# ika-rwth-aachen/PCLSegmentation

Measured on NVIDIA B200. Metric: range-image frames/sec (SqueezeSegV2, 64x2048), higher is better.
Workload: dtype f16 storage / f32 accumulate

## Files before the change

pclsegmentation_b200/csrc/conv_tc.cu:

```cuda
#include "tc_ptx.cuh"

#include <cstring>

namespace pcls {

constexpr int TC_MAX_TAPS = 9;
#ifndef PCLS_TC_VSTREAM
#define PCLS_TC_VSTREAM 0
#endif
#ifndef PCLS_TC_NG_NORES
#define PCLS_TC_NG_NORES 2
#endif
constexpr int tc_ng(bool res) { return res ? 2 : PCLS_TC_NG_NORES; }
constexpr int tc_threads(bool res) { return 64 + 128 * tc_ng(res); }

struct TcParams {
  int pdl_early;
  int BW, BH, bw_shift;
  int n_wt, n_ht, n_nt, n_phase, num_tiles;
  int Hgrid, Wgrid;
  int out_wmul;
  int Wout;
  int n_groups, sub;
  int kchunks;
  int ksteps;
  int KC, BN;
  int grp_dh[2][TC_MAX_TAPS], grp_dw[2][TC_MAX_TAPS], grp_par[2][TC_MAX_TAPS];
  int grp_w[2][TC_MAX_TAPS][3];
  int sub_row[3];
  int a_is_5d;
  int a_rows;
  int b_resident;
  int ntaps_total;
  int use_base_offset;
  int stages, a_bytes, b_tile_bytes, bres_bytes;
  uint32_t idesc, desc_hi;
  uint32_t tmem_cols;
  int n_acc;
  int tma_store, cbw, c_is_5d, c_stage_bytes;
  int G, cout_blk, cout_blk_shift;
  int res_smem;
  int res_tma;
  int n_cbuf;
  int n1, b_small_bytes, bres_tx;
  uint32_t idesc_small, idesc_lo;
  int nsplit, perm, cblk_off[8];
  int vstream, R, n_hseg;
  uint32_t desc_hi_b, idesc_blk;
  int cout, out_channels, out_coff, act, out_f32, is_bf16;
  void* out;
  const void* res0;
  const void* res1;
  int res0_channels, res1_channels;
  const float* bias;
  int skip;
  const void* skip_w;
  int head, none_index;
  const uint8_t* mask;
  float* probs;
  int32_t* preds;
  float* logits;
  unsigned long long* dbg;
};

template <typename T> __device__ __forceinline__ uint32_t pack2_relu(float lo, float hi);
template <> __device__ __forceinline__ uint32_t pack2_relu<__half>(float lo, float hi) {
  uint32_t d;
  asm("cvt.rn.relu.f16x2.f32 %0, %1, %2;" : "=r"(d) : "f"(hi), "f"(lo));
  return d;
}
template <> __device__ __forceinline__ uint32_t pack2_relu<__nv_bfloat16>(float lo, float hi) {
  uint32_t d;
  asm("cvt.rn.relu.bf16x2.f32 %0, %1, %2;" : "=r"(d) : "f"(hi), "f"(lo));
  return d;
}

template <typename T> __device__ __forceinline__ uint32_t add2_16(uint32_t a, uint32_t b);
template <> __device__ __forceinline__ uint32_t add2_16<__half>(uint32_t a, uint32_t b) {
  uint32_t d;
  asm("add.rn.f16x2 %0, %1, %2;" : "=r"(d) : "r"(a), "r"(b));
  return d;
}
template <> __device__ __forceinline__ uint32_t add2_16<__nv_bfloat16>(uint32_t a, uint32_t b) {
  uint32_t d;
  asm("add.rn.bf16x2 %0, %1, %2;" : "=r"(d) : "r"(a), "r"(b));
  return d;
}

#ifndef PCLS_TC_PACKED_SKIP
#define PCLS_TC_PACKED_SKIP 1
#endif

template <typename T> __device__ __forceinline__ uint32_t pack2_rn(float lo, float hi);
template <> __device__ __forceinline__ uint32_t pack2_rn<__half>(float lo, float hi) {
  uint32_t d;
  asm("cvt.rn.f16x2.f32 %0, %1, %2;" : "=r"(d) : "f"(hi), "f"(lo));
  return d;
}
template <> __device__ __forceinline__ uint32_t pack2_rn<__nv_bfloat16>(float lo, float hi) {
  uint32_t d;
  asm("cvt.rn.bf16x2.f32 %0, %1, %2;" : "=r"(d) : "f"(hi), "f"(lo));
  return d;
}
template <typename T> __device__ __forceinline__ void mma_16x8x8(float (&d)[4], uint32_t a0, uint32_t a1, uint32_t b);
template <> __device__ __forceinline__ void mma_16x8x8<__half>(float (&d)[4], uint32_t a0, uint32_t a1, uint32_t b) {
  asm volatile("mma.sync.aligned.m16n8k8.row.col.f32.f16.f16.f32 {%0, %1, %2, %3}, {%4, %5}, {%6}, {%7, %7, %7, %7};"
               : "=f"(d[0]), "=f"(d[1]), "=f"(d[2]), "=f"(d[3]) : "r"(a0), "r"(a1), "r"(b), "f"(0.0f));
}
template <> __device__ __forceinline__ void mma_16x8x8<__nv_bfloat16>(float (&d)[4], uint32_t a0, uint32_t a1, uint32_t b) {
  asm volatile("mma.sync.aligned.m16n8k8.row.col.f32.bf16.bf16.f32 {%0, %1, %2, %3}, {%4, %5}, {%6}, {%7, %7, %7, %7};"
               : "=f"(d[0]), "=f"(d[1]), "=f"(d[2]), "=f"(d[3]) : "r"(a0), "r"(a1), "r"(b), "f"(0.0f));
}
__device__ __forceinline__ void ldmatrix_x4(uint32_t addr, uint32_t (&r)[4]) {
  asm volatile("ldmatrix.sync.aligned.m8n8.x4.shared.b16 {%0, %1, %2, %3}, [%4];"
               : "=r"(r[0]), "=r"(r[1]), "=r"(r[2]), "=r"(r[3]) : "r"(addr) : "memory");
}
__device__ __forceinline__ void stmatrix_x4(uint32_t addr, uint32_t r0, uint32_t r1, uint32_t r2, uint32_t r3) {
  asm volatile("stmatrix.sync.aligned.m8n8.x4.shared.b16 [%0], {%1, %2, %3, %4};" ::"r"(addr), "r"(r0), "r"(r1), "r"(r2), "r"(r3)
               : "memory");
}

template <typename T, bool LEAKY, bool BIAS>
__device__ __forceinline__ int4 epilogue_vec8(const uint32_t* acc, const float* bias8, float lo, bool has_r0, const int4& r0,
                                              bool has_r1, const int4& r1) {
  if constexpr (!BIAS && !LEAKY) {
    if (!has_r0 && !has_r1) {
      int4 o;
      if (lo == 0.0f) {
        o.x = (int)pack2_relu<T>(__uint_as_float(acc[0]), __uint_as_float(acc[1]));
        o.y = (int)pack2_relu<T>(__uint_as_float(acc[2]), __uint_as_float(acc[3]));
        o.z = (int)pack2_relu<T>(__uint_as_float(acc[4]), __uint_as_float(acc[5]));
        o.w = (int)pack2_relu<T>(__uint_as_float(acc[6]), __uint_as_float(acc[7]));
      } else {
        const float f[8] = {__uint_as_float(acc[0]), __uint_as_float(acc[1]), __uint_as_float(acc[2]), __uint_as_float(acc[3]),
                            __uint_as_float(acc[4]), __uint_as_float(acc[5]), __uint_as_float(acc[6]), __uint_as_float(acc[7])};
        o = pack8<T>(f);
      }
      return o;
    }
  }
  if constexpr (PCLS_TC_PACKED_SKIP && !LEAKY) {
    if (has_r0 && !has_r1 && lo == 0.0f) {
      float v[8];
      if constexpr (BIAS) {
        const float4 b0 = *reinterpret_cast<const float4*>(bias8);
        const float4 b1 = *reinterpret_cast<const float4*>(bias8 + 4);
        v[0] = __uint_as_float(acc[0]) + b0.x; v[1] = __uint_as_float(acc[1]) + b0.y; v[2] = __uint_as_float(acc[2]) + b0.z;
        v[3] = __uint_as_float(acc[3]) + b0.w; v[4] = __uint_as_float(acc[4]) + b1.x; v[5] = __uint_as_float(acc[5]) + b1.y;
        v[6] = __uint_as_float(acc[6]) + b1.z; v[7] = __uint_as_float(acc[7]) + b1.w;
      } else {
#pragma unroll
        for (int j = 0; j < 8; ++j) v[j] = __uint_as_float(acc[j]);
      }
      int4 o;
      o.x = (int)add2_16<T>(pack2_relu<T>(v[0], v[1]), (uint32_t)r0.x);
      o.y = (int)add2_16<T>(pack2_relu<T>(v[2], v[3]), (uint32_t)r0.y);
      o.z = (int)add2_16<T>(pack2_relu<T>(v[4], v[5]), (uint32_t)r0.z);
      o.w = (int)add2_16<T>(pack2_relu<T>(v[6], v[7]), (uint32_t)r0.w);
      return o;
    }
  }
  float v[8];
  if constexpr (BIAS) {
    const float4 b0 = *reinterpret_cast<const float4*>(bias8);
    const float4 b1 = *reinterpret_cast<const float4*>(bias8 + 4);
    v[0] = __uint_as_float(acc[0]) + b0.x; v[1] = __uint_as_float(acc[1]) + b0.y; v[2] = __uint_as_float(acc[2]) + b0.z;
    v[3] = __uint_as_float(acc[3]) + b0.w; v[4] = __uint_as_float(acc[4]) + b1.x; v[5] = __uint_as_float(acc[5]) + b1.y;
    v[6] = __uint_as_float(acc[6]) + b1.z; v[7] = __uint_as_float(acc[7]) + b1.w;
  } else {
#pragma unroll
    for (int j = 0; j < 8; ++j) v[j] = __uint_as_float(acc[j]);
  }
#pragma unroll
  for (int j = 0; j < 8; ++j) v[j] = LEAKY ? fmaxf(v[j], v[j] * 0.1f) : fmaxf(v[j], lo);
  if (has_r0) {
    float f[8];
    unpack8<T>(r0, f);
#pragma unroll
    for (int j = 0; j < 8; ++j) v[j] += f[j];
  }
  if (has_r1) {
    float f[8];
    unpack8<T>(r1, f);
#pragma unroll
    for (int j = 0; j < 8; ++j) v[j] += f[j];
  }
  return pack8<T>(v);
}

template <typename T, int KC, int SUB, int G, bool RES, bool LEAKY, int KS = KC / 16, int RM = 0>
__global__ void __launch_bounds__(tc_threads(RES), 1)
conv_tc_kernel(const __grid_constant__ CUtensorMap map_a, const __grid_constant__ CUtensorMap map_b,
               const __grid_constant__ CUtensorMap map_c, const __grid_constant__ CUtensorMap map_r,
               const __grid_constant__ CUtensorMap map_b2, const __grid_constant__ CUtensorMap map_c2,
               const __grid_constant__ TcParams p, const int num_tiles) {
  constexpr bool PRELOAD = !RES;
  constexpr int TC_NG = tc_ng(RES);
  constexpr bool RTMA = RES && RM == 1;
  constexpr bool PTMA = !RES && RM == 2;
  constexpr bool SKIP = RES && RM == 3;
  static_assert(!SKIP || (G == 4 && !LEAKY), "the computed skip exists for the pixel-group view G = 4 with ReLU");
  constexpr bool FIXED = RTMA || SKIP;
  extern __shared__ uint8_t smem_raw[];
  const uint32_t smem_base = (smem_u32(smem_raw) + 1023u) & ~1023u;
  const int S = p.stages;
  const uint32_t a_bytes = (uint32_t)p.a_bytes, b_tile_bytes = (uint32_t)p.b_tile_bytes;
  const bool b_resident = p.b_resident != 0;
  const uint32_t b_stage_bytes = b_resident ? 0u : (uint32_t)SUB * b_tile_bytes;
  const uint32_t stage_bytes = a_bytes + b_stage_bytes;
  const uint32_t bres_base = smem_base + (uint32_t)S * stage_bytes;
  const uint32_t cstage_base = bres_base + (uint32_t)p.bres_bytes;
  const uint32_t rstage_base = cstage_base + (p.tma_store ? (uint32_t)(p.n_cbuf * TC_NG) * (uint32_t)p.c_stage_bytes : 0u);
  const uint32_t bar_base = rstage_base + ((RES && (SKIP || p.res_smem)) ? (uint32_t)TC_NG * 16384u : 0u);
#define FULL_BAR(s) (bar_base + 8u * (uint32_t)(s))
#define EMPTY_BAR(s) (bar_base + 8u * (uint32_t)(S + (s)))
#define TFULL_BAR(a) (bar_base + 8u * (uint32_t)(2 * S + (a)))
#define TEMPTY_BAR(a) (bar_base + 8u * (uint32_t)(2 * S + 8 + (a)))
#define BRES_BAR (bar_base + 8u * (uint32_t)(2 * S + 16))
#define RFULL_BAR(i) (bar_base + 8u * (uint32_t)(2 * S + 17 + (i)))
  const uint32_t tmem_slot = bar_base + 8u * (uint32_t)(2 * S + 17 + 3 * TC_NG);
  volatile uint32_t* tmem_slot_ptr =
      reinterpret_cast<volatile uint32_t*>(smem_raw + (tmem_slot - smem_u32(smem_raw)));
  float* bias_s = reinterpret_cast<float*>(smem_raw + (((tmem_slot + 16u + 15u) & ~15u) - smem_u32(smem_raw)));
  for (int i = threadIdx.x; i < p.n_nt * p.BN; i += blockDim.x) bias_s[i] = p.bias[G > 1 ? i % p.cout_blk : i];
  float* head_s = bias_s + ((p.n_nt * p.BN + 3) & ~3);

  const int warp = threadIdx.x >> 5, lane = threadIdx.x & 31;
  unsigned long long* const dbg = PCLS_TC_DEBUG ? p.dbg : nullptr;
  unsigned long long dbg_acc[8] = {0, 0, 0, 0, 0, 0, 0, 0};
  const unsigned long long dbg_start = dbg ? clk() : 0ull;

  if (warp == 0 && lane == 0) {
    asm volatile("prefetch.tensormap [%0];" ::"l"(&map_a) : "memory");
    asm volatile("prefetch.tensormap [%0];" ::"l"(&map_b) : "memory");
    if (p.n1 > 0) asm volatile("prefetch.tensormap [%0];" ::"l"(&map_b2) : "memory");
    if (p.tma_store) asm volatile("prefetch.tensormap [%0];" ::"l"(&map_c) : "memory");
    if (RES && (SKIP || p.res_tma)) asm volatile("prefetch.tensormap [%0];" ::"l"(&map_r) : "memory");
    for (int i = 0; i < 3 * TC_NG; ++i) mbar_init(RFULL_BAR(i), 1);
    for (int s = 0; s < S; ++s) { mbar_init(FULL_BAR(s), 1); mbar_init(EMPTY_BAR(s), 1); }
    for (int a = 0; a < 8; ++a) { mbar_init(TFULL_BAR(a), 1); mbar_init(TEMPTY_BAR(a), 4); }
    mbar_init(BRES_BAR, 1);
    asm volatile("fence.mbarrier_init.release.cluster;" ::: "memory");
    asm volatile("fence.proxy.async.shared::cta;" ::: "memory");
  }
  if (warp == 1) {
    asm volatile("tcgen05.alloc.cta_group::1.sync.aligned.shared::cta.b32 [%0], %1;" ::"r"(tmem_slot), "r"(p.tmem_cols)
                 : "memory");
    asm volatile("tcgen05.relinquish_alloc_permit.cta_group::1.sync.aligned;" ::: "memory");
  }
  tc_fence_before();
  __syncthreads();
  tc_fence_after();
  const uint32_t tmem_base = *tmem_slot_ptr;
  pdl_trigger(p.pdl_early);
  if (warp != 0) pdl_wait();

  const int n_groups = p.n_groups, kchunks = p.kchunks, n_nt = p.n_nt, n_phase = p.n_phase, n_wt = p.n_wt, n_ht = p.n_ht;
  const int BN = p.BN;

  if (warp == 0) {
    {
      if (b_resident) {
        mbar_arrive_expect_tx_elect(BRES_BAR, (uint32_t)p.bres_tx);
        uint32_t dst = bres_base;
        const int n0r = p.nsplit ? (int)(blockIdx.x % (unsigned)n_nt) * BN : 0;
        for (int ph = 0; ph < n_phase; ++ph)
          for (int g = 0; g < n_groups; ++g)
            for (int kc = 0; kc < kchunks; ++kc)
#pragma unroll
              for (int u = 0; u < SUB; ++u) {
                const int tap = p.grp_w[ph][g][u];
                if (p.n1 > 0 && tap != 4) {
                  tma_load_3d_elect(dst, &map_b2, BRES_BAR, kc * KC, n0r + p.n1, tap);
                  dst += (uint32_t)p.b_small_bytes;
                } else {
                  tma_load_3d_elect(dst, &map_b, BRES_BAR, kc * KC, n0r, tap);
                  dst += b_tile_bytes;
                }
              }
      }
      pdl_wait();
      const uint32_t a_tx_bytes = (uint32_t)(p.a_rows * KC * 2);
      const int BW = p.BW, BH = p.BH;
      const bool is5d = p.a_is_5d != 0;
      int stage = 0;
      uint32_t phase = 0;
      if (PCLS_TC_VSTREAM && p.vstream) {
        const int R = p.R, n_hseg = p.n_hseg, num_units = num_tiles / R;
        for (int unit = blockIdx.x; unit < num_units; unit += gridDim.x) {
          const int wt = unit % n_wt, hseg = (unit / n_wt) % n_hseg, b = unit / (n_wt * n_hseg);
          const int ww = wt * BW - 1;
          for (int hh = hseg * R - 1; hh <= hseg * R + R; ++hh)
            for (int kc = 0; kc < kchunks; ++kc) {
              { DBG_T0; mbar_wait(EMPTY_BAR(stage), phase ^ 1u); DBG_ADD(0); }
              const uint32_t fb = FULL_BAR(stage);
              mbar_arrive_expect_tx_elect(fb, a_tx_bytes);
              tma_load_4d_elect(smem_base + (uint32_t)stage * stage_bytes, &map_a, fb, kc * KC, ww, hh, b);
              if (++stage == S) { stage = 0; phase ^= 1u; }
            }
        }
      } else
      for (int tile = blockIdx.x; tile < num_tiles; tile += gridDim.x) {
        int r = tile;
        const int nt = r % n_nt; r /= n_nt;
        const int ph = r % n_phase; r /= n_phase;
        const int wt = r % n_wt; r /= n_wt;
        const int ht = r % n_ht;
        const int b = r / n_ht;
        const int w0 = wt * BW, h0 = ht * BH, n0 = nt * BN;
        for (int g = 0; g < n_groups; ++g) {
          const int hh = h0 + p.grp_dh[ph][g], ww = w0 + p.grp_dw[ph][g], par = p.grp_par[ph][g];
          int wtap[SUB];
#pragma unroll
          for (int u = 0; u < SUB; ++u) wtap[u] = p.grp_w[ph][g][u];
          for (int kc = 0; kc < kchunks; ++kc) {
            { DBG_T0; mbar_wait(EMPTY_BAR(stage), phase ^ 1u); DBG_ADD(0); }
            const uint32_t a_dst = smem_base + (uint32_t)stage * stage_bytes;
            const uint32_t fb = FULL_BAR(stage);
            uint32_t tx_bytes = a_tx_bytes;
            if (!b_resident) {
#pragma unroll
              for (int u = 0; u < SUB; ++u) tx_bytes += (p.n1 > 0 && wtap[u] != 4) ? (uint32_t)p.b_small_bytes : b_tile_bytes;
            }
            mbar_arrive_expect_tx_elect(fb, tx_bytes);
            if (is5d) tma_load_5d_elect(a_dst, &map_a, fb, kc * KC, par, ww, hh, b);
            else tma_load_4d_elect(a_dst, &map_a, fb, kc * KC, ww, hh, b);
            if (!b_resident) {
#pragma unroll
              for (int u = 0; u < SUB; ++u) {
                if (p.n1 > 0 && wtap[u] != 4)
                  tma_load_3d_elect(a_dst + a_bytes + (uint32_t)u * b_tile_bytes, &map_b2, fb, kc * KC, p.n1, wtap[u]);
                else
                  tma_load_3d_elect(a_dst + a_bytes + (uint32_t)u * b_tile_bytes, &map_b, fb, kc * KC, n0, wtap[u]);
              }
            }
            if (++stage == S) { stage = 0; phase ^= 1u; }
          }
        }
      }
    }
  } else if (warp == 1) {
    {
      const uint32_t desc_hi = p.desc_hi, idesc = p.idesc;
      const uint32_t n_acc = (uint32_t)p.n_acc;
      uint32_t sub_off[SUB];
#pragma unroll
      for (int u = 0; u < SUB; ++u) sub_off[u] = (uint32_t)(p.sub_row[u] * KC * 2);
      const int k_iters = n_groups * kchunks;
      const uint32_t bres_phase_bytes = (uint32_t)(k_iters * SUB) * b_tile_bytes;
      int stage = 0;
      uint32_t phase = 0, acc = 0, acc_phase = 0;
      if (b_resident) mbar_wait(BRES_BAR, 0u);
      const bool vs = PCLS_TC_VSTREAM && p.vstream != 0;
      const int vs_R = vs ? p.R : 1;
      const int my_tiles = vs ? ((num_tiles / vs_R - (int)blockIdx.x + (int)gridDim.x - 1) / (int)gridDim.x) * vs_R
                              : (num_tiles - (int)blockIdx.x + (int)gridDim.x - 1) / (int)gridDim.x;
      uint32_t vs_slot = 0, vs_phase = 0, vs_idx = 0, vs_waited = 0;
      int vs_row = 0;
      auto vs_release = [&](int n) {
        for (int i = 0; i < n; ++i) {
          umma_commit_elect(EMPTY_BAR(vs_slot));
          if (++vs_slot == (uint32_t)S) { vs_slot = 0; vs_phase ^= 1u; }
        }
        vs_idx += (uint32_t)n;
      };
      for (int seq = 0; seq < my_tiles; ++seq) {
        const int tile = blockIdx.x + seq * gridDim.x;
        { DBG_T0; mbar_wait(TEMPTY_BAR(acc), PRELOAD ? acc_phase : (acc_phase ^ 1u)); DBG_ADD(1); }
        tc_fence_after();
        const uint32_t d_tmem = tmem_base + acc * (uint32_t)BN;
        uint32_t b_res = bres_base + (n_phase > 1 ? (uint32_t)((tile / n_nt) % n_phase) * bres_phase_bytes : 0u);
        uint32_t accumulate = PRELOAD ? 1u : 0u, acc_lo = accumulate;
        int kc_i = 0, g_i = 0;
        for (int k = 0; k < k_iters; ++k) {
          uint32_t a_addr;
          if (vs) {
            uint32_t sl = vs_slot + (uint32_t)k, par = vs_phase;
            if (sl >= (uint32_t)S) { sl -= (uint32_t)S; par ^= 1u; }
            if (vs_idx + (uint32_t)k >= vs_waited) {
              { DBG_T0; mbar_wait(FULL_BAR(sl), par); DBG_ADD(2); }
              vs_waited = vs_idx + (uint32_t)k + 1u;
            }
            a_addr = smem_base + sl * stage_bytes;
          } else {
            { DBG_T0; mbar_wait(FULL_BAR(stage), phase); DBG_ADD(2); }
            a_addr = smem_base + (uint32_t)stage * stage_bytes;
          }
          tc_fence_after();
          if constexpr (G == 1) {
            uint32_t b_addr = b_resident ? b_res : a_addr + a_bytes;
            const uint32_t n1 = (uint32_t)p.n1;
#pragma unroll
            for (int u = 0; u < SUB; ++u) {
              const uint64_t a_desc = ((uint64_t)desc_hi << 32) | (uint64_t)((((a_addr + sub_off[u]) >> 4) & 0x3FFFu) | 0x10000u);
              const uint64_t b_desc = ((uint64_t)desc_hi << 32) | (uint64_t)(((b_addr >> 4) & 0x3FFFu) | 0x10000u);
              if (n1 == 0u) {
#pragma unroll
                for (int j = 0; j < KS; ++j) {
                  umma_f16_elect(d_tmem, a_desc + (uint64_t)(2 * j), b_desc + (uint64_t)(2 * j), idesc, accumulate);
                  accumulate = 1u;
                }
                b_addr += b_tile_bytes;
              } else if (p.grp_w[0][g_i][u] != 4) {
#pragma unroll
                for (int j = 0; j < KC / 16; ++j) {
                  umma_f16_elect(d_tmem + n1, a_desc + (uint64_t)(2 * j), b_desc + (uint64_t)(2 * j), p.idesc_small, accumulate);
                  accumulate = 1u;
                }
                b_addr += b_resident ? (uint32_t)p.b_small_bytes : b_tile_bytes;
              } else {
                const uint32_t b_hi = b_addr + n1 * (uint32_t)(KC * 2);
                const uint64_t b_desc_hi = ((uint64_t)desc_hi << 32) | (uint64_t)(((b_hi >> 4) & 0x3FFFu) | 0x10000u);
#pragma unroll
                for (int j = 0; j < KC / 16; ++j) {
                  umma_f16_elect(d_tmem, a_desc + (uint64_t)(2 * j), b_desc + (uint64_t)(2 * j), p.idesc_lo, acc_lo);
                  umma_f16_elect(d_tmem + n1, a_desc + (uint64_t)(2 * j), b_desc_hi + (uint64_t)(2 * j), p.idesc_small, accumulate);
                  acc_lo = 1u; accumulate = 1u;
                }
                b_addr += b_tile_bytes;
              }
            }
            if (b_resident) b_res = b_addr;
          } else {
            constexpr int CIN = KC / G;
            const uint32_t desc_hi_b = p.desc_hi_b, idesc_blk = p.idesc_blk, cout_blk = (uint32_t)p.cout_blk;
#pragma unroll
            for (int u = 0; u < SUB; ++u) {
              const uint32_t b_addr = b_res + (uint32_t)u * b_tile_bytes;
              const uint64_t b_desc = ((uint64_t)desc_hi_b << 32) | (uint64_t)(((b_addr >> 4) & 0x3FFFu) | 0x10000u);
#pragma unroll
              for (int pp = 0; pp < G; ++pp) {
                constexpr int dummy = 0; (void)dummy;
                const int t = pp + (SUB == 3 ? u - 1 : 0);
                const int dq = t < 0 ? -1 : (t >= G ? 1 : 0);
                const int par = t - dq * G;
                const uint32_t a_start = a_addr + (uint32_t)((SUB == 3 ? dq + 1 : 0) * KC * 2 + par * CIN * 2);
                const uint64_t a_desc = ((uint64_t)desc_hi << 32) | (uint64_t)(((a_start >> 4) & 0x3FFFu) | 0x10000u);
#pragma unroll
                for (int j = 0; j < CIN / 16; ++j)
                  umma_f16_elect(d_tmem + (uint32_t)pp * cout_blk, a_desc + (uint64_t)(2 * j), b_desc + (uint64_t)(2 * j),
                           idesc_blk, (PRELOAD || (k | u | j) != 0) ? 1u : 0u);
              }
            }
          }
          if constexpr (G > 1) b_res += (uint32_t)SUB * b_tile_bytes;
          if (++kc_i == kchunks) { kc_i = 0; ++g_i; }
          if (!vs) {
            umma_commit_elect(EMPTY_BAR(stage));
            if (++stage == S) { stage = 0; phase ^= 1u; }
          }
        }
        if (vs) {
          if (++vs_row == vs_R) { vs_row = 0; vs_release(3 * kchunks); }
          else vs_release(kchunks);
        }
        umma_commit_elect(TFULL_BAR(acc));
        if (++acc == n_acc) { acc = 0; acc_phase ^= 1u; }
      }
    }
  } else {
    const int grp = (warp - 2) >> 2;
    const int q = warp & 3;
    const int m = q * 32 + lane;
    const int ml_h = m >> p.bw_shift, ml_w = m & (p.BW - 1);
    const uint32_t n_acc = (uint32_t)p.n_acc;
    const int BW = p.BW, BH = p.BH, Hgrid = p.Hgrid, Wgrid = p.Wgrid, Wout = p.Wout, out_wmul = p.out_wmul;
    const int cout = p.cout, out_channels = p.out_channels, out_coff = p.out_coff;
    const int blk_shift = p.cout_blk_shift;
    const int blk_mask = G > 1 ? (1 << blk_shift) - 1 : -1;
    const float slope = p.act == PCLS_ACT_RELU ? 0.0f : (p.act == PCLS_ACT_LEAKY ? 0.1f : 1.0f);
    const float act_lo = (FIXED || p.act == PCLS_ACT_RELU) ? 0.0f : -INFINITY;
    const uint16_t* res0 = reinterpret_cast<const uint16_t*>(p.res0);
    const uint16_t* res1 = reinterpret_cast<const uint16_t*>(p.res1);
    const int res0_channels = p.res0_channels, res1_channels = p.res1_channels;
    const bool has_r0 = FIXED || res0 != nullptr, has_r1 = !FIXED && res1 != nullptr;
    const bool tma_store = FIXED || PTMA || p.tma_store != 0, out_f32 = !FIXED && !PTMA && p.out_f32 != 0, c_is_5d = p.c_is_5d != 0;
    const uint32_t c_stage_bytes = (uint32_t)p.c_stage_bytes;
    T* const outp = reinterpret_cast<T*>(p.out);
    const bool issuer = (q == 2) && lane == 0;
    const int bar_id = 1 + grp;
    const uint32_t ng = n_acc < (uint32_t)TC_NG ? n_acc : (uint32_t)TC_NG;
    uint32_t tl = 0, blk = 0;
    const uint32_t nrb = (uint32_t)p.n_cbuf;
    auto issue_res = [&](int rtile, int rcb, uint32_t bi) {
      int r2 = rtile;
      const int nt2 = r2 % n_nt; r2 /= n_nt;
      const int ph2 = r2 % n_phase; r2 /= n_phase;
      const int wt2 = r2 % n_wt; r2 /= n_wt;
      const int ht2 = r2 % n_ht;
      const int b2 = r2 / n_ht;
      const uint32_t dst = cstage_base + (uint32_t)(grp * p.n_cbuf + (int)bi) * c_stage_bytes;
      const uint32_t bar = RFULL_BAR(grp * 3 + (int)bi);
      const int pp2 = G > 1 ? (nt2 * BN + rcb) >> blk_shift : 0;
      const int c02 = out_coff + (p.perm ? p.cblk_off[(nt2 * BN + rcb) >> 6] : ((nt2 * BN + rcb) & blk_mask));
      mbar_arrive_expect_tx(bar, 128u * 64u * 2u);
      if (c_is_5d) tma_load_5d(dst, &map_r, bar, c02, G > 1 ? pp2 : ph2, wt2 * BW, ht2 * BH, b2);
      else tma_load_4d(dst, &map_r, bar, c02, wt2 * BW, ht2 * BH, b2);
    };
    const bool vs = PCLS_TC_VSTREAM && p.vstream != 0;
    const int vs_R = vs ? p.R : 1, vs_hseg = p.n_hseg;
    auto tile_at = [&](uint32_t seq) -> int {
      if (!vs) {
        const long long t = (long long)blockIdx.x + (long long)seq * gridDim.x;
        return t < num_tiles ? (int)t : -1;
      }
      const int unit = (int)blockIdx.x + (int)(seq / (uint32_t)vs_R) * (int)gridDim.x;
      if (unit >= num_tiles / vs_R) return -1;
      const int i = (int)(seq % (uint32_t)vs_R);
      const int uwt = unit % n_wt, hseg = (unit / n_wt) % vs_hseg, ub = unit / (n_wt * vs_hseg);
      return (ub * n_ht + hseg * vs_R + i) * n_wt + uwt;
    };
    if (RES && !SKIP && p.res_tma != 0 && has_r0 && issuer && (uint32_t)grp < ng && tile_at((uint32_t)grp) >= 0)
      issue_res(tile_at((uint32_t)grp), 0, 0u);
    uint32_t skw[8] = {0, 0, 0, 0, 0, 0, 0, 0};
    const uint32_t in_base = rstage_base + (uint32_t)grp * 16384u;
    const bool ones_lane = (lane & 3) == 3;
    const uint32_t one2 = std::is_same<T, __half>::value ? 0x3C003C00u : 0x3F803F80u;
    if constexpr (SKIP) {
      const uint32_t* w32 = reinterpret_cast<const uint32_t*>(p.skip_w);
#pragma unroll
      for (int j = 0; j < 8; ++j) skw[j] = __ldg(w32 + (8 * j + (lane >> 2)) * 4 + (lane & 3));
    }
    auto issue_in = [&](int rtile, uint32_t bi) {
      const int wt2 = (rtile / n_nt / n_phase) % n_wt;
      const int ht2 = (rtile / n_nt / n_phase / n_wt) % n_ht;
      const int b2 = rtile / n_nt / n_phase / n_wt / n_ht;
      const uint32_t bar = RFULL_BAR(grp * 3 + (int)bi);
      mbar_arrive_expect_tx(bar, 8192u);
      tma_load_4d(in_base + bi * 8192u, &map_r, bar, 0, wt2 * BW, ht2 * BH, b2);
    };
    auto compute_skip = [&](uint32_t buf, int pp, uint32_t in_buf) {
      uint32_t a[4];
      ldmatrix_x4(in_buf + (uint32_t)(m * 64) + (uint32_t)((pp ^ ((m >> 1) & 3)) << 4), a);
#pragma unroll
      for (int k = 0; k < 4; ++k) a[k] = ones_lane ? one2 : a[k];
      const int sr = (q * 32 + ((lane >> 3) & 1) * 8 + (lane & 7));
#pragma unroll
      for (int i = 0; i < 2; ++i)
#pragma unroll
        for (int jp = 0; jp < 4; ++jp) {
          float d0[4], d1[4];
          mma_16x8x8<T>(d0, a[2 * i], a[2 * i + 1], skw[2 * jp]);
          mma_16x8x8<T>(d1, a[2 * i], a[2 * i + 1], skw[2 * jp + 1]);
          const uint32_t chunk = (uint32_t)((2 * jp + (lane >> 4)) ^ (lane & 7));
          stmatrix_x4(buf + (uint32_t)((sr + 16 * i) * 128) + (chunk << 4), pack2_rn<T>(d0[0], d0[1]), pack2_rn<T>(d0[2], d0[3]),
                      pack2_rn<T>(d1[0], d1[1]), pack2_rn<T>(d1[2], d1[3]));
        }
      __syncwarp();
    };
    if (SKIP && issuer && (uint32_t)grp < ng && tile_at((uint32_t)grp) >= 0) issue_in(tile_at((uint32_t)grp), 0u);
    auto preload_bias = [&](uint32_t a, int tile_next) {
      if (tile_next >= 0) {
        const float* bsrc = bias_s + (tile_next % n_nt) * BN;
        const uint32_t t_dst = tmem_base + ((uint32_t)(q * 32) << 16) + a * (uint32_t)BN;
#pragma unroll 1
        for (int c = 0; c + 32 <= BN; c += 32) {
          uint32_t bv[32];
#pragma unroll
          for (int j = 0; j < 32; j += 4) {
            const float4 t4 = *reinterpret_cast<const float4*>(bsrc + c + j);
            bv[j] = __float_as_uint(t4.x); bv[j + 1] = __float_as_uint(t4.y); bv[j + 2] = __float_as_uint(t4.z); bv[j + 3] = __float_as_uint(t4.w);
          }
          tmem_st32(t_dst + (uint32_t)c, bv);
        }
        if (BN & 16) {
          uint32_t bv[16];
#pragma unroll
          for (int j = 0; j < 16; j += 4) {
            const float4 t4 = *reinterpret_cast<const float4*>(bsrc + (BN & ~31) + j);
            bv[j] = __float_as_uint(t4.x); bv[j + 1] = __float_as_uint(t4.y); bv[j + 2] = __float_as_uint(t4.z); bv[j + 3] = __float_as_uint(t4.w);
          }
          tmem_st16(t_dst + (uint32_t)(BN & ~31), bv);
        }
        tmem_st_wait();
      }
      tc_fence_before();
      __syncwarp();
      if (lane == 0) mbar_arrive(TEMPTY_BAR(a));
    };
    if (PRELOAD && (uint32_t)grp < ng)
      for (uint32_t a = (uint32_t)grp; a < n_acc; a += ng) preload_bias(a, tile_at(a));
    for (; (uint32_t)grp < ng; ++tl) {
      const int tile = tile_at(tl);
      if (tile < 0) break;
      if ((int)(tl % ng) != grp) continue;
      int r = tile;
      const int nt = r % n_nt; r /= n_nt;
      const int ph = r % n_phase; r /= n_phase;
      const int wt = r % n_wt; r /= n_wt;
      const int ht = r % n_ht;
      const int b = r / n_ht;
      const int h = ht * BH + ml_h, w = wt * BW + ml_w;
      const bool valid = h < Hgrid && w < Wgrid;
      const int64_t pix = ((int64_t)b * Hgrid + h) * Wout + (int64_t)w * out_wmul + ph;
      const uint32_t acc = tl & (n_acc - 1u), acc_parity = (tl / n_acc) & 1u;
      const int n0 = nt * BN;
      const uint32_t t_row = tmem_base + ((uint32_t)(q * 32) << 16) + acc * (uint32_t)BN;
      auto elem_off = [&](int n, int channels) -> int64_t {
        const int pp = G > 1 ? n >> blk_shift : 0;
        const int co = n & blk_mask;
        return (valid && co + 8 <= cout) ? (pix + pp) * channels + out_coff + co : (int64_t)-1;
      };
      const uint32_t rslot = rstage_base + (uint32_t)grp * 16384u + (uint32_t)(m & 127) * 16u;
      int4 r0[4], r1[4];
      const bool res_smem = !FIXED && RES && p.res_smem != 0 && has_r0;
      const bool res_tma = RTMA || (RES && !SKIP && p.res_tma != 0 && has_r0);
      const bool res_stage = res_tma || SKIP;
      uint32_t res_row = 0;
      auto prefetch_r0 = [&](int cs) {
        if constexpr (RES) {
          if (res_smem) {
#pragma unroll 4
            for (int i = 0; i < 8; ++i) {
              const int64_t o = (cs + i * 8 < BN) ? elem_off(n0 + cs + i * 8, res0_channels) : (int64_t)-1;
              cp_async16(rslot + (uint32_t)i * 2048u, res0 + (o >= 0 ? o : 0), o >= 0);
            }
            cp_async_commit();
          }
        }
      };
      auto load_r1 = [&](int c) {
        if constexpr (RES) {
#pragma unroll
          for (int g = 0; g < 4; ++g) {
            const int64_t o = has_r1 ? elem_off(n0 + c + g * 8, res1_channels) : (int64_t)-1;
            r1[g] = o >= 0 ? __ldg(reinterpret_cast<const int4*>(res1 + o)) : make_int4(0, 0, 0, 0);
            if (has_r0 && !res_smem && !res_stage) {
              const int64_t o0 = elem_off(n0 + c + g * 8, res0_channels);
              r0[g] = o0 >= 0 ? __ldg(reinterpret_cast<const int4*>(res0 + o0)) : make_int4(0, 0, 0, 0);
            }
          }
        }
      };
      const bool reg_res = RES && (has_r1 || (has_r0 && !res_smem && !res_stage));
      prefetch_r0(0);
      if (reg_res) load_r1(0);
      uint8_t head_mask = 1;
      if (out_f32 && p.head && valid) head_mask = p.mask[pix];
      { DBG_T0; mbar_wait(TFULL_BAR(acc), acc_parity); DBG_ADD(3); }
      const unsigned long long _te = dbg ? clk() : 0ull;
      tc_fence_after();
      if (res_smem) cp_async_wait_all();
      auto process = [&](const uint32_t* v, int cc, auto&& sink) {
        if constexpr (RES) {
          if (res_smem && cc > 0 && (cc & 63) == 0) { prefetch_r0(cc); cp_async_wait_all(); }
        }
#pragma unroll
        for (int g = 0; g < 4; ++g) {
          int4 r0v = make_int4(0, 0, 0, 0);
          if constexpr (RES) {
            r0v = res_stage ? ld_shared_v4(res_row + (uint32_t)(((((cc & 63) >> 3) + g) ^ (m & 7)) << 4))
                : res_smem ? ld_shared_v4(rslot + (uint32_t)(((cc & 63) >> 3) + g) * 2048u) : r0[g];
          }
          sink(g, epilogue_vec8<T, LEAKY, !PRELOAD>(v + g * 8, bias_s + n0 + cc + g * 8, act_lo, RES && has_r0, r0v, RES && has_r1, r1[g]));
        }
        if (reg_res && cc + 32 < BN) load_r1(cc + 32);
      };
      auto chunk = [&](int cc, auto&& sink) {
        uint32_t v[32];
        if (cc + 32 <= BN) {
          tmem_ld32(t_row + (uint32_t)cc, v);
        } else {
          uint32_t v16[16];
          tmem_ld16(t_row + (uint32_t)cc, v16);
#pragma unroll
          for (int j = 0; j < 16; ++j) { v[j] = v16[j]; v[16 + j] = 0u; }
        }
        tmem_ld_wait();
        process(v, cc, sink);
      };
      bool released = false;
      auto release_acc = [&]() {
        released = true;
        if constexpr (PRELOAD) {
          preload_bias(acc, tile_at(tl + n_acc));
        } else {
          tc_fence_before();
          __syncwarp();
          if (lane == 0) mbar_arrive(TEMPTY_BAR(acc));
        }
      };
      if (out_f32) {
        float lg[32];
        {
          uint32_t v[32];
          if (BN >= 32) {
            tmem_ld32(t_row, v);
          } else {
            uint32_t v16[16];
            tmem_ld16(t_row, v16);
#pragma unroll
            for (int j = 0; j < 16; ++j) { v[j] = v16[j]; v[16 + j] = 0u; }
          }
          tmem_ld_wait();
#pragma unroll
          for (int c4 = 0; c4 < 32; c4 += 4) {
            if (c4 < cout) {
#pragma unroll
              for (int j = c4; j < c4 + 4; ++j) {
                const float x = __uint_as_float(v[j]) + (PRELOAD ? 0.0f : bias_s[n0 + j]);
                lg[j] = (j < cout) ? fmaxf(x, x * slope) : -INFINITY;
              }
            }
          }
        }
        float* stg = head_s + (warp - 2) * (32 * 33);
        const int64_t pix0 = __shfl_sync(0xffffffffu, pix, 0);
        const int n_valid = __popc(__ballot_sync(0xffffffffu, valid));
        auto write_rows = [&](float* dst) {
          if ((cout & 3) == 0) {
            if (lane == 0) bulk_wait_read0();
            __syncwarp();
#pragma unroll
            for (int c4 = 0; c4 < 32; c4 += 4)
              if (c4 < cout) *reinterpret_cast<float4*>(stg + lane * cout + c4) = make_float4(lg[c4], lg[c4 + 1], lg[c4 + 2], lg[c4 + 3]);
            asm volatile("fence.proxy.async.shared::cta;" ::: "memory");
            __syncwarp();
            if (lane == 0 && n_valid > 0) {
              bulk_store_1d(dst + pix0 * cout, smem_u32(stg), (uint32_t)(n_valid * cout * 4));
              bulk_commit();
            }
            return;
          }
          __syncwarp();
#pragma unroll
          for (int c = 0; c < 32; ++c) if (c < cout) stg[lane * 33 + c] = lg[c];
          __syncwarp();
          const int n_el = n_valid * cout;
          int px = lane / cout, cc = lane - px * cout;
          const int dpx = 32 / cout, dcc = 32 - dpx * cout;
          for (int e = lane; e < n_el; e += 32) {
            dst[pix0 * cout + e] = stg[px * 33 + cc];
            px += dpx; cc += dcc;
            if (cc >= cout) { cc -= cout; ++px; }
          }
        };
        if (!p.head) {
          if (valid) {
            float* o = reinterpret_cast<float*>(p.out) + pix * out_channels + out_coff;
#pragma unroll
            for (int c = 0; c < 32; ++c) if (c < cout) o[c] = lg[c];
          }
        } else {
          if (p.logits) write_rows(p.logits);
          float mx = lg[0];
#pragma unroll
          for (int c4 = 0; c4 < 32; c4 += 4)
            if (c4 < cout) mx = fmaxf(fmaxf(mx, fmaxf(lg[c4], lg[c4 + 1])), fmaxf(lg[c4 + 2], lg[c4 + 3]));
          float sum = 0.0f;
#pragma unroll
          for (int c4 = 0; c4 < 32; c4 += 4)
            if (c4 < cout) {
#pragma unroll
              for (int j = c4; j < c4 + 4; ++j) { lg[j] = ex2_ftz((lg[j] - mx) * 1.4426950408889634f); sum += lg[j]; }
            }
          const float inv = __fdividef(1.0f, sum);
          int best = 0;
          float bp = -1.0f;
#pragma unroll
          for (int c4 = 0; c4 < 32; c4 += 4)
            if (c4 < cout) {
#pragma unroll
              for (int j = c4; j < c4 + 4; ++j) { lg[j] *= inv; if (lg[j] > bp) { bp = lg[j]; best = j; } }
            }
          if (valid) {
            if (head_mask == 0) best = p.none_index;
            p.preds[pix] = best;
          }
          if (p.probs) write_rows(p.probs);
        }
      } else if (tma_store) {
        constexpr bool DBUF = !(RES && G == 1);
        uint32_t va[32], vb[DBUF ? 32 : 1];
        if constexpr (DBUF) tmem_ld32(t_row, va);
        for (int cb = 0; cb < BN; cb += 64, ++blk) {
          uint32_t buf;
          if (res_tma) {
            if (issuer) {
              int ntile = tile, ncb = cb + 64;
              if (ncb >= BN) { ncb = 0; ntile = tile_at(tl + ng); }
              if (ntile >= 0) {
                if (nrb == 3u) bulk_wait_read1(); else bulk_wait_read0();
                issue_res(ntile, ncb, (blk + 1u) % nrb);
              }
            }
            buf = cstage_base + (uint32_t)(grp * (int)nrb + (int)(blk % nrb)) * c_stage_bytes;
            { DBG_T0; mbar_wait(RFULL_BAR(grp * 3 + (int)(blk % nrb)), (blk / nrb) & 1u); DBG_ADD(4); }
          } else {
            buf = cstage_base + (uint32_t)(grp * 2 + (int)(blk & 1u)) * c_stage_bytes;
            if constexpr (SKIP) {
              const uint32_t tg = tl / ng;
              if (cb == 0) {
                if (issuer && tile_at(tl + ng) >= 0) issue_in(tile_at(tl + ng), (tg + 1u) & 1u);
                DBG_T0; mbar_wait(RFULL_BAR(grp * 3 + (int)(tg & 1u)), (tg >> 1) & 1u); DBG_ADD(4);
              }
              compute_skip(buf, cb >> 6, in_base + (tg & 1u) * 8192u);
            }
          }
          const bool narrow = !RES && BN - cb < 64;
          const uint32_t row_addr = buf + (uint32_t)(m * (narrow ? 64 : 128));
          res_row = row_addr;
          if constexpr (!DBUF) {
#pragma unroll 1
            for (int ci = 0; ci < 2; ++ci)
              chunk(cb + ci * 32, [&](int g, const int4& o) {
                st_shared_v4(row_addr + (uint32_t)(((ci * 4 + g) ^ (m & 7)) << 4), o); });
          } else if (narrow) {
            tmem_ld_wait();
            release_acc();
            process(va, cb, [&](int g, const int4& o) { st_shared_v4(row_addr + (uint32_t)((g ^ ((m >> 1) & 3)) << 4), o); });
          } else {
            tmem_ld_wait();
            tmem_ld32(t_row + (uint32_t)(cb + 32), vb);
            process(va, cb, [&](int g, const int4& o) { st_shared_v4(row_addr + (uint32_t)((g ^ (m & 7)) << 4), o); });
            tmem_ld_wait();
            if (cb + 64 < BN) tmem_ld32(t_row + (uint32_t)(cb + 64), va);
            else release_acc();
            process(vb, cb + 32, [&](int g, const int4& o) { st_shared_v4(row_addr + (uint32_t)(((4 + g) ^ (m & 7)) << 4), o); });
          }
          asm volatile("fence.proxy.async.shared::cta;" ::: "memory");
          if (!res_tma) { DBG_T0; if (issuer) bulk_wait_read0(); DBG_ADD(4); }
          { DBG_T0; group_barrier(bar_id); DBG_ADD(5); }
          if (issuer) {
            const int pp = G > 1 ? (n0 + cb) >> blk_shift : 0;
            const int c0 = out_coff + (p.perm ? p.cblk_off[(n0 + cb) >> 6] : ((n0 + cb) & blk_mask));
            if (c_is_5d) tma_store_5d(&map_c, buf, c0, G > 1 ? pp : ph, wt * BW, ht * BH, b);
            else tma_store_4d(narrow ? &map_c2 : &map_c, buf, c0, wt * BW, ht * BH, b);
            bulk_commit();
          }
        }
      } else {
#pragma unroll 1
        for (int c = 0; c < BN; c += 32)
          chunk(c, [&](int g, const int4& o) {
            const int64_t off = (c + g * 8 < BN) ? elem_off(n0 + c + g * 8, out_channels) : (int64_t)-1;
            if (off >= 0) *reinterpret_cast<int4*>(outp + off) = o;
          });
      }
      if (!released) release_acc();
      if (dbg) { dbg_acc[6] += clk() - _te; dbg_acc[7] += 1; }
    }
    if (p.tma_store && q == 2 && lane == 0) bulk_wait_all();
    if (out_f32 && lane == 0) bulk_wait_all();
  }

  if (dbg && lane == 0 && (warp == 0 || warp == 1 || warp == 2 || warp == 6)) {
    unsigned long long* o = dbg + (size_t)blockIdx.x * 24;
    if (warp == 0) { o[0] = dbg_acc[0]; o[8] = clk() - dbg_start; }
    if (warp == 1) { o[1] = dbg_acc[1]; o[2] = dbg_acc[2]; o[9] = clk() - dbg_start; }
    if (warp == 2) { for (int i = 3; i < 8; ++i) o[i] = dbg_acc[i]; o[10] = clk() - dbg_start; }
    if (warp == 6) { for (int i = 3; i < 8; ++i) o[8 + i] = dbg_acc[i]; }
  }
  __syncwarp();
  tc_fence_before();
  __syncthreads();
  if (warp == 1) {
    tc_fence_after();
    asm volatile("tcgen05.dealloc.cta_group::1.sync.aligned.b32 %0, %1;" ::"r"(tmem_base), "r"(p.tmem_cols) : "memory");
  }
#undef FULL_BAR
#undef EMPTY_BAR
#undef TFULL_BAR
#undef TEMPTY_BAR
#undef BRES_BAR
#undef RFULL_BAR
}

typedef void (*TcKernelFn)(const CUtensorMap, const CUtensorMap, const CUtensorMap, const CUtensorMap, const CUtensorMap, const CUtensorMap, const TcParams, const int);

#ifndef PCLS_TC_PART
#define PCLS_TC_PART -1
#endif
template <typename T, bool RES, bool LEAKY>
TcKernelFn tc_kernel_for_t(int KC, int SUB, int G) {
  if (G == 4) return SUB == 3 ? conv_tc_kernel<T, 64, 3, 4, RES, LEAKY> : conv_tc_kernel<T, 64, 1, 4, RES, LEAKY>;
  if (G == 2) {
    if (KC == 64) return SUB == 3 ? conv_tc_kernel<T, 64, 3, 2, RES, LEAKY> : conv_tc_kernel<T, 64, 1, 2, RES, LEAKY>;
    return SUB == 3 ? conv_tc_kernel<T, 32, 3, 2, RES, LEAKY> : conv_tc_kernel<T, 32, 1, 2, RES, LEAKY>;
  }
  if (SUB == 3) return KC == 64 ? conv_tc_kernel<T, 64, 3, 1, RES, LEAKY> : KC == 32 ? conv_tc_kernel<T, 32, 3, 1, RES, LEAKY> : conv_tc_kernel<T, 16, 3, 1, RES, LEAKY>;
  return KC == 64 ? conv_tc_kernel<T, 64, 1, 1, RES, LEAKY> : KC == 32 ? conv_tc_kernel<T, 32, 1, 1, RES, LEAKY> : conv_tc_kernel<T, 16, 1, 1, RES, LEAKY>;
}
template <typename T, bool LEAKY>
TcKernelFn tc_ptma_kernel_for(int KC, int SUB, int G, int ks) {
  if constexpr (!LEAKY) {
    if (ks == 3 && KC == 64 && SUB == 3 && G == 1) return conv_tc_kernel<T, 64, 3, 1, false, false, 3, 2>;
  }
  if (G == 4) return SUB == 3 ? conv_tc_kernel<T, 64, 3, 4, false, LEAKY, 4, 2> : conv_tc_kernel<T, 64, 1, 4, false, LEAKY, 4, 2>;
  if (G == 2) {
    if (KC == 64) return SUB == 3 ? conv_tc_kernel<T, 64, 3, 2, false, LEAKY, 4, 2> : conv_tc_kernel<T, 64, 1, 2, false, LEAKY, 4, 2>;
    return SUB == 3 ? conv_tc_kernel<T, 32, 3, 2, false, LEAKY, 2, 2> : conv_tc_kernel<T, 32, 1, 2, false, LEAKY, 2, 2>;
  }
  if (SUB == 3) return KC == 64 ? conv_tc_kernel<T, 64, 3, 1, false, LEAKY, 4, 2> : KC == 32 ? conv_tc_kernel<T, 32, 3, 1, false, LEAKY, 2, 2> : conv_tc_kernel<T, 16, 3, 1, false, LEAKY, 1, 2>;
  return KC == 64 ? conv_tc_kernel<T, 64, 1, 1, false, LEAKY, 4, 2> : KC == 32 ? conv_tc_kernel<T, 32, 1, 1, false, LEAKY, 2, 2> : conv_tc_kernel<T, 16, 1, 1, false, LEAKY, 1, 2>;
}
#if PCLS_TC_PART >= 0
#if PCLS_TC_PART == 1
template TcKernelFn tc_kernel_for_t<__half, false, false>(int, int, int);
#else
extern template TcKernelFn tc_kernel_for_t<__half, false, false>(int, int, int);
#endif
#if PCLS_TC_PART == 2
template TcKernelFn tc_kernel_for_t<__half, false, true>(int, int, int);
#else
extern template TcKernelFn tc_kernel_for_t<__half, false, true>(int, int, int);
#endif
#if PCLS_TC_PART == 3
template TcKernelFn tc_kernel_for_t<__half, true, false>(int, int, int);
#else
extern template TcKernelFn tc_kernel_for_t<__half, true, false>(int, int, int);
#endif
#if PCLS_TC_PART == 4
template TcKernelFn tc_kernel_for_t<__half, true, true>(int, int, int);
#else
extern template TcKernelFn tc_kernel_for_t<__half, true, true>(int, int, int);
#endif
#if PCLS_TC_PART == 5
template TcKernelFn tc_kernel_for_t<__nv_bfloat16, false, false>(int, int, int);
#else
extern template TcKernelFn tc_kernel_for_t<__nv_bfloat16, false, false>(int, int, int);
#endif
#if PCLS_TC_PART == 6
template TcKernelFn tc_kernel_for_t<__nv_bfloat16, false, true>(int, int, int);
#else
extern template TcKernelFn tc_kernel_for_t<__nv_bfloat16, false, true>(int, int, int);
#endif
#if PCLS_TC_PART == 7
template TcKernelFn tc_kernel_for_t<__nv_bfloat16, true, false>(int, int, int);
#else
extern template TcKernelFn tc_kernel_for_t<__nv_bfloat16, true, false>(int, int, int);
#endif
#if PCLS_TC_PART == 8
template TcKernelFn tc_kernel_for_t<__nv_bfloat16, true, true>(int, int, int);
#else
extern template TcKernelFn tc_kernel_for_t<__nv_bfloat16, true, true>(int, int, int);
#endif
#if PCLS_TC_PART == 9
template TcKernelFn tc_ptma_kernel_for<__half, false>(int, int, int, int);
#else
extern template TcKernelFn tc_ptma_kernel_for<__half, false>(int, int, int, int);
#endif
#if PCLS_TC_PART == 10
template TcKernelFn tc_ptma_kernel_for<__half, true>(int, int, int, int);
#else
extern template TcKernelFn tc_ptma_kernel_for<__half, true>(int, int, int, int);
#endif
#if PCLS_TC_PART == 11
template TcKernelFn tc_ptma_kernel_for<__nv_bfloat16, false>(int, int, int, int);
#else
extern template TcKernelFn tc_ptma_kernel_for<__nv_bfloat16, false>(int, int, int, int);
#endif
#if PCLS_TC_PART == 12
template TcKernelFn tc_ptma_kernel_for<__nv_bfloat16, true>(int, int, int, int);
#else
extern template TcKernelFn tc_ptma_kernel_for<__nv_bfloat16, true>(int, int, int, int);
#endif
#endif

#if PCLS_TC_PART <= 0
template <typename T>
static TcKernelFn tc_kernel_for_tt(int KC, int SUB, int G, int res, int leaky) {
  if (res) return leaky ? tc_kernel_for_t<T, true, true>(KC, SUB, G) : tc_kernel_for_t<T, true, false>(KC, SUB, G);
  return leaky ? tc_kernel_for_t<T, false, true>(KC, SUB, G) : tc_kernel_for_t<T, false, false>(KC, SUB, G);
}
static bool tc_kskip_kernel(int KC, int SUB, int G, int res, int leaky, int ks) {
  return ks == 3 && KC == 64 && SUB == 3 && G == 1 && !res && !leaky;
}
static bool tc_rtma_kernel(int KC, int SUB, int G, int res, int leaky, int rtma) {
  return rtma == 1 && res && KC == 64 && SUB == 3 && (G == 1 || G == 2 || G == 4);
}
template <typename T, bool LEAKY>
static TcKernelFn tc_rtma_kernel_for(int G) {
  if (G == 4) return conv_tc_kernel<T, 64, 3, 4, true, LEAKY, 4, 1>;
  if (G == 2) return conv_tc_kernel<T, 64, 3, 2, true, LEAKY, 4, 1>;
  return conv_tc_kernel<T, 64, 3, 1, true, LEAKY, 4, 1>;
}
static TcKernelFn tc_kernel_for(int KC, int SUB, int G, int is_bf16, int res, int leaky, int ks = 0, int rtma = 0) {
  if (rtma == 3)
    return is_bf16 ? conv_tc_kernel<__nv_bfloat16, 64, 3, 4, true, false, 4, 3> : conv_tc_kernel<__half, 64, 3, 4, true, false, 4, 3>;
  if (rtma == 2 && !res) {
    if (is_bf16) return leaky ? tc_ptma_kernel_for<__nv_bfloat16, true>(KC, SUB, G, ks) : tc_ptma_kernel_for<__nv_bfloat16, false>(KC, SUB, G, ks);
    return leaky ? tc_ptma_kernel_for<__half, true>(KC, SUB, G, ks) : tc_ptma_kernel_for<__half, false>(KC, SUB, G, ks);
  }
  if (tc_rtma_kernel(KC, SUB, G, res, leaky, rtma)) {
    if (is_bf16) return leaky ? tc_rtma_kernel_for<__nv_bfloat16, true>(G) : tc_rtma_kernel_for<__nv_bfloat16, false>(G);
    return leaky ? tc_rtma_kernel_for<__half, true>(G) : tc_rtma_kernel_for<__half, false>(G);
  }
  if (tc_kskip_kernel(KC, SUB, G, res, leaky, ks))
    return is_bf16 ? conv_tc_kernel<__nv_bfloat16, 64, 3, 1, false, false, 3> : conv_tc_kernel<__half, 64, 3, 1, false, false, 3>;
  return is_bf16 ? tc_kernel_for_tt<__nv_bfloat16>(KC, SUB, G, res, leaky) : tc_kernel_for_tt<__half>(KC, SUB, G, res, leaky);
}

struct TcPlan {
  CUtensorMap map_a, map_b, map_c, map_r, map_b2, map_c2;
  TcParams prm;
  size_t smem_bytes;
  void* w_dev;
  float* bias_dev;
  ~TcPlan() { if (w_dev) cudaFree(w_dev); if (bias_dev) cudaFree(bias_dev); }
};

typedef CUresult (*EncodeTiledFn)(CUtensorMap*, CUtensorMapDataType, cuuint32_t, void*, const cuuint64_t*,
                                  const cuuint64_t*, const cuuint32_t*, const cuuint32_t*, CUtensorMapInterleave,
                                  CUtensorMapSwizzle, CUtensorMapL2promotion, CUtensorMapFloatOOBfill);

static EncodeTiledFn encode_fn() {
  static EncodeTiledFn fn = nullptr;
  if (!fn) {
    void* sym = nullptr;
    cudaDriverEntryPointQueryResult q;
    if (cudaGetDriverEntryPoint("cuTensorMapEncodeTiled", &sym, cudaEnableDefault, &q) == cudaSuccess &&
        q == cudaDriverEntryPointSuccess)
      fn = (EncodeTiledFn)sym;
  }
  return fn;
}

int make_map(CUtensorMap* map, bool bf16, void* base, int rank, const uint64_t* dims, const uint64_t* strides_bytes,
                    const uint32_t* box, int swizzle_bytes) {
  EncodeTiledFn fn = encode_fn();
  if (!fn) { set_error("cuTensorMapEncodeTiled is not available from the driver"); return PCLS_ERR_CUDA; }
  cuuint64_t gd[5], gs[4];
  cuuint32_t bx[5], es[5];
  for (int i = 0; i < rank; ++i) { gd[i] = dims[i]; bx[i] = box[i]; es[i] = 1; }
  for (int i = 0; i + 1 < rank; ++i) gs[i] = strides_bytes[i];
  const CUtensorMapSwizzle sw = swizzle_bytes == 128 ? CU_TENSOR_MAP_SWIZZLE_128B
                              : swizzle_bytes == 64 ? CU_TENSOR_MAP_SWIZZLE_64B
                              : swizzle_bytes == 32 ? CU_TENSOR_MAP_SWIZZLE_32B : CU_TENSOR_MAP_SWIZZLE_NONE;
  CUresult r = fn(map, bf16 ? CU_TENSOR_MAP_DATA_TYPE_BFLOAT16 : CU_TENSOR_MAP_DATA_TYPE_FLOAT16, (cuuint32_t)rank, base,
                  gd, gs, bx, es, CU_TENSOR_MAP_INTERLEAVE_NONE, sw, CU_TENSOR_MAP_L2_PROMOTION_L2_256B,
                  CU_TENSOR_MAP_FLOAT_OOB_FILL_NONE);
  if (r != CUDA_SUCCESS) { set_error("cuTensorMapEncodeTiled failed with CUresult %d (rank %d)", (int)r, rank); return PCLS_ERR_CUDA; }
  return PCLS_OK;
}

int tc_rtma_mode = 3;
int tc_tma_store_mode = 1, tc_group_mode = 1, tc_res_tma_mode = 1, tc_split_mode = 1, tc_vstream_mode = 0, tc_nsplit_mode = 1;
const int tc_debug_compiled = PCLS_TC_DEBUG;
unsigned long long* tc_debug_buf = nullptr;
int tc_halo_mode = 1, tc_resident_mode = 1, tc_base_offset_mode = 0;

static bool tc_eligible(const ConvParams& p) {
  if (p.in_channels < 16 || p.cin_pad > p.in_channels) return false;
  if (p.mode == MODE_3x3_S2 && (p.Win % 2 != 0 || p.pad_left != 0)) return false;
  if (p.cout_pad > 256 && p.cout_pad % 256 != 0) return false;
  return true;
}

static int tc_group_size(const ConvParams& cp) {
  if (tc_group_mode && tc_resident_mode && (cp.mode == MODE_1x1 || cp.mode == MODE_3x3_S1 || cp.mode == MODE_ROW3) &&
      (cp.cin_pad == 16 || cp.cin_pad == 32) && cp.in_channels == cp.cin_pad && cp.cout == cp.cout_pad && !cp.out_f32 &&
      cp.Wout == cp.Win) {
    for (int g = 64 / cp.cin_pad; g >= 2; g /= 2)
      if (cp.Win % g == 0 && cp.Win / g >= 128 && g * cp.cout_pad <= 256 && (cp.cout_pad & (cp.cout_pad - 1)) == 0) return g;
  }
  return 1;
}

bool Net::tc_skip_fusable(const ConvLayer& P, const ConvLayer& E) const {
  const ConvParams &pp = P.p, &e = E.p;
  if (P.in != 0 || pp.mode != MODE_1x1 || pp.act != PCLS_ACT_NONE || P.res0 >= 0 || P.res1 >= 0 ||
      pp.out_f32 || pp.out_coff != 0 || P.cin_logical > 6 || pp.cout != 64 || pp.out_channels != 64)
    return false;
  if (E.res0 != P.out || E.res1 >= 0 || E.in == P.out || E.pair_view || e.mode != MODE_3x3_S1 || e.act != PCLS_ACT_RELU ||
      e.out_f32 || e.cout != 64 || e.res0_channels != 64)
    return false;
  if (!tc_eligible(e) || tc_group_size(e) != 4 || !tc_halo_mode || !tc_tma_store_mode || !tc_res_tma_mode || !tc_rtma_mode ||
      (e.out_channels * 2) % 16 != 0)
    return false;
  return true;
}

int Net::tc_plan_layer(ConvLayer& L, bool allow_group, bool* retry) {
  const int max_smem = 227 * 1024;
    ConvParams& cp = L.pair_view ? L.ptc : L.p;
    L.tc_ok = false;
    *retry = false;
    if (!tc_eligible(cp)) return PCLS_OK;
    TcPlan* plan = new TcPlan();
    memset(plan, 0, sizeof(TcPlan));
    TcParams& q = plan->prm;
    const int TC_NG = tc_ng(L.res0 >= 0 || L.res1 >= 0);
    const bool bf16 = precision == PCLS_BF16;
    q.KC = (cp.cin_pad % 64 == 0) ? 64 : (cp.cin_pad % 32 == 0) ? 32 : 16;
    q.kchunks = cp.cin_pad / q.KC;
    q.ksteps = q.KC / 16;
    q.BN = cp.cout_pad <= 256 ? cp.cout_pad : 256;
    q.n_nt = cp.cout_pad / q.BN;
    const int G = allow_group ? tc_group_size(cp) : 1;
    const bool skip = L.skip_src >= 0;
    const int cin_blk = cp.cin_pad;
    q.G = G; q.cout_blk = G > 1 ? cp.cout_pad : (1 << 30);
    q.cout_blk_shift = 0;
    while ((1 << q.cout_blk_shift) < q.cout_blk && q.cout_blk_shift < 30) ++q.cout_blk_shift;
    if (G > 1) { q.KC = G * cin_blk; q.kchunks = 1; q.BN = G * cp.cout_pad; q.n_nt = 1; }
    const int swz = q.KC * 2;
    const int swz_b = G > 1 ? cin_blk * 2 : swz;
    q.n1 = 0;
    if (tc_split_mode && G == 1 && cp.mode == MODE_3x3_S1 && q.n_nt == 1 && !L.pair_view) {
      int z = 0;
      for (; z < cp.cout_pad; ++z) {
        bool zero = true;
        for (int t = 0; t < 9 && zero; ++t) {
          if (t == 4) continue;
          const float* wr = &L.w_f32[((size_t)t * cp.cout_pad + z) * cp.cin_pad];
          for (int ci = 0; ci < cp.cin_pad; ++ci) if (wr[ci] != 0.0f) { zero = false; break; }
        }
        if (!zero) break;
      }
      z = z / 16 * 16;
      if (z >= 16 && q.BN - z >= 16) q.n1 = z;
    }
#ifndef PCLS_TC_KSKIP
#define PCLS_TC_KSKIP 1
#endif
    if (PCLS_TC_KSKIP && G == 1 && q.kchunks == 1 && q.n1 == 0) q.ksteps = std::min(q.KC / 16, (cp.cin + 15) / 16);
    q.nsplit = 0; q.perm = 0;
    for (int i = 0; i < 8; ++i) q.cblk_off[i] = i * 64;
    std::vector<int> row_perm;
    if (tc_nsplit_mode && tc_resident_mode && tc_halo_mode && G == 1 && cp.mode == MODE_3x3_S1 && q.n_nt == 1 && !L.pair_view &&
        q.KC == 64 && !cp.out_f32 && cp.cout == cp.cout_pad && cp.Wout >= 128 && L.res1 < 0) {
      const int btile1 = q.BN * q.KC * 2, bsmall1 = (q.BN - q.n1) * q.KC * 2;
      const int all_w1 = q.n1 > 0 ? q.kchunks * (btile1 + 8 * bsmall1) : 9 * q.kchunks * btile1;
      const int half = q.BN / 2;
      if (all_w1 > 112 * 1024) {
        if (q.n1 > 0 && q.n1 % 128 == 0 && (q.BN - q.n1) % 128 == 0 && tc_tma_store_mode && (L.res0 < 0 || tc_res_tma_mode)) {
          const int h1 = q.n1 / 2, h3 = (q.BN - q.n1) / 2;
          if (q.kchunks * ((h1 + h3) * q.KC * 2 + 8 * h3 * q.KC * 2) <= 112 * 1024) {
            row_perm.resize(q.BN);
            int blk = 0;
            for (int nt = 0; nt < 2; ++nt) {
              for (int j = 0; j < h1; ++j) row_perm[nt * (h1 + h3) + j] = nt * h1 + j;
              for (int j = 0; j < h3; ++j) row_perm[nt * (h1 + h3) + h1 + j] = q.n1 + nt * h3 + j;
              for (int j = 0; j < h1; j += 64) q.cblk_off[blk++] = nt * h1 + j;
              for (int j = 0; j < h3; j += 64) q.cblk_off[blk++] = q.n1 + nt * h3 + j;
            }
            q.BN = h1 + h3; q.n_nt = 2; q.n1 = h1; q.nsplit = 1; q.perm = 1;
          }
        } else if (q.n1 == 0 && half % 32 == 0 && 9 * q.kchunks * half * q.KC * 2 <= 112 * 1024) {
          q.BN = half; q.n_nt = 2; q.nsplit = 1;
        }
      }
    }
    q.b_small_bytes = (q.BN - q.n1) * q.KC * 2;
    const bool deconv = cp.mode == MODE_DECONV;
    q.Hgrid = cp.H;
    q.Wgrid = deconv ? cp.Win : cp.Wout / G;
    q.Wout = cp.Wout;
    q.out_wmul = deconv ? 2 : G;
    q.n_phase = deconv ? 2 : 1;
    int bw = 128;
    while (bw > 1 && bw / 2 >= q.Wgrid) bw /= 2;
    q.BW = bw; q.BH = 128 / bw;
    q.bw_shift = 0;
    while ((1 << q.bw_shift) < bw) ++q.bw_shift;
    q.n_wt = (q.Wgrid + q.BW - 1) / q.BW;
    q.n_ht = (q.Hgrid + q.BH - 1) / q.BH;
    q.num_tiles = q.n_nt * q.n_phase * q.n_wt * q.n_ht;
    q.a_is_5d = cp.mode == MODE_3x3_S2 ? 1 : 0;
    q.sub = 1; q.a_rows = 128; q.ntaps_total = cp.ntaps;
    q.use_base_offset = tc_base_offset_mode;
    bool halo = (cp.mode == MODE_3x3_S1 || cp.mode == MODE_ROW3) && q.BW == 128 && tc_halo_mode;
    if (halo) {
      const int btile_ = G > 1 ? cp.cout_pad * cin_blk * 2 : q.BN * q.KC * 2;
      const int all_w_ = q.n1 > 0 ? q.kchunks * (btile_ + (cp.ntaps - 1) * q.b_small_bytes) : cp.ntaps * q.kchunks * btile_;
      const bool resident_ = tc_resident_mode && (q.n_nt == 1 || q.nsplit) && all_w_ <= 112 * 1024;
      const int st_ = (130 * q.KC * 2 + 1023) / 1024 * 1024 + (resident_ ? 0 : 3 * btile_);
      const int staging_ = 2 * TC_NG * 16384 + ((L.res0 >= 0 && (q.BN <= 128 || resident_) && !q.nsplit) ? TC_NG * 16384 : 0);
      if ((max_smem - 2048 - staging_ - cp.cout_pad * 4 - (resident_ ? all_w_ + 1024 : 0)) / st_ < 3) halo = false;
    }
    if (G > 1 && cp.mode != MODE_1x1 && !halo) {
      delete plan;
      *retry = true;
      return PCLS_OK;
    }
    if (cp.mode == MODE_1x1) {
      q.n_groups = 1;
    } else if (halo && cp.mode == MODE_3x3_S1) {
      q.n_groups = 3; q.sub = 3; q.a_rows = 130;
      for (int g = 0; g < 3; ++g) {
        q.grp_dh[0][g] = g - 1; q.grp_dw[0][g] = -1;
        for (int u = 0; u < 3; ++u) q.grp_w[0][g][u] = g * 3 + u;
      }
      q.sub_row[0] = 0; q.sub_row[1] = 1; q.sub_row[2] = 2;
    } else if (halo && cp.mode == MODE_ROW3) {
      q.n_groups = 1; q.sub = 3; q.a_rows = 130;
      q.grp_dh[0][0] = 0; q.grp_dw[0][0] = -1;
      for (int u = 0; u < 3; ++u) { q.grp_w[0][0][u] = u; q.sub_row[u] = u; }
    } else if (cp.mode == MODE_ROW3) {
      q.n_groups = 3;
      for (int t = 0; t < 3; ++t) { q.grp_dh[0][t] = 0; q.grp_dw[0][t] = t - 1; q.grp_w[0][t][0] = t; }
    } else if (cp.mode == MODE_3x3_S1) {
      q.n_groups = 9;
      for (int t = 0; t < 9; ++t) { q.grp_dh[0][t] = t / 3 - 1; q.grp_dw[0][t] = t % 3 - 1; q.grp_w[0][t][0] = t; }
    } else if (cp.mode == MODE_PAIR6) {
      q.n_groups = 6;
      for (int t = 0; t < 6; ++t) { q.grp_dh[0][t] = t / 2 - 1; q.grp_dw[0][t] = t % 2; q.grp_w[0][t][0] = t; }
    } else if (cp.mode == MODE_3x3_S2) {
      q.n_groups = 9;
      for (int t = 0; t < 9; ++t) {
        q.grp_dh[0][t] = t / 3 - 1; q.grp_par[0][t] = (t % 3) & 1; q.grp_dw[0][t] = (t % 3) >> 1; q.grp_w[0][t][0] = t;
      }
    } else {
      q.n_groups = 2;
      q.grp_dw[0][0] = 0;  q.grp_w[0][0][0] = 1;
      q.grp_dw[0][1] = -1; q.grp_w[0][1][0] = 3;
      q.grp_dw[1][0] = 1;  q.grp_w[1][0][0] = 0;
      q.grp_dw[1][1] = 0;  q.grp_w[1][1][0] = 2;
    }
    q.tma_store = 0; q.cbw = 0; q.c_stage_bytes = 0; q.c_is_5d = (deconv || G > 1) ? 1 : 0;
    const bool narrow_tail = q.BN % 64 == 32 && q.BN > 64 && G == 1 && !deconv && L.res0 < 0 && L.res1 < 0;
    if (tc_tma_store_mode && !cp.out_f32 && cp.cout == cp.cout_pad && (q.BN % 64 == 0 || narrow_tail) &&
        (G == 1 || cp.cout_pad % 64 == 0) &&
        (cp.out_channels * 2) % 16 == 0) {
      q.tma_store = 1;
      q.cbw = q.BN < 64 ? q.BN : 64;
      q.c_stage_bytes = (128 * q.cbw * 2 + 1023) / 1024 * 1024;
    }
    q.a_bytes = (q.a_rows * q.KC * 2 + 1023) / 1024 * 1024;
    q.b_tile_bytes = G > 1 ? cp.cout_pad * cin_blk * 2 : q.BN * q.KC * 2;
    const int all_w = q.n1 > 0 ? q.kchunks * (q.b_tile_bytes + 8 * q.b_small_bytes)
                               : q.n_phase * q.n_groups * q.kchunks * q.sub * q.b_tile_bytes;
    q.bres_tx = all_w;
    q.b_resident = (tc_resident_mode && (q.n_nt == 1 || q.nsplit) && all_w <= 112 * 1024) ? 1 : 0;
    if (q.nsplit && !q.b_resident) { set_error("tc plan: N-split layer lost its resident weights"); delete plan; return PCLS_ERR_STATE; }
    q.bres_bytes = q.b_resident ? (all_w + 1023) / 1024 * 1024 : 0;
    q.res_tma = (!skip && tc_res_tma_mode && L.res0 >= 0 && q.tma_store && q.cbw == 64 && q.b_resident && (cp.res0_channels * 2) % 16 == 0) ? 1 : 0;
    q.n_cbuf = (q.res_tma && !q.nsplit) ? 3 : 2;
    q.res_smem = (!skip && !q.res_tma && L.res0 >= 0 && q.BN <= 128) ? 1 : 0;
    const int cstage_total = (q.tma_store ? q.n_cbuf * TC_NG * q.c_stage_bytes : 0) + ((q.res_smem || skip) ? TC_NG * 16384 : 0);
    if (skip && !(G == 4 && q.tma_store && q.cbw == 64 && q.b_resident && q.BN == 256 && q.BW == 128 && q.BH == 1)) {
      set_error("tc plan: the layer that computes the fused skip is not planned on the G = 4 TMA-store path");
      delete plan; return PCLS_ERR_STATE;
    }
    if (G > 1 && !q.b_resident) { delete plan; *retry = true; return PCLS_OK; }
    const int stage_bytes = q.a_bytes + (q.b_resident ? 0 : q.sub * q.b_tile_bytes);
    int stages = (max_smem - 2048 - cp.cout_pad * 4 - q.bres_bytes - cstage_total - (cp.out_f32 ? 4 * TC_NG * 32 * 33 * 4 : 0)) / stage_bytes;
    if (stages > 12) stages = 12;
    if (stages < 2) { delete plan; *retry = G > 1; return PCLS_OK; }
    q.stages = stages;
    q.vstream = (PCLS_TC_VSTREAM && tc_vstream_mode && halo && cp.mode == MODE_3x3_S1 && q.b_resident && stages >= 3 * q.kchunks + 1) ? 1 : 0;
    q.R = 1; q.n_hseg = q.Hgrid;
    plan->smem_bytes = (size_t)stages * stage_bytes + q.bres_bytes + cstage_total + 1024  +
                       (size_t)(2 * stages + 17 + 3 * TC_NG) * 8 + 48 + (cp.out_f32 ? 4 * TC_NG * 32 * 33 * 4 : 0) + (size_t)cp.cout_pad * 4 ;
    const uint32_t layout = swz == 128 ? 2u : swz == 64 ? 4u : 6u;
    const uint32_t sbo = (uint32_t)(8 * swz) >> 4;
    q.desc_hi = sbo | (1u << 14)  | (layout << 29);
    {
      const uint32_t layout_b = swz_b == 128 ? 2u : swz_b == 64 ? 4u : 6u;
      q.desc_hi_b = ((uint32_t)(8 * swz_b) >> 4) | (1u << 14) | (layout_b << 29);
      q.idesc_blk = (1u << 4) | ((bf16 ? 1u : 0u) << 7) | ((bf16 ? 1u : 0u) << 10) |
                    ((uint32_t)(cp.cout_pad >> 3) << 17) | ((uint32_t)(128 >> 4) << 24);
    }
    q.idesc = (1u << 4)  | ((bf16 ? 1u : 0u) << 7) | ((bf16 ? 1u : 0u) << 10) |
              ((uint32_t)(q.BN >> 3) << 17) | ((uint32_t)(128 >> 4) << 24);
    q.idesc_small = (q.idesc & ~(0x3Fu << 17)) | ((uint32_t)((q.BN - q.n1) >> 3) << 17);
    q.idesc_lo = (q.idesc & ~(0x3Fu << 17)) | ((uint32_t)(q.n1 >> 3) << 17);
    q.n_acc = 2;
    while (q.n_acc < 8 && q.n_acc * 2 * q.BN <= 512) q.n_acc *= 2;
    uint32_t cols = 32;
    while (cols < (uint32_t)(q.n_acc * q.BN)) cols <<= 1;
    q.tmem_cols = cols;
    q.cout = cp.cout; q.out_channels = cp.out_channels; q.out_coff = cp.out_coff; q.act = cp.act;
    q.out_f32 = cp.out_f32; q.is_bf16 = bf16 ? 1 : 0;
    q.res0_channels = cp.res0_channels; q.res1_channels = cp.res1_channels;
    q.bias = cp.bias;

    char* a_base = (char*)tensor_ptr(L.in, frames_per_pass);
    const uint64_t C = (uint64_t)cp.in_channels * G, Wi = (uint64_t)cp.Win / G, Hh = (uint64_t)cp.H, F = (uint64_t)frames_per_pass;
    int rc;
    if (q.a_is_5d) {
      const uint64_t dims[5] = {C, 2, Wi / 2, Hh, F};
      const uint64_t str[4] = {C * 2, C * 4, Wi * C * 2, Hh * Wi * C * 2};
      const uint32_t box[5] = {(uint32_t)q.KC, 1, (uint32_t)q.BW, (uint32_t)q.BH, 1};
      rc = make_map(&plan->map_a, bf16, a_base, 5, dims, str, box, swz);
    } else {
      const uint64_t dims[4] = {C, Wi, Hh, F};
      const uint64_t str[3] = {C * 2, Wi * C * 2, Hh * Wi * C * 2};
      const uint32_t box[4] = {(uint32_t)q.KC, (uint32_t)(q.BH == 1 ? q.a_rows : q.BW), (uint32_t)q.BH, 1};
      rc = make_map(&plan->map_a, bf16, a_base, 4, dims, str, box, swz);
    }
    if (rc) { delete plan; return rc; }
    const void* w_src = cp.w;
    if (q.perm) {
      std::vector<uint16_t> hw((size_t)cp.ntaps * cp.cout_pad * cp.cin_pad);
      std::vector<float> hb(cp.cout_pad);
      for (int t = 0; t < cp.ntaps; ++t)
        for (int n = 0; n < cp.cout_pad; ++n)
          for (int ci = 0; ci < cp.cin_pad; ++ci) {
            const float w = L.w_f32[((size_t)t * cp.cout_pad + row_perm[n]) * cp.cin_pad + ci];
            uint16_t bits;
            if (bf16) { __nv_bfloat16 hv = __float2bfloat16_rn(w); memcpy(&bits, &hv, 2); }
            else { __half hv = __float2half_rn(w); memcpy(&bits, &hv, 2); }
            hw[((size_t)t * cp.cout_pad + n) * cp.cin_pad + ci] = bits;
          }
      for (int n = 0; n < cp.cout_pad; ++n) hb[n] = L.bias_f32[row_perm[n]];
      if (cudaMalloc(&plan->w_dev, hw.size() * 2) != cudaSuccess || cudaMalloc((void**)&plan->bias_dev, hb.size() * 4) != cudaSuccess ||
          cudaMemcpy(plan->w_dev, hw.data(), hw.size() * 2, cudaMemcpyHostToDevice) != cudaSuccess ||
          cudaMemcpy(plan->bias_dev, hb.data(), hb.size() * 4, cudaMemcpyHostToDevice) != cudaSuccess) {
        set_error("tc plan: upload of the permuted weights failed"); delete plan; return PCLS_ERR_CUDA;
      }
      w_src = plan->w_dev;
      q.bias = plan->bias_dev;
    }
    {
      const uint64_t dims[3] = {(uint64_t)cp.cin_pad, (uint64_t)cp.cout_pad, (uint64_t)cp.ntaps};
      const uint64_t str[2] = {(uint64_t)cp.cin_pad * 2, (uint64_t)cp.cin_pad * cp.cout_pad * 2};
      const uint32_t box[3] = {(uint32_t)(G > 1 ? cin_blk : q.KC), (uint32_t)(G > 1 ? cp.cout_pad : q.BN), 1};
      rc = make_map(&plan->map_b, bf16, const_cast<void*>(w_src), 3, dims, str, box, swz_b);
    }
    if (rc) { delete plan; return rc; }
    plan->map_b2 = plan->map_b;
    if (q.n1 > 0) {
      const uint64_t dims[3] = {(uint64_t)cp.cin_pad, (uint64_t)cp.cout_pad, (uint64_t)cp.ntaps};
      const uint64_t str[2] = {(uint64_t)cp.cin_pad * 2, (uint64_t)cp.cin_pad * cp.cout_pad * 2};
      const uint32_t box[3] = {(uint32_t)q.KC, (uint32_t)(q.BN - q.n1), 1};
      rc = make_map(&plan->map_b2, bf16, const_cast<void*>(w_src), 3, dims, str, box, swz_b);
      if (rc) { delete plan; return rc; }
    }
    if (q.tma_store) {
      char* c_base = (char*)tensor_ptr(L.out, frames_per_pass);
      const uint64_t Co = (uint64_t)cp.out_channels, Wo = (uint64_t)cp.Wout;
      const int csw = q.cbw == 64 ? 128 : 0;
      if (q.c_is_5d) {
        const uint64_t gg = G > 1 ? (uint64_t)G : 2;
        const uint64_t dims[5] = {Co, gg, Wo / gg, Hh, F};
        const uint64_t str[4] = {Co * 2, Co * 2 * gg, Wo * Co * 2, Hh * Wo * Co * 2};
        const uint32_t box[5] = {(uint32_t)q.cbw, 1, (uint32_t)q.BW, (uint32_t)q.BH, 1};
        rc = make_map(&plan->map_c, bf16, c_base, 5, dims, str, box, csw);
      } else {
        const uint64_t dims[4] = {Co, Wo, Hh, F};
        const uint64_t str[3] = {Co * 2, Wo * Co * 2, Hh * Wo * Co * 2};
        const uint32_t box[4] = {(uint32_t)q.cbw, (uint32_t)q.BW, (uint32_t)q.BH, 1};
        rc = make_map(&plan->map_c, bf16, c_base, 4, dims, str, box, csw);
      }
      if (rc) { delete plan; return rc; }
      plan->map_c2 = plan->map_c;
      if (q.BN % 64 == 32) {
        const uint64_t dims[4] = {Co, Wo, Hh, F};
        const uint64_t str[3] = {Co * 2, Wo * Co * 2, Hh * Wo * Co * 2};
        const uint32_t box[4] = {32u, (uint32_t)q.BW, (uint32_t)q.BH, 1};
        rc = make_map(&plan->map_c2, bf16, c_base, 4, dims, str, box, 64);
        if (rc) { delete plan; return rc; }
      }
    } else {
      plan->map_c = plan->map_a;
      plan->map_c2 = plan->map_a;
    }
    plan->map_r = plan->map_c;
    if (skip) {
      const ConvLayer& P = convs[L.skip_src];
      const uint64_t dims[4] = {32, (uint64_t)W / 4, Hh, F};
      const uint64_t str[3] = {64, (uint64_t)W / 4 * 64, Hh * (uint64_t)W / 4 * 64};
      const uint32_t box[4] = {32, (uint32_t)q.BW, 1, 1};
      rc = make_map(&plan->map_r, bf16, tensor_ptr(P.in, frames_per_pass), 4, dims, str, box, 64);
      if (rc) { delete plan; return rc; }
      std::vector<float> ws(64 * 8, 0.0f);
      for (int n = 0; n < 64; ++n) {
        for (int ci = 0; ci < P.cin_logical; ++ci) ws[n * 8 + ci] = P.w_f32[(size_t)n * P.p.cin_pad + ci];
        const float b = P.bias_f32[n];
        const float hi = bf16 ? __bfloat162float(__float2bfloat16_rn(b)) : __half2float(__float2half_rn(b));
        ws[n * 8 + 6] = hi; ws[n * 8 + 7] = b - hi;
      }
      std::vector<uint16_t> hw(ws.size());
      for (size_t i = 0; i < ws.size(); ++i) {
        if (bf16) { __nv_bfloat16 hv = __float2bfloat16_rn(ws[i]); memcpy(&hw[i], &hv, 2); }
        else { __half hv = __float2half_rn(ws[i]); memcpy(&hw[i], &hv, 2); }
      }
      if (cudaMalloc(&plan->w_dev, hw.size() * 2) != cudaSuccess ||
          cudaMemcpy(plan->w_dev, hw.data(), hw.size() * 2, cudaMemcpyHostToDevice) != cudaSuccess) {
        set_error("tc plan: upload of the skip weights failed"); delete plan; return PCLS_ERR_CUDA;
      }
      q.skip = 1; q.skip_w = plan->w_dev;
    }
    if (q.res_tma) {
      char* r_base = (char*)tensor_ptr(L.res0, frames_per_pass);
      const uint64_t Co = (uint64_t)cp.res0_channels, Wo = (uint64_t)cp.Wout;
      if (q.c_is_5d) {
        const uint64_t gg = G > 1 ? (uint64_t)G : 2;
        const uint64_t dims[5] = {Co, gg, Wo / gg, Hh, F};
        const uint64_t str[4] = {Co * 2, Co * 2 * gg, Wo * Co * 2, Hh * Wo * Co * 2};
        const uint32_t box[5] = {(uint32_t)q.cbw, 1, (uint32_t)q.BW, (uint32_t)q.BH, 1};
        rc = make_map(&plan->map_r, bf16, r_base, 5, dims, str, box, 128);
      } else {
        const uint64_t dims[4] = {Co, Wo, Hh, F};
        const uint64_t str[3] = {Co * 2, Wo * Co * 2, Hh * Wo * Co * 2};
        const uint32_t box[4] = {(uint32_t)q.cbw, (uint32_t)q.BW, (uint32_t)q.BH, 1};
        rc = make_map(&plan->map_r, bf16, r_base, 4, dims, str, box, 128);
      }
      if (rc) { delete plan; return rc; }
    }
    L.tc = plan;
    L.tc_ok = true;
  return PCLS_OK;
}

int Net::tc_prepare() {
  const int max_smem = 227 * 1024;
  static bool attr_set_dev[64] = {false};
  int dev = 0;
  PCLS_CHECK_CUDA(cudaGetDevice(&dev));
  bool& attr_set = attr_set_dev[dev & 63];
  for (auto& L : convs) {
    bool retry = false;
    if (L.skip_into >= 0) continue;
    int rc = head_plan_layer(L);
    if (rc) return rc;
    if (L.hp) { L.tc_ok = true; continue; }
    rc = tc_plan_layer(L, true, &retry);
    if (rc == PCLS_OK && retry) rc = tc_plan_layer(L, false, &retry);
    if (rc) return rc;
  }
  if (!attr_set) {
    for (int kc = 16; kc <= 64; kc *= 2)
      for (int sub = 1; sub <= 3; sub += 2)
        for (int g = 1; g <= 4; g *= 2) {
          if ((g == 4 && kc != 64) || (g == 2 && kc == 16)) continue;
          for (int bf = 0; bf < 2; ++bf)
            for (int rs = 0; rs < 2; ++rs)
              for (int lk = 0; lk < 2; ++lk)
                PCLS_CHECK_CUDA(cudaFuncSetAttribute(tc_kernel_for(kc, sub, g, bf, rs, lk), cudaFuncAttributeMaxDynamicSharedMemorySize, max_smem));
        }
    for (int bf = 0; bf < 2; ++bf) {
      PCLS_CHECK_CUDA(cudaFuncSetAttribute(tc_kernel_for(64, 3, 1, bf, 0, 0, 3), cudaFuncAttributeMaxDynamicSharedMemorySize, max_smem));
      for (int g = 1; g <= 4; g *= 2)
        for (int lk = 0; lk < 2; ++lk)
          PCLS_CHECK_CUDA(cudaFuncSetAttribute(tc_kernel_for(64, 3, g, bf, 1, lk, 0, 1), cudaFuncAttributeMaxDynamicSharedMemorySize, max_smem));
      for (int kc = 16; kc <= 64; kc *= 2)
        for (int sub = 1; sub <= 3; sub += 2)
          for (int g = 1; g <= 4; g *= 2) {
            if ((g == 2 && kc < 32) || (g == 4 && kc < 64)) continue;
            for (int lk = 0; lk < 2; ++lk)
              PCLS_CHECK_CUDA(cudaFuncSetAttribute(tc_kernel_for(kc, sub, g, bf, 0, lk, 0, 2), cudaFuncAttributeMaxDynamicSharedMemorySize, max_smem));
          }
      PCLS_CHECK_CUDA(cudaFuncSetAttribute(tc_kernel_for(64, 3, 1, bf, 0, 0, 3, 2), cudaFuncAttributeMaxDynamicSharedMemorySize, max_smem));
      PCLS_CHECK_CUDA(cudaFuncSetAttribute(tc_kernel_for(64, 3, 4, bf, 1, 0, 0, 3), cudaFuncAttributeMaxDynamicSharedMemorySize, max_smem));
    }
    attr_set = true;
  }
  return PCLS_OK;
}

int Net::tc_launch(ConvLayer& L, const ConvParams& p, int nb, cudaStream_t s) {
  if (L.hp) return head_launch(L, p, nb, s);
  TcPlan* plan = L.tc;
  TcParams prm = plan->prm;
  prm.out = p.out; prm.res0 = p.res0; prm.res1 = p.res1;
  prm.dbg = tc_debug_buf;
  prm.pdl_early = pdl_early_now;
  prm.head = (prm.out_f32 && head_args.head) ? 1 : 0;
  prm.none_index = head_args.none_index; prm.mask = head_args.mask;
  prm.probs = head_args.probs; prm.preds = head_args.preds; prm.logits = head_args.logits;
  const int num_tiles = prm.num_tiles * nb;
  if (num_tiles == 0) return PCLS_OK;
  int work = num_tiles;
  if (prm.vstream) {
    int R = 1;
    for (int r = 32; r > 1; r /= 2)
      if (prm.Hgrid % r == 0 && (long long)nb * prm.n_wt * (prm.Hgrid / r) >= 6LL * sm_count()) { R = r; break; }
    prm.R = R; prm.n_hseg = prm.Hgrid / R;
    work = num_tiles / R;
  }
  int grid = work < sm_count() ? work : sm_count();
  if (prm.nsplit) grid -= grid % prm.n_nt;
  const int rtma = prm.skip ? 3 : (tc_rtma_mode && prm.res_tma && prm.res0 && !prm.res1 && prm.tma_store && !prm.out_f32 &&
                    (prm.act == PCLS_ACT_RELU || prm.act == PCLS_ACT_LEAKY) && !(PCLS_TC_VSTREAM && prm.vstream)) ? 1
                 : ((tc_rtma_mode & 2) && !prm.res0 && !prm.res1 && prm.tma_store && !prm.out_f32 && !(PCLS_TC_VSTREAM && prm.vstream)) ? 2 : 0;
  const bool res = prm.res0 || prm.res1 || prm.skip;
  PCLS_CHECK_CUDA(launch_pdl(tc_kernel_for(prm.KC, prm.sub, prm.G, prm.is_bf16, res ? 1 : 0, prm.act == PCLS_ACT_LEAKY ? 1 : 0, prm.ksteps, rtma),
                             dim3(grid), dim3(tc_threads(res)), plan->smem_bytes, s,
                             plan->map_a, plan->map_b, plan->map_c, plan->map_r, plan->map_b2, plan->map_c2, prm, num_tiles));
  return check_launch("conv_tc_kernel");
}

void Net::tc_release() {
  for (auto& L : convs) { delete L.tc; L.tc = nullptr; L.tc_ok = false; head_release(L); }
}

#endif

}
```

pclsegmentation_b200/csrc/net.cu:

```cuda
#include "net.cuh"

#include <algorithm>
#include <cmath>
#include <cstring>

namespace pcls {

int pad48_mode = 1;
int pair_s2_mode = 1;

static size_t align_up(size_t v, size_t a) { return (v + a - 1) / a * a; }

template <typename T>
static void pack_to(std::vector<uint16_t>& dst, const std::vector<float>& src) {
  dst.resize(src.size());
  for (size_t i = 0; i < src.size(); ++i) {
    if (sizeof(T) == 2 && std::is_same<T, __half>::value) {
      __half h = __float2half_rn(src[i]);
      memcpy(&dst[i], &h, 2);
    } else {
      __nv_bfloat16 h = __float2bfloat16_rn(src[i]);
      memcpy(&dst[i], &h, 2);
    }
  }
}

static void fold_bn(int cout, const float* b, const float* gamma, const float* beta, const float* mean,
                    const float* var, float eps, std::vector<double>& scale, std::vector<double>& bias) {
  scale.assign(cout, 1.0);
  bias.assign(cout, 0.0);
  for (int c = 0; c < cout; ++c) {
    const double b0 = b ? (double)b[c] : 0.0;
    if (gamma) {
      const double sc = (double)gamma[c] / std::sqrt((double)var[c] + (double)eps);
      scale[c] = sc;
      bias[c] = (b0 - (double)mean[c]) * sc + (double)beta[c];
    } else {
      bias[c] = b0;
    }
  }
}

int Net::add_tensor(int width, int channels, bool logits) {
  TensorInfo t;
  t.width = width;
  t.channels = channels;
  t.stride = channels;
  t.logits = logits;
  tensors.push_back(t);
  return (int)tensors.size() - 1;
}

size_t Net::tensor_frame_bytes(const TensorInfo& t) const {
  return (size_t)H * t.width * t.stride * (t.logits ? 4 : 2);
}

int Net::add_conv(const pcls_conv_desc& d) {
  PCLS_REQUIRE(!finalized, "pcls_net_conv: net already finalized");
  ConvLayer L;
  if (d.kind == PCLS_CONV) {
    if (d.kh == 1 && d.kw == 1 && d.stride_w == 1) L.p.mode = MODE_1x1;
    else if (d.kh == 3 && d.kw == 3 && d.stride_w == 1) L.p.mode = MODE_3x3_S1;
    else if (d.kh == 3 && d.kw == 3 && d.stride_w == 2) L.p.mode = MODE_3x3_S2;
    else PCLS_REQUIRE(false, "pcls_net_conv: unsupported Conv2D %dx%d stride_w %d", d.kh, d.kw, d.stride_w);
  } else if (d.kind == PCLS_DECONV_1x4_S2) {
    PCLS_REQUIRE(d.kh == 1 && d.kw == 4 && d.stride_w == 2, "pcls_net_conv: transposed conv must be [1,4] stride [1,2]");
    L.p.mode = MODE_DECONV;
  } else {
    PCLS_REQUIRE(false, "pcls_net_conv: unknown kind %d", d.kind);
  }
  PCLS_REQUIRE(d.in_tensor >= 0 && d.in_tensor < (int)tensors.size() && d.out_tensor > 0 &&
                   d.out_tensor < (int)tensors.size() && d.in_tensor != d.out_tensor,
               "pcls_net_conv: bad tensor ids in=%d out=%d", d.in_tensor, d.out_tensor);
  if (pad48_mode && !tensors[d.out_tensor].logits && tensors[d.out_tensor].channels == 48 && tensors[d.out_tensor].stride == 48 &&
      d.out_channel_offset == 0 && d.cout == 48 && d.residual0 < 0 && d.residual1 < 0 && d.kind == PCLS_CONV)
    tensors[d.out_tensor].stride = 64;
  const TensorInfo& ti = tensors[d.in_tensor];
  const TensorInfo& to = tensors[d.out_tensor];
  PCLS_REQUIRE(!ti.logits, "pcls_net_conv: cannot read a logits tensor");
  PCLS_REQUIRE(d.cin >= 1 && d.cin <= ti.channels && d.cout >= 1, "pcls_net_conv: cin %d exceeds input tensor channels %d",
               d.cin, ti.channels);
  PCLS_REQUIRE(d.out_channel_offset >= 0 && d.out_channel_offset + d.cout <= to.channels,
               "pcls_net_conv: output slice [%d,%d) exceeds tensor channels %d", d.out_channel_offset,
               d.out_channel_offset + d.cout, to.channels);
  PCLS_REQUIRE((d.out_is_logits != 0) == to.logits, "pcls_net_conv: out_is_logits does not match the output tensor");
  PCLS_REQUIRE(to.logits || d.out_channel_offset % 8 == 0, "pcls_net_conv: channel offset must be a multiple of 8");
  int wout = ti.width;
  if (L.p.mode == MODE_3x3_S2) wout = (ti.width + 1) / 2;
  if (L.p.mode == MODE_DECONV) wout = ti.width * 2;
  PCLS_REQUIRE(to.width == wout, "pcls_net_conv: output width %d, expected %d", to.width, wout);
  PCLS_REQUIRE(d.h_kernel != nullptr, "pcls_net_conv: kernel is NULL");
  const bool bn = d.h_bn_gamma != nullptr;
  PCLS_REQUIRE(!bn || (d.h_bn_beta && d.h_bn_mean && d.h_bn_var), "pcls_net_conv: incomplete BatchNorm parameters");
  PCLS_REQUIRE(d.act >= 0 && d.act <= 2, "pcls_net_conv: bad activation %d", d.act);
  const int res[2] = {d.residual0, d.residual1};
  for (int r = 0; r < 2; ++r) {
    if (res[r] < 0) continue;
    PCLS_REQUIRE(res[r] < (int)tensors.size() && !tensors[res[r]].logits && tensors[res[r]].width == to.width &&
                     d.out_channel_offset + d.cout <= tensors[res[r]].channels && res[r] != d.out_tensor,
                 "pcls_net_conv: residual tensor %d does not match the output", res[r]);
  }

  ConvParams& p = L.p;
  p.H = H; p.Win = ti.width; p.Wout = wout;
  const bool in_padded = ti.stride > ti.channels, out_padded = to.stride > to.channels;
  p.cin = d.cin; p.cin_pad = in_padded ? ti.stride : (d.cin + 15) / 16 * 16;
  p.in_channels = ti.stride;
  p.cout = out_padded ? to.stride : d.cout; p.cout_pad = (p.cout + 15) / 16 * 16;
  p.out_channels = to.stride; p.out_coff = d.out_channel_offset;
  L.cin_logical = d.cin; L.cout_logical = d.cout;
  p.act = d.act;
  p.ntaps = (p.mode == MODE_1x1) ? 1 : (p.mode == MODE_DECONV ? 4 : 9);
  p.pad_left = 0;
  if (p.mode == MODE_3x3_S2) {
    const int total = std::max((wout - 1) * 2 + 3 - ti.width, 0);
    p.pad_left = total / 2;
  }
  p.out_f32 = d.out_is_logits ? 1 : 0;
  p.res0_channels = d.residual0 >= 0 ? tensors[d.residual0].stride : 0;
  p.res1_channels = d.residual1 >= 0 ? tensors[d.residual1].stride : 0;
  L.in = d.in_tensor; L.out = d.out_tensor; L.res0 = d.residual0; L.res1 = d.residual1;

  std::vector<double> scale, bias;
  fold_bn(d.cout, d.h_bias, d.h_bn_gamma, d.h_bn_beta, d.h_bn_mean, d.h_bn_var, d.bn_eps, scale, bias);
  L.w_f32.assign((size_t)p.ntaps * p.cout_pad * p.cin_pad, 0.0f);
  for (int t = 0; t < p.ntaps; ++t)
    for (int co = 0; co < d.cout; ++co)
      for (int ci = 0; ci < d.cin; ++ci) {
        const size_t src = (d.kind == PCLS_CONV) ? ((size_t)t * d.cin + ci) * d.cout + co
                                                 : ((size_t)t * d.cout + co) * d.cin + ci;
        L.w_f32[((size_t)t * p.cout_pad + co) * p.cin_pad + ci] = (float)((double)d.h_kernel[src] * scale[co]);
      }
  L.bias_f32.assign(p.cout_pad, 0.0f);
  for (int co = 0; co < d.cout; ++co) L.bias_f32[co] = (float)bias[co];

  build_pair_view(L);
  convs.push_back(std::move(L));
  ops.push_back({OP_CONV, (int)convs.size() - 1});
  return PCLS_OK;
}

void Net::build_deconv_row3(ConvLayer& L) {
  const ConvParams& p = L.p;
  if (p.mode != MODE_DECONV || p.out_f32 || p.out_coff != 0 || p.cout != p.out_channels) return;
  if (2 * p.cout_pad > 256 || p.cout % 8 != 0) return;
  ConvParams q = p;
  q.mode = MODE_ROW3; q.ntaps = 3; q.Wout = p.Win;
  q.cout = 2 * p.cout; q.cout_pad = (q.cout + 15) / 16 * 16; q.out_channels = 2 * p.out_channels;
  q.res0_channels = 2 * p.res0_channels; q.res1_channels = 2 * p.res1_channels;
  auto wf = [&](int tap, int co, int ci) { return L.w_f32[((size_t)tap * p.cout_pad + co) * p.cin_pad + ci]; };
  L.w_tc.assign((size_t)3 * q.cout_pad * p.cin_pad, 0.0f);
  auto put = [&](int t, int half, int k) {
    for (int co = 0; co < p.cout; ++co)
      for (int ci = 0; ci < p.cin; ++ci)
        L.w_tc[((size_t)t * q.cout_pad + half * p.cout + co) * p.cin_pad + ci] = wf(k, co, ci);
  };
  put(0, 0, 3); put(1, 0, 1); put(1, 1, 2); put(2, 1, 0);
  L.bias_tc.assign(q.cout_pad, 0.0f);
  for (int n = 0; n < q.cout; ++n) L.bias_tc[n] = L.bias_f32[n % p.cout];
  L.ptc = q;
  L.pair_view = true;
}

void Net::build_pair_view(ConvLayer& L) {
  const ConvParams& p = L.p;
  if (p.mode == MODE_DECONV) { build_deconv_row3(L); return; }
  if (L.in != 0 && pair_s2_mode && p.mode == MODE_3x3_S2 && p.pad_left == 0 && p.Win % 2 == 0 && !p.out_f32 && L.res0 < 0 &&
      L.res1 < 0 && p.cin == p.cin_pad && p.in_channels == p.cin_pad && p.cin_pad == 32 && p.Wout == p.Win / 2) {
    ConvParams q = p;
    const int cp2 = 2 * p.cin_pad;
    q.Win = p.Win / 2; q.in_channels = cp2; q.cin = cp2; q.cin_pad = cp2; q.pad_left = 0;
    q.mode = MODE_3x3_S1; q.ntaps = 9;
    L.w_tc.assign((size_t)9 * q.cout_pad * cp2, 0.0f);
    for (int dh = 0; dh < 3; ++dh)
      for (int kx = 0; kx < 3; ++kx)
        for (int co = 0; co < p.cout; ++co)
          for (int ci = 0; ci < p.cin; ++ci)
            L.w_tc[((size_t)(dh * 3 + 1 + (kx >> 1)) * q.cout_pad + co) * cp2 + (kx & 1) * p.cin_pad + ci] =
                L.w_f32[((size_t)(dh * 3 + kx) * p.cout_pad + co) * p.cin_pad + ci];
    L.bias_tc = L.bias_f32;
    L.ptc = q;
    L.pair_view = true;
    return;
  }
  if (L.in != 0 || W % 2 != 0 || p.out_f32 || L.res0 >= 0 || L.res1 >= 0) return;
  if (p.mode == MODE_3x3_S2 && p.pad_left != 0) return;
  if (p.mode == MODE_DECONV) return;
  const bool doubled = p.mode != MODE_3x3_S2;
  if (doubled && (p.out_coff != 0 || p.cout != p.out_channels)) return;
  ConvParams q = p;
  q.Win = W / 2; q.Wout = W / 2; q.in_channels = 16; q.cin = 16; q.cin_pad = 16; q.pad_left = 0;
  const int co_n = p.cout;
  if (doubled) { q.cout = 2 * co_n; q.out_channels = 2 * p.out_channels; }
  q.cout_pad = (q.cout + 15) / 16 * 16;
  if (q.cout_pad > 256) return;
  auto wf = [&](int tap, int co, int ci) { return L.w_f32[((size_t)tap * p.cout_pad + co) * p.cin_pad + ci]; };
  if (p.mode == MODE_1x1) {
    q.mode = MODE_1x1; q.ntaps = 1;
    L.w_tc.assign((size_t)q.cout_pad * 16, 0.0f);
    for (int px = 0; px < 2; ++px)
      for (int co = 0; co < co_n; ++co)
        for (int ci = 0; ci < p.cin; ++ci) L.w_tc[(size_t)(px * co_n + co) * 16 + px * 8 + ci] = wf(0, co, ci);
  } else if (p.mode == MODE_3x3_S1) {
    q.mode = MODE_3x3_S1; q.ntaps = 9;
    L.w_tc.assign((size_t)9 * q.cout_pad * 16, 0.0f);
    for (int dh = 0; dh < 3; ++dh)
      for (int dw = -1; dw <= 1; ++dw)
        for (int px = 0; px < 2; ++px)
          for (int par = 0; par < 2; ++par) {
            const int kx = 2 * dw + par - px + 1;
            if (kx < 0 || kx > 2) continue;
            for (int co = 0; co < co_n; ++co)
              for (int ci = 0; ci < p.cin; ++ci)
                L.w_tc[((size_t)(dh * 3 + dw + 1) * q.cout_pad + px * co_n + co) * 16 + par * 8 + ci] = wf(dh * 3 + kx, co, ci);
          }
  } else {
    q.mode = MODE_3x3_S1; q.ntaps = 9;
    L.w_tc.assign((size_t)9 * q.cout_pad * 16, 0.0f);
    for (int dh = 0; dh < 3; ++dh)
      for (int kx = 0; kx < 3; ++kx)
        for (int co = 0; co < co_n; ++co)
          for (int ci = 0; ci < p.cin; ++ci)
            L.w_tc[((size_t)(dh * 3 + 1 + (kx >> 1)) * q.cout_pad + co) * 16 + (kx & 1) * 8 + ci] = wf(dh * 3 + kx, co, ci);
  }
  L.bias_tc.assign(q.cout_pad, 0.0f);
  for (int n = 0; n < q.cout; ++n) L.bias_tc[n] = L.bias_f32[n % co_n];
  L.ptc = q;
  L.pair_view = true;
}

int Net::add_pool(int in, int out) {
  PCLS_REQUIRE(!finalized, "pcls_net_maxpool3x3_s2: net already finalized");
  PCLS_REQUIRE(in >= 0 && in < (int)tensors.size() && out > 0 && out < (int)tensors.size() && in != out,
               "pcls_net_maxpool3x3_s2: bad tensor ids");
  const TensorInfo &ti = tensors[in], &to = tensors[out];
  PCLS_REQUIRE(!ti.logits && !to.logits && ti.channels == to.channels && to.width == (ti.width + 1) / 2,
               "pcls_net_maxpool3x3_s2: shape mismatch");
  tensors[out].stride = tensors[in].stride;
  PoolLayer L;
  L.in = in; L.out = out;
  L.pad_left = std::max((to.width - 1) * 2 + 3 - ti.width, 0) / 2;
  pools.push_back(L);
  ops.push_back({OP_POOL, (int)pools.size() - 1});
  return PCLS_OK;
}

int Net::add_cam(const pcls_cam_desc& d) {
  PCLS_REQUIRE(!finalized, "pcls_net_cam: net already finalized");
  PCLS_REQUIRE(d.in_tensor >= 0 && d.in_tensor < (int)tensors.size() && d.out_tensor > 0 &&
                   d.out_tensor < (int)tensors.size() && d.in_tensor != d.out_tensor,
               "pcls_net_cam: bad tensor ids");
  const TensorInfo &ti = tensors[d.in_tensor], &to = tensors[d.out_tensor];
  PCLS_REQUIRE(ti.channels == d.channels && to.channels == d.channels && ti.width == to.width && !ti.logits && !to.logits,
               "pcls_net_cam: shape mismatch");
  PCLS_REQUIRE((d.channels == 64 || d.channels == 128) && d.reduced == d.channels / 16,
               "pcls_net_cam: supported channels 64/128 with reduction 16 (got %d -> %d)", d.channels, d.reduced);
  PCLS_REQUIRE(d.h_sq_kernel && d.h_ex_kernel, "pcls_net_cam: kernels must not be NULL");
  CamLayer L;
  L.in = d.in_tensor; L.out = d.out_tensor; L.C = d.channels; L.R = d.reduced;
  std::vector<double> s1, bb1, s2, bb2;
  fold_bn(L.R, d.h_sq_bias, d.h_sq_gamma, d.h_sq_beta, d.h_sq_mean, d.h_sq_var, d.bn_eps, s1, bb1);
  fold_bn(L.C, d.h_ex_bias, d.h_ex_gamma, d.h_ex_beta, d.h_ex_mean, d.h_ex_var, d.bn_eps, s2, bb2);
  L.h.resize((size_t)2 * L.C * L.R + L.R + L.C);
  float* w1 = L.h.data();
  float* w2 = w1 + L.C * L.R;
  float* b1 = w2 + L.R * L.C;
  float* b2 = b1 + L.R;
  for (int c = 0; c < L.C; ++c)
    for (int j = 0; j < L.R; ++j) w1[c * L.R + j] = (float)((double)d.h_sq_kernel[c * L.R + j] * s1[j]);
  for (int j = 0; j < L.R; ++j)
    for (int c = 0; c < L.C; ++c) w2[j * L.C + c] = (float)((double)d.h_ex_kernel[j * L.C + c] * s2[c]);
  for (int j = 0; j < L.R; ++j) b1[j] = (float)bb1[j];
  for (int c = 0; c < L.C; ++c) b2[c] = (float)bb2[c];
  cams.push_back(std::move(L));
  ops.push_back({OP_CAM, (int)cams.size() - 1});
  return PCLS_OK;
}

void Net::op_tensors(const OpRef& op, std::vector<int>& reads, std::vector<int>& writes) const {
  reads.clear(); writes.clear();
  if (op.type == OP_CONV) {
    const ConvLayer& L = convs[op.index];
    if (L.skip_into >= 0) return;
    reads.push_back(L.in);
    if (L.pool_src >= 0) reads.push_back(L.pool_src);
    if (L.up_squeeze >= 0) reads.push_back(convs[L.up_squeeze].in);
    if (L.skip_src >= 0) reads.push_back(convs[L.skip_src].in);
    else if (L.res0 >= 0) reads.push_back(L.res0);
    if (L.res1 >= 0) reads.push_back(L.res1);
    writes.push_back(L.out);
  } else if (op.type == OP_POOL) {
    reads.push_back(pools[op.index].in); writes.push_back(pools[op.index].out);
  } else {
    reads.push_back(cams[op.index].in); writes.push_back(cams[op.index].out);
  }
}

int Net::finalize(int logits_tensor_, int num_classes_, int none_index_) {
  PCLS_REQUIRE(!finalized, "pcls_net_finalize: already finalized");
  PCLS_REQUIRE(logits_tensor_ > 0 && logits_tensor_ < (int)tensors.size() && tensors[logits_tensor_].logits,
               "pcls_net_finalize: logits tensor id %d is not a logits tensor", logits_tensor_);
  PCLS_REQUIRE(num_classes_ >= 1 && num_classes_ <= 32 && tensors[logits_tensor_].channels == num_classes_ &&
                   tensors[logits_tensor_].width == W,
               "pcls_net_finalize: logits tensor must be [B,H,W,num_classes] with num_classes <= 32");
  PCLS_REQUIRE(none_index_ >= 0 && none_index_ < num_classes_, "pcls_net_finalize: none_index out of range");
  logits_tensor = logits_tensor_; num_classes = num_classes_; none_index = none_index_;

  const int n_ops = (int)ops.size();
  if (fuse_pool)
    for (int i = 0; i + 1 < n_ops; ++i) {
      if (ops[i].type != OP_POOL || ops[i + 1].type != OP_CONV) continue;
      PoolLayer& P = pools[ops[i].index];
      ConvLayer& L = convs[ops[i + 1].index];
      const ConvParams& cp = L.p;
      if (L.in != P.out || cp.mode != MODE_1x1 || L.res0 >= 0 || L.res1 >= 0 || cp.out_f32 || cp.out_coff != 0) continue;
      if (tensors[P.in].stride != tensors[P.in].channels || cp.cin_pad != tensors[P.in].channels) continue;
      if (!pool_conv1x1_supported(tensors[P.in].channels, (L.cout_logical + 15) / 16 * 16) || cp.cout != cp.cout_pad) continue;
      bool other_reader = false;
      std::vector<int> rd, wr;
      for (int k = 0; k < n_ops; ++k) {
        if (k == i + 1) continue;
        op_tensors(ops[k], rd, wr);
        for (int r : rd) other_reader = other_reader || r == P.out;
      }
      if (other_reader) continue;
      P.fused_conv = ops[i + 1].index;
      L.pool_src = P.in; L.pool_pad_left = P.pad_left;
    }
  if (fuse_up && !keep_tensors)
    for (int i = 0; i + 1 < n_ops; ++i) {
      if (ops[i].type != OP_CONV || ops[i + 1].type != OP_CONV) continue;
      ConvLayer& Q = convs[ops[i].index];
      ConvLayer& U = convs[ops[i + 1].index];
      const ConvParams &q = Q.p, &u = U.p;
      if (q.mode != MODE_1x1 || u.mode != MODE_DECONV || U.in != Q.out || Q.pool_src >= 0) continue;
      if (Q.res0 >= 0 || Q.res1 >= 0 || U.res0 >= 0 || U.res1 >= 0 || q.out_f32 || u.out_f32 || q.out_coff != 0 || u.out_coff != 0) continue;
      const int C = q.cin_pad, S = q.cout;
      if (tensors[Q.in].stride != C || tensors[Q.in].channels != C || Q.cin_logical != C) continue;
      if (q.cout != q.cout_pad || q.out_channels != S || Q.cout_logical != S) continue;
      if (u.cin_pad != S || u.cout != S || u.cout_pad != S || u.out_channels != S || U.cin_logical != S) continue;
      if (!squeeze_upconv_supported(C, S)) continue;
      bool other_reader = false;
      std::vector<int> rd, wr;
      for (int k = 0; k < n_ops; ++k) {
        if (k == i + 1) continue;
        op_tensors(ops[k], rd, wr);
        for (int r : rd) other_reader = other_reader || r == Q.out;
      }
      if (other_reader || Q.out == logits_tensor) continue;
      U.up_squeeze = ops[i].index;
      Q.fused_into_up = ops[i + 1].index;
    }
  if (fuse_skip && !keep_tensors && conv_impl == 0)
    for (int i = 0; i < n_ops; ++i) {
      if (ops[i].type != OP_CONV) continue;
      ConvLayer& P = convs[ops[i].index];
      if (P.in != 0 || P.out == logits_tensor || P.fused_into_up >= 0) continue;
      int reader = -1, n_use = 0;
      std::vector<int> rd, wr;
      for (int k = 0; k < n_ops; ++k) {
        if (k == i) continue;
        op_tensors(ops[k], rd, wr);
        for (int r : rd) if (r == P.out) { ++n_use; reader = k; }
        for (int w : wr) if (w == P.out) n_use += 2;
      }
      if (n_use != 1 || ops[reader].type != OP_CONV) continue;
      ConvLayer& E = convs[ops[reader].index];
      if (E.pool_src >= 0 || E.up_squeeze >= 0 || !tc_skip_fusable(P, E)) continue;
      E.skip_src = ops[i].index;
      P.skip_into = ops[reader].index;
    }
  std::vector<int> reads, writes;
  for (auto& t : tensors) { t.first = -1; t.last = -1; }
  tensors[0].first = -1; tensors[0].last = -1;
  for (int i = 0; i < n_ops; ++i) {
    op_tensors(ops[i], reads, writes);
    for (int r : reads) {
      PCLS_REQUIRE(r == 0 || tensors[r].first >= 0, "pcls_net_finalize: op %d reads tensor %d before it is written", i, r);
      tensors[r].last = std::max(tensors[r].last, i);
    }
    for (int w : writes) {
      if (tensors[w].first < 0) tensors[w].first = i;
      tensors[w].last = std::max(tensors[w].last, i);
    }
  }
  tensors[logits_tensor].last = n_ops;
  if (keep_tensors)
    for (auto& t : tensors) t.last = n_ops;

  struct Block { size_t off, size; };
  std::vector<Block> free_list;
  size_t top = 0;
  auto alloc = [&](size_t size) -> size_t {
    size = align_up(size, 1024);
    for (size_t i = 0; i < free_list.size(); ++i) {
      if (free_list[i].size >= size) {
        size_t off = free_list[i].off;
        free_list[i].off += size; free_list[i].size -= size;
        if (free_list[i].size == 0) free_list.erase(free_list.begin() + i);
        return off;
      }
    }
    size_t off = top; top += size; return off;
  };
  auto release = [&](size_t off, size_t size) {
    size = align_up(size, 1024);
    free_list.push_back({off, size});
    std::sort(free_list.begin(), free_list.end(), [](const Block& a, const Block& b) { return a.off < b.off; });
    for (size_t i = 0; i + 1 < free_list.size();) {
      if (free_list[i].off + free_list[i].size == free_list[i + 1].off) {
        free_list[i].size += free_list[i + 1].size; free_list.erase(free_list.begin() + i + 1);
      } else ++i;
    }
    if (!free_list.empty() && free_list.back().off + free_list.back().size == top) { top = free_list.back().off; free_list.pop_back(); }
  };
  tensors[0].offset = alloc(tensor_frame_bytes(tensors[0]));
  mask_offset = alloc((size_t)H * W);
  size_t peak = top;
  for (int i = 0; i < n_ops; ++i) {
    op_tensors(ops[i], reads, writes);
    for (int w : writes)
      if (tensors[w].first == i) { tensors[w].offset = alloc(tensor_frame_bytes(tensors[w])); peak = std::max(peak, top); }
    for (size_t t = 0; t < tensors.size(); ++t)
      if (tensors[t].last == i && (int)t != logits_tensor && !(t == 0 && tensors[0].last < 0))
        release(tensors[t].offset, tensor_frame_bytes(tensors[t]));
  }
  frame_bytes = align_up(peak, 1024);
  for (size_t t = 0; t < tensors.size(); ++t) {
    bool fused_skip = false;
    for (const auto& L : convs) fused_skip = fused_skip || (L.skip_into >= 0 && L.out == (int)t);
    PCLS_REQUIRE(t == 0 || tensors[t].first >= 0 || fused_skip, "pcls_net_finalize: tensor %d is never written", (int)t);
  }

  frames_per_pass = (micro_batch > 0 && micro_batch < max_batch) ? micro_batch : max_batch;
  PCLS_CHECK_CUDA(cudaMalloc(&arena, frame_bytes * (size_t)frames_per_pass));
  arena_bytes = frame_bytes * (size_t)frames_per_pass;

  size_t wbytes = 0;
  for (auto& L : convs) {
    wbytes += align_up(L.w_f32.size() * 2, 256) + align_up(L.bias_f32.size() * 4, 256);
    if (L.pair_view) wbytes += align_up(L.w_tc.size() * 2, 256) + align_up(L.bias_tc.size() * 4, 256);
  }
  for (auto& L : cams) wbytes += align_up(L.h.size() * 4, 256);
  PCLS_CHECK_CUDA(cudaMalloc(&weights, std::max<size_t>(wbytes, 256)));
  weight_bytes = wbytes;
  size_t off = 0;
  std::vector<uint16_t> packed;
  for (auto& L : convs) {
    if (precision == PCLS_F16) pack_to<__half>(packed, L.w_f32); else pack_to<__nv_bfloat16>(packed, L.w_f32);
    PCLS_CHECK_CUDA(cudaMemcpy((char*)weights + off, packed.data(), packed.size() * 2, cudaMemcpyHostToDevice));
    L.p.w = (char*)weights + off; off += align_up(packed.size() * 2, 256);
    PCLS_CHECK_CUDA(cudaMemcpy((char*)weights + off, L.bias_f32.data(), L.bias_f32.size() * 4, cudaMemcpyHostToDevice));
    L.p.bias = (const float*)((char*)weights + off); off += align_up(L.bias_f32.size() * 4, 256);
    if (L.pair_view) {
      if (precision == PCLS_F16) pack_to<__half>(packed, L.w_tc); else pack_to<__nv_bfloat16>(packed, L.w_tc);
      PCLS_CHECK_CUDA(cudaMemcpy((char*)weights + off, packed.data(), packed.size() * 2, cudaMemcpyHostToDevice));
      L.ptc.w = (char*)weights + off; off += align_up(packed.size() * 2, 256);
      PCLS_CHECK_CUDA(cudaMemcpy((char*)weights + off, L.bias_tc.data(), L.bias_tc.size() * 4, cudaMemcpyHostToDevice));
      L.ptc.bias = (const float*)((char*)weights + off); off += align_up(L.bias_tc.size() * 4, 256);
    }
  }
  for (auto& L : cams) {
    PCLS_CHECK_CUDA(cudaMemcpy((char*)weights + off, L.h.data(), L.h.size() * 4, cudaMemcpyHostToDevice));
    const float* base = (const float*)((char*)weights + off);
    L.p.C = L.C; L.p.R = L.R;
    L.p.w1 = base; L.p.w2 = base + L.C * L.R; L.p.b1 = L.p.w2 + L.R * L.C; L.p.b2 = L.p.b1 + L.R;
    off += align_up(L.h.size() * 4, 256);
  }
  int rc = tc_prepare();
  if (rc != PCLS_OK) return rc;
  finalized = true;
  return PCLS_OK;
}

void* Net::tensor_ptr(int t, int frames) const {
  (void)frames;
  return (char*)arena + tensors[t].offset * (size_t)frames_per_pass;
}

template <typename T>
int Net::run_pass(const float* lidar, int channels, const uint8_t* mask, bool raw, const double* mean5,
                  const double* std5, int nb, float* logits, float* probs, int32_t* preds, cudaStream_t s,
                  cudaEvent_t* ev) {
  const int64_t n_pixels = (int64_t)nb * H * W;
  pdl_early_now = (pdl_mode && n_pixels <= pdl_early_px) ? 1 : 0;
  uint8_t* mask_buf = (uint8_t*)arena + mask_offset * (size_t)frames_per_pass;
  int evi = 0;
  if (ev) cudaEventRecord(ev[evi++], s);
  int rc = PCLS_OK;
  if (lidar != nullptr) {
    if (channels & kIn16) rc = launch_net_input16(lidar, channels & ~kIn16, mask, n_pixels, tensor_ptr(0, nb), mask_buf, s);
    else rc = launch_net_input<T>(lidar, channels, mask, raw, mean5, std5, n_pixels, (T*)tensor_ptr(0, nb), mask_buf, s);
  }
  if (rc) return rc;
  float* logits_buf = logits ? logits : (float*)tensor_ptr(logits_tensor, nb);
  bool head_done = false;
  for (const OpRef& op : ops) {
    if (ev) cudaEventRecord(ev[evi++], s);
    if (op.type == OP_CONV) {
      ConvLayer& L = convs[op.index];
      ConvParams p = L.p;
      p.in = tensor_ptr(L.in, nb);
      p.out = (L.out == logits_tensor) ? (void*)logits_buf : tensor_ptr(L.out, nb);
      p.res0 = (L.res0 >= 0 && L.skip_src < 0) ? tensor_ptr(L.res0, nb) : nullptr;
      p.res1 = L.res1 >= 0 ? tensor_ptr(L.res1, nb) : nullptr;
      if (conv_impl == 0 && L.fused_into_up >= 0) continue;
      if (L.skip_into >= 0) continue;
      if (conv_impl == 0 && L.up_squeeze >= 0) {
        const ConvLayer& Q = convs[L.up_squeeze];
        SqueezeUpconvParams su;
        su.in = tensor_ptr(Q.in, nb); su.out = p.out;
        su.w1 = Q.p.w; su.b1 = Q.p.bias; su.w1_stride = Q.p.cin_pad; su.act1 = Q.p.act;
        su.w2 = p.w; su.b2 = p.bias; su.w2_cout_pad = p.cout_pad; su.w2_cin_pad = p.cin_pad; su.act2 = p.act;
        su.H = H; su.W = p.Win; su.rows = 0; su.tiles_per_row = 0;
        rc = launch_squeeze_upconv<T>(su, Q.p.cin_pad, Q.p.cout, nb, s);
      } else if (conv_impl == 0 && L.pool_src >= 0) {
        PoolConvParams pc;
        pc.in = tensor_ptr(L.pool_src, nb); pc.out = p.out; pc.w = p.w; pc.bias = p.bias;
        pc.H = H; pc.Win = tensors[L.pool_src].width; pc.Wout = p.Wout; pc.out_channels = p.out_channels;
        pc.w_stride = p.cin_pad; pc.pad_left = L.pool_pad_left; pc.act = p.act; pc.n_strips = 0; pc.tiles_per_row = 0;
        const int S_real = (L.cout_logical + 15) / 16 * 16;
        pc.zero_to = S_real < p.cout ? p.cout : 0;
        rc = launch_pool_conv1x1<T>(pc, tensors[L.pool_src].channels, S_real, nb, s);
      } else if (conv_impl == 0 && L.tc_ok) {
        const bool fuse = L.out == logits_tensor && head_is_fused();
        head_args.head = fuse ? 1 : 0;
        head_args.none_index = none_index; head_args.mask = mask_buf;
        head_args.probs = probs; head_args.preds = preds; head_args.logits = logits;
        head_done = head_done || fuse;
        if (L.pair_view) {
          ConvParams pv = L.ptc;
          pv.in = p.in; pv.out = p.out; pv.res0 = p.res0; pv.res1 = p.res1;
          rc = tc_launch(L, pv, nb, s);
        } else {
          rc = tc_launch(L, p, nb, s);
        }
      }
      else rc = launch_conv_direct<T>(p, nb, s);
    } else if (op.type == OP_POOL) {
      const PoolLayer& L = pools[op.index];
      if (conv_impl == 0 && L.fused_conv >= 0) continue;
      rc = launch_maxpool3x3_s2<T>((const T*)tensor_ptr(L.in, nb), (T*)tensor_ptr(L.out, nb), nb, H, tensors[L.in].width,
                                   tensors[L.out].width, tensors[L.in].stride, L.pad_left, s);
    } else {
      const CamLayer& L = cams[op.index];
      rc = launch_cam<T>((const T*)tensor_ptr(L.in, nb), (T*)tensor_ptr(L.out, nb), L.p, nb, H, tensors[L.in].width, cam_px, s);
    }
    if (rc) return rc;
    if (tc_debug_buf && ev && op.type == OP_CONV) {
      cudaStreamSynchronize(s);
      std::vector<unsigned long long> h(148 * 24);
      cudaMemcpy(h.data(), tc_debug_buf, h.size() * 8, cudaMemcpyDeviceToHost);
      cudaMemset(tc_debug_buf, 0, h.size() * 8);
      double a[24] = {0};
      for (int c = 0; c < 148; ++c) for (int i = 0; i < 24; ++i) a[i] += (double)h[c * 24 + i] / 148.0;
      const ConvParams& cp = convs[op.index].p;
      fprintf(stderr, "[tc_debug] conv mode %d %dx%d w%d | cycles/CTA: total %.0f | producer wait-empty %.0f | issuer wait-tempty %.0f wait-full %.0f | "
              "epi(g0) wait-tfull %.0f store-drain %.0f barrier %.0f busy %.0f tiles %.0f | epi(g1) wait-tfull %.0f busy %.0f tiles %.0f\n",
              cp.mode, cp.cin, cp.cout, cp.Wout, a[8], a[0], a[1], a[2], a[3], a[4], a[5], a[6], a[7], a[11], a[14], a[15]);
    }
  }
  if (ev) cudaEventRecord(ev[evi++], s);
  rc = head_done ? PCLS_OK : launch_head(logits_buf, mask_buf, n_pixels, num_classes, none_index, probs, preds, s);
  if (ev) cudaEventRecord(ev[evi++], s);
  return rc;
}

int Net::run_all(const float* lidar, int channels, const uint8_t* mask, bool raw, const double* mean5,
                 const double* std5, int B, float* logits, float* probs, int32_t* preds, cudaStream_t s,
                 cudaEvent_t* ev) {
  const size_t px = (size_t)H * W;
  for (int b0 = 0; b0 < B; b0 += frames_per_pass) {
    const int nb = std::min(frames_per_pass, B - b0);
    const float* l = (channels & kIn16)
        ? (const float*)((const uint16_t*)lidar + (size_t)b0 * px * (channels & ~kIn16))
        : lidar + (size_t)b0 * px * channels;
    const uint8_t* m = mask ? mask + (size_t)b0 * px : nullptr;
    float* lg = logits ? logits + (size_t)b0 * px * num_classes : nullptr;
    float* pr = probs ? probs + (size_t)b0 * px * num_classes : nullptr;
    int32_t* pd = preds + (size_t)b0 * px;
    int rc = (precision == PCLS_F16) ? run_pass<__half>(l, channels, m, raw, mean5, std5, nb, lg, pr, pd, s, ev)
                                     : run_pass<__nv_bfloat16>(l, channels, m, raw, mean5, std5, nb, lg, pr, pd, s, ev);
    if (rc) return rc;
  }
  return PCLS_OK;
}

static int check_forward_args(const Net& n, const float* lidar, int channels, const double* mean5, const double* std5,
                              int B, const int32_t* preds) {
  PCLS_REQUIRE(n.finalized, "pcls_net_forward: call pcls_net_finalize first");
  PCLS_REQUIRE(B >= 0 && B <= n.max_batch, "pcls_net_forward: batch %d exceeds max_batch %d", B, n.max_batch);
  const bool raw = mean5 != nullptr;
  if (lidar == nullptr && channels == 0) {
    PCLS_REQUIRE(B <= n.frames_per_pass, "pcls_net_forward: a staged input must fit one pass (%d frames)", n.frames_per_pass);
    PCLS_REQUIRE(B == 0 || preds != nullptr, "pcls_net_forward: preds must not be NULL");
    return PCLS_OK;
  }
  if (channels & kIn16) {
    PCLS_REQUIRE(!raw && ((channels & ~kIn16) == 6 || (channels & ~kIn16) == 8),
                 "pcls_net_forward_in16: channels must be 6 or 8 (normalised 16-bit input), got %d", channels & ~kIn16);
    PCLS_REQUIRE(B == 0 || (lidar != nullptr && preds != nullptr), "pcls_net_forward_in16: lidar/preds must not be NULL");
    return PCLS_OK;
  }
  PCLS_REQUIRE(raw ? (channels == 5 || channels == 6) : channels == 6,
               "pcls_net_forward: channels must be 6 (normalised input) or 5/6 with mean/std (raw input), got %d", channels);
  PCLS_REQUIRE(!raw || std5 != nullptr, "pcls_net_forward: std is NULL");
  PCLS_REQUIRE(B == 0 || (lidar != nullptr && preds != nullptr), "pcls_net_forward: lidar/preds must not be NULL");
  return PCLS_OK;
}

int Net::forward(const float* lidar, int channels, const uint8_t* mask, const double* mean5, const double* std5, int B,
                 float* logits, float* probs, int32_t* preds, cudaStream_t s) {
  int rc = check_forward_args(*this, lidar, channels, mean5, std5, B, preds);
  if (rc) return rc;
  last_B = B;
  if (B == 0) return PCLS_OK;
  const bool raw = mean5 != nullptr;
  if (!use_graph) return run_all(lidar, channels, mask, raw, mean5, std5, B, logits, probs, preds, s, nullptr);

  GraphKey key;
  memset(&key, 0, sizeof(key));
  key.lidar = lidar; key.mask = mask; key.logits = logits; key.probs = probs; key.preds = preds;
  key.channels = channels; key.B = B; key.raw = raw ? 1 : 0; key.conv_impl = conv_impl;
  for (int c = 0; c < 5; ++c) { key.norm[c] = raw ? mean5[c] : 0.0; key.norm[5 + c] = raw ? std5[c] : 0.0; }
  for (auto& g : graphs) {
    if (!memcmp(&g.key, &key, sizeof(key))) {
      g.stamp = ++graph_clock;
      graph_misses = 0;
      PCLS_CHECK_CUDA(cudaGraphLaunch(g.exec, s));
      return PCLS_OK;
    }
  }
  if (++graph_misses > 4) return run_all(lidar, channels, mask, raw, mean5, std5, B, logits, probs, preds, s, nullptr);
  if (!cap_stream) PCLS_CHECK_CUDA(cudaStreamCreateWithFlags(&cap_stream, cudaStreamNonBlocking));
  PCLS_CHECK_CUDA(cudaStreamBeginCapture(cap_stream, cudaStreamCaptureModeRelaxed));
  rc = run_all(lidar, channels, mask, raw, mean5, std5, B, logits, probs, preds, cap_stream, nullptr);
  cudaGraph_t graph = nullptr;
  cudaError_t e = cudaStreamEndCapture(cap_stream, &graph);
  if (rc) { if (graph) cudaGraphDestroy(graph); return rc; }
  if (e != cudaSuccess) { set_error("cudaStreamEndCapture failed: %s", cudaGetErrorString(e)); return PCLS_ERR_CUDA; }
  CachedGraph cg;
  cg.key = key;
  e = cudaGraphInstantiate(&cg.exec, graph, 0);
  cudaGraphDestroy(graph);
  if (e != cudaSuccess) { set_error("cudaGraphInstantiate failed: %s", cudaGetErrorString(e)); return PCLS_ERR_CUDA; }
  cg.stamp = ++graph_clock;
  if (graphs.size() >= 16) {
    size_t victim = 0;
    for (size_t i = 1; i < graphs.size(); ++i) if (graphs[i].stamp < graphs[victim].stamp) victim = i;
    cudaGraphExecDestroy(graphs[victim].exec);
    graphs.erase(graphs.begin() + victim);
  }
  graphs.push_back(cg);
  PCLS_CHECK_CUDA(cudaGraphLaunch(cg.exec, s));
  return PCLS_OK;
}

void Net::drop_graphs() {
  for (auto& g : graphs) cudaGraphExecDestroy(g.exec);
  graphs.clear();
}

int Net::profile_ops(const float* lidar, int channels, const uint8_t* mask, const double* mean5, const double* std5,
                     int B, float* logits, float* probs, int32_t* preds, float* h_ms, cudaStream_t s) {
  int rc = check_forward_args(*this, lidar, channels, mean5, std5, B, preds);
  if (rc) return rc;
  PCLS_REQUIRE(B >= 1 && B <= frames_per_pass, "pcls_net_profile_ops: B must fit one pass (<= %d)", frames_per_pass);
  PCLS_REQUIRE(h_ms != nullptr, "pcls_net_profile_ops: h_ms is NULL");
  const int n = (int)ops.size() + 2;
  std::vector<cudaEvent_t> ev(n + 1);
  for (auto& e : ev) PCLS_CHECK_CUDA(cudaEventCreate(&e));
  rc = run_all(lidar, channels, mask, mean5 != nullptr, mean5, std5, B, logits, probs, preds, s, ev.data());
  if (rc == PCLS_OK) {
    cudaError_t e = cudaStreamSynchronize(s);
    if (e != cudaSuccess) { set_error("profile: %s", cudaGetErrorString(e)); rc = PCLS_ERR_CUDA; }
  }
  if (rc == PCLS_OK)
    for (int i = 0; i < n; ++i) cudaEventElapsedTime(&h_ms[i], ev[i], ev[i + 1]);
  for (auto& e : ev) cudaEventDestroy(e);
  return rc;
}

bool Net::head_is_fused() const {
  if (!fuse_head || conv_impl != 0) return false;
  for (const auto& L : convs)
    if (L.out == logits_tensor) return L.tc_ok && (W % 128 == 0 || L.hp != nullptr);
  return false;
}

int Net::op_info(int i, char* name, int* family, int64_t* flops, int64_t* bytes) const {
  const int n = (int)ops.size() + 2;
  PCLS_REQUIRE(i >= 0 && i < n, "pcls_net_op_info: op index %d out of range", i);
  const int64_t HW = (int64_t)H * W;
  int fam = 0;
  int64_t fl = 0, by = 0;
  char buf[64];
  if (i == 0) {
    snprintf(buf, sizeof(buf), "input_stage");
    by = HW * (5 * 4 + 16 + 1);
  } else if (i == n - 1) {
    snprintf(buf, sizeof(buf), head_is_fused() ? "head_softmax_argmax(fused)" : "head_softmax_argmax");
    by = head_is_fused() ? 0 : HW * ((int64_t)num_classes * 4 * 2 + 4 + 1);
  } else {
    const OpRef& op = ops[i - 1];
    if (op.type == OP_CONV) {
      const ConvLayer& L = convs[op.index];
      const ConvParams& p = L.p;
      const char* mode = p.mode == MODE_1x1 ? "conv1x1" : p.mode == MODE_3x3_S1 ? "conv3x3" : p.mode == MODE_3x3_S2 ? "conv3x3s2" : "deconv1x4s2";
      const int64_t cin = L.cin_logical, cout = L.cout_logical;
      snprintf(buf, sizeof(buf), "%s_%dx%d_w%d", mode, (int)cin, (int)cout, p.Wout);
      const int64_t taps = p.mode == MODE_DECONV ? 2 : p.ntaps;
      fl = 2 * (int64_t)H * p.Wout * cin * cout * taps;
      by = (int64_t)H * p.Win * cin * 2 + (int64_t)H * p.Wout * cout * (p.out_f32 ? 4 : 2) +
           (int64_t)p.ntaps * cin * cout * 2;
      if (L.out == logits_tensor && head_is_fused()) by += (int64_t)H * p.Wout * (4 + 1);
      if (conv_impl == 0 && L.pool_src >= 0) {
        by += (int64_t)H * (tensors[L.pool_src].width - p.Win) * cin * 2;
        snprintf(buf, sizeof(buf), "pool+%s_%dx%d_w%d", mode, (int)cin, (int)cout, p.Wout);
      }
      if (L.skip_src >= 0) {
        const ConvLayer& P = convs[L.skip_src];
        by += (int64_t)H * W * tensors[P.in].stride * 2 + (int64_t)P.cin_logical * P.cout_logical * 2;
        fl += 2 * (int64_t)H * W * P.cin_logical * P.cout_logical;
      } else if (L.res0 >= 0) {
        by += (int64_t)H * p.Wout * cout * 2;
      }
      if (L.res1 >= 0) by += (int64_t)H * p.Wout * cout * 2;
      fam = (conv_impl == 0 && L.tc_ok) ? 1 : 0;
      if (L.skip_into >= 0) {
        snprintf(buf, sizeof(buf), "%s_%dx%d_w%d(fused)", mode, (int)cin, (int)cout, p.Wout);
        fl = 0; by = 0; fam = 0;
      }
      if (conv_impl == 0 && L.fused_into_up >= 0) {
        snprintf(buf, sizeof(buf), "%s_%dx%d_w%d(fused)", mode, (int)cin, (int)cout, p.Wout);
        fl = 0; by = 0; fam = 0;
      }
      if (conv_impl == 0 && L.up_squeeze >= 0) {
        const ConvLayer& Q = convs[L.up_squeeze];
        snprintf(buf, sizeof(buf), "conv1x1_%dx%d+%s_w%d", Q.cin_logical, Q.cout_logical, mode, p.Wout);
        fl += 2 * (int64_t)H * p.Win * Q.cin_logical * Q.cout_logical;
        by = (int64_t)H * p.Win * Q.cin_logical * 2 + (int64_t)H * p.Wout * cout * 2 +
             ((int64_t)Q.cin_logical * Q.cout_logical + (int64_t)p.ntaps * cin * cout) * 2;
        fam = 0;
      }
    } else if (op.type == OP_POOL) {
      const PoolLayer& L = pools[op.index];
      const bool fused = conv_impl == 0 && L.fused_conv >= 0;
      snprintf(buf, sizeof(buf), fused ? "maxpool3x3s2_c%d_w%d(fused)" : "maxpool3x3s2_c%d_w%d", tensors[L.in].channels, tensors[L.out].width);
      by = fused ? 0 : (int64_t)H * (tensors[L.in].width + tensors[L.out].width) * tensors[L.in].channels * 2;
    } else {
      const CamLayer& L = cams[op.index];
      snprintf(buf, sizeof(buf), "cam_c%d_w%d", L.C, tensors[L.in].width);
      fl = 2 * (int64_t)H * tensors[L.in].width * L.C * L.R * 2;
      by = (int64_t)H * tensors[L.in].width * L.C * 2 * 2;
    }
  }
  if (name) { strncpy(name, buf, 63); name[63] = 0; }
  if (family) *family = fam;
  if (flops) *flops = fl;
  if (bytes) *bytes = by;
  return PCLS_OK;
}

int Net::read_tensor(int t, int B, float* out, cudaStream_t s) {
  PCLS_REQUIRE(finalized && t >= 0 && t < (int)tensors.size(), "pcls_net_read_tensor: bad tensor id %d", t);
  PCLS_REQUIRE(B >= 0 && B <= frames_per_pass, "pcls_net_read_tensor: B exceeds the frames of one pass");
  PCLS_REQUIRE(t == 0 || tensors[t].first >= 0, "pcls_net_read_tensor: tensor %d is computed inside the conv that reads it "
               "(set keep_tensors or fuse_skip = 0 before finalize)", t);
  const TensorInfo& ti = tensors[t];
  const int64_t n = (int64_t)B * H * ti.width * ti.channels;
  if (ti.logits) { PCLS_CHECK_CUDA(cudaMemcpyAsync(out, tensor_ptr(t, B), n * 4, cudaMemcpyDeviceToDevice, s)); return PCLS_OK; }
  return precision == PCLS_F16 ? launch_tensor_to_f32<__half>((const __half*)tensor_ptr(t, B), out, n, ti.channels, ti.stride, s)
                               : launch_tensor_to_f32<__nv_bfloat16>((const __nv_bfloat16*)tensor_ptr(t, B), out, n, ti.channels, ti.stride, s);
}

Net::~Net() {
  drop_graphs();
  if (cap_stream) cudaStreamDestroy(cap_stream);
  if (arena) cudaFree(arena);
  if (weights) cudaFree(weights);
  tc_release();
}

}

using namespace pcls;

extern "C" int pcls_net_create(pcls_net** out, int H, int W, int precision, int max_batch) {
  PCLS_REQUIRE(out != nullptr, "pcls_net_create: out is NULL");
  PCLS_REQUIRE(H > 0 && W > 0 && max_batch > 0, "pcls_net_create: bad shape H=%d W=%d max_batch=%d", H, W, max_batch);
  PCLS_REQUIRE(precision == PCLS_F16 || precision == PCLS_BF16, "pcls_net_create: bad precision %d", precision);
  int ndev = 0;
  if (cudaGetDeviceCount(&ndev) != cudaSuccess || ndev == 0) {
    set_error("pcls_net_create: no CUDA device (libpclseg has no CPU fallback)");
    return PCLS_ERR_CUDA;
  }
  Net* n = new Net();
  n->H = H; n->W = W; n->precision = precision; n->max_batch = max_batch;
  n->add_tensor(W, 8, false);
  *out = reinterpret_cast<pcls_net*>(n);
  return PCLS_OK;
}

extern "C" void pcls_net_destroy(pcls_net* net) { delete reinterpret_cast<Net*>(net); }

extern "C" int pcls_net_tensor(pcls_net* net, int width, int channels, int is_logits) {
  Net* n = reinterpret_cast<Net*>(net);
  PCLS_REQUIRE(n != nullptr && !n->finalized, "pcls_net_tensor: bad or finalized net");
  PCLS_REQUIRE(width > 0 && channels > 0 && (is_logits || channels % 8 == 0),
               "pcls_net_tensor: width %d channels %d (activation channels must be a multiple of 8)", width, channels);
  return n->add_tensor(width, channels, is_logits != 0);
}

extern "C" int pcls_net_conv(pcls_net* net, const pcls_conv_desc* desc) {
  PCLS_REQUIRE(net != nullptr && desc != nullptr, "pcls_net_conv: NULL argument");
  return reinterpret_cast<Net*>(net)->add_conv(*desc);
}

extern "C" int pcls_net_maxpool3x3_s2(pcls_net* net, int in_tensor, int out_tensor) {
  PCLS_REQUIRE(net != nullptr, "pcls_net_maxpool3x3_s2: NULL net");
  return reinterpret_cast<Net*>(net)->add_pool(in_tensor, out_tensor);
}

extern "C" int pcls_net_cam(pcls_net* net, const pcls_cam_desc* desc) {
  PCLS_REQUIRE(net != nullptr && desc != nullptr, "pcls_net_cam: NULL argument");
  return reinterpret_cast<Net*>(net)->add_cam(*desc);
}

extern "C" int pcls_net_finalize(pcls_net* net, int logits_tensor, int num_classes, int none_index) {
  PCLS_REQUIRE(net != nullptr, "pcls_net_finalize: NULL net");
  return reinterpret_cast<Net*>(net)->finalize(logits_tensor, num_classes, none_index);
}

extern "C" int pcls_net_forward(pcls_net* net, const float* lidar, int channels, const uint8_t* mask,
                                const double* h_mean5, const double* h_std5, int B, float* logits, float* probs,
                                int32_t* preds, pcls_stream stream) {
  PCLS_REQUIRE(net != nullptr, "pcls_net_forward: NULL net");
  return reinterpret_cast<Net*>(net)->forward(lidar, channels, mask, h_mean5, h_std5, B, logits, probs, preds,
                                              (cudaStream_t)stream);
}

extern "C" int pcls_net_forward_in16(pcls_net* net, const void* lidar16, int channels, const uint8_t* mask, int B,
                                     float* logits, float* probs, int32_t* preds, pcls_stream stream) {
  PCLS_REQUIRE(net != nullptr, "pcls_net_forward_in16: NULL net");
  PCLS_REQUIRE(channels == 6 || channels == 8, "pcls_net_forward_in16: channels must be 6 or 8, got %d", channels);
  PCLS_REQUIRE(B == 0 || lidar16 != nullptr, "pcls_net_forward_in16: lidar16 is NULL");
  return reinterpret_cast<Net*>(net)->forward((const float*)lidar16, channels | kIn16, mask, nullptr, nullptr, B, logits,
                                              probs, preds, (cudaStream_t)stream);
}

extern "C" int pcls_net_input_buffers(pcls_net* net, void** input8, uint8_t** mask, int* frames) {
  Net* n = reinterpret_cast<Net*>(net);
  PCLS_REQUIRE(n != nullptr && n->finalized, "pcls_net_input_buffers: net is NULL or not finalized");
  if (input8) *input8 = n->tensor_ptr(0, n->frames_per_pass);
  if (mask) *mask = (uint8_t*)n->arena + n->mask_offset * (size_t)n->frames_per_pass;
  if (frames) *frames = n->frames_per_pass;
  return PCLS_OK;
}

extern "C" int pcls_net_read_tensor(pcls_net* net, int tensor, int B, float* out, pcls_stream stream) {
  PCLS_REQUIRE(net != nullptr && out != nullptr, "pcls_net_read_tensor: NULL argument");
  return reinterpret_cast<Net*>(net)->read_tensor(tensor, B, out, (cudaStream_t)stream);
}

extern "C" int pcls_net_num_ops(const pcls_net* net) {
  const Net* n = reinterpret_cast<const Net*>(net);
  return n ? (int)n->ops.size() + 2 : 0;
}

extern "C" int pcls_net_profile_ops(pcls_net* net, const float* lidar, int channels, const uint8_t* mask,
                                    const double* h_mean5, const double* h_std5, int B, float* logits, float* probs,
                                    int32_t* preds, float* h_ms, pcls_stream stream) {
  PCLS_REQUIRE(net != nullptr, "pcls_net_profile_ops: NULL net");
  return reinterpret_cast<Net*>(net)->profile_ops(lidar, channels, mask, h_mean5, h_std5, B, logits, probs, preds, h_ms,
                                                  (cudaStream_t)stream);
}

extern "C" int pcls_net_op_info(const pcls_net* net, int i, char* h_name, int* family, int64_t* flops_per_frame,
                                int64_t* bytes_per_frame) {
  PCLS_REQUIRE(net != nullptr, "pcls_net_op_info: NULL net");
  return reinterpret_cast<const Net*>(net)->op_info(i, h_name, family, flops_per_frame, bytes_per_frame);
}

extern "C" int pcls_net_launches_per_forward(const pcls_net* net) {
  const Net* n = reinterpret_cast<const Net*>(net);
  if (!n) return 0;
  int launches = 1;
  for (const OpRef& op : n->ops) {
    if (op.type == OP_CONV && n->conv_impl == 0 && n->convs[op.index].fused_into_up >= 0) continue;
    if (op.type == OP_CONV && n->convs[op.index].skip_into >= 0) continue;
    if (op.type == OP_POOL && n->conv_impl == 0 && n->pools[op.index].fused_conv >= 0) continue;
    ++launches;
  }
  return launches + (n->head_is_fused() ? 0 : 1);
}

extern "C" int64_t pcls_net_workspace_bytes(const pcls_net* net) {
  const Net* n = reinterpret_cast<const Net*>(net);
  return n ? (int64_t)(n->arena_bytes + n->weight_bytes) : 0;
}

extern "C" int pcls_net_set_option(pcls_net* net, const char* name, int value) {
  Net* n = reinterpret_cast<Net*>(net);
  PCLS_REQUIRE(n != nullptr && name != nullptr, "pcls_net_set_option: NULL argument");
  if (!strcmp(name, "conv_impl")) {
    PCLS_REQUIRE(value == 0 || value == 1, "conv_impl must be 0 or 1");
    bool skip_fused = false;
    for (const auto& L : n->convs) skip_fused = skip_fused || L.skip_into >= 0;
    PCLS_REQUIRE(value == 0 || !skip_fused, "conv_impl = 1 needs a net finalized with fuse_skip = 0 (or conv_impl = 1 set before)");
    n->conv_impl = value; return PCLS_OK;
  }
  if (!strcmp(name, "use_graph")) { n->use_graph = value != 0; if (!n->use_graph) n->drop_graphs(); return PCLS_OK; }
  if (!strcmp(name, "micro_batch")) {
    PCLS_REQUIRE(!n->finalized, "micro_batch must be set before pcls_net_finalize");
    PCLS_REQUIRE(value >= 0, "micro_batch must be >= 0");
    n->micro_batch = value; return PCLS_OK;
  }
  if (!strcmp(name, "keep_tensors")) {
    PCLS_REQUIRE(!n->finalized, "keep_tensors must be set before pcls_net_finalize");
    n->keep_tensors = value != 0; return PCLS_OK;
  }
  if (!strcmp(name, "tc_head")) { tc_head_mode = value; return PCLS_OK; }
  if (!strcmp(name, "cam_px")) { PCLS_REQUIRE(value >= 0 && value <= 2, "cam_px must be 0 (default), 1 or 2"); n->cam_px = value; n->drop_graphs(); return PCLS_OK; }
  if (!strcmp(name, "tc_nsplit")) { tc_nsplit_mode = value; return PCLS_OK; }
  if (!strcmp(name, "pad48")) {
    PCLS_REQUIRE(n->convs.empty(), "pad48 must be set before the first pcls_net_conv");
    pad48_mode = value; return PCLS_OK;
  }
  if (!strcmp(name, "pair_s2")) {
    PCLS_REQUIRE(n->convs.empty(), "pair_s2 must be set before the first pcls_net_conv");
    pair_s2_mode = value; return PCLS_OK;
  }
  if (!strcmp(name, "tc_halo")) { tc_halo_mode = value; return PCLS_OK; }
  if (!strcmp(name, "tc_rtma")) { tc_rtma_mode = value; n->drop_graphs(); return PCLS_OK; }
  if (!strcmp(name, "tc_tma_store")) { tc_tma_store_mode = value; return PCLS_OK; }
  if (!strcmp(name, "tc_group")) { tc_group_mode = value; return PCLS_OK; }
  if (!strcmp(name, "tc_res_tma")) { tc_res_tma_mode = value; return PCLS_OK; }
  if (!strcmp(name, "tc_split")) { tc_split_mode = value; return PCLS_OK; }
  if (!strcmp(name, "tc_vstream")) { tc_vstream_mode = value; return PCLS_OK; }
  if (!strcmp(name, "fuse_up")) {
    PCLS_REQUIRE(!n->finalized, "fuse_up must be set before pcls_net_finalize");
    n->fuse_up = value != 0; return PCLS_OK;
  }
  if (!strcmp(name, "fuse_pool")) {
    PCLS_REQUIRE(!n->finalized, "fuse_pool must be set before pcls_net_finalize");
    n->fuse_pool = value != 0; return PCLS_OK;
  }
  if (!strcmp(name, "fuse_skip")) {
    PCLS_REQUIRE(!n->finalized, "fuse_skip must be set before pcls_net_finalize");
    n->fuse_skip = value != 0; return PCLS_OK;
  }
  if (!strcmp(name, "fuse_head")) { n->fuse_head = value != 0; n->drop_graphs(); return PCLS_OK; }
  if (!strcmp(name, "tc_debug")) {
    PCLS_REQUIRE(!value || tc_debug_compiled, "tc_debug needs a library built with PCLS_NVCC_FLAGS=-DPCLS_TC_DEBUG=1");
    if (value && !tc_debug_buf) { PCLS_CHECK_CUDA(cudaMalloc(&tc_debug_buf, 148 * 24 * 8)); PCLS_CHECK_CUDA(cudaMemset(tc_debug_buf, 0, 148 * 24 * 8)); }
    if (!value && tc_debug_buf) { cudaFree(tc_debug_buf); tc_debug_buf = nullptr; }
    return PCLS_OK;
  }
  if (!strcmp(name, "tc_resident")) { tc_resident_mode = value; return PCLS_OK; }
  if (!strcmp(name, "tc_base_offset")) { tc_base_offset_mode = value; return PCLS_OK; }
  set_error("pcls_net_set_option: unknown option '%s'", name);
  return PCLS_ERR_INVALID;
}
```

pclsegmentation_b200/csrc/net.cuh:

```cuda
#pragma once
#include <vector>

#include "nn_kernels.cuh"

namespace pcls {

struct TensorInfo {
  int width = 0, channels = 0;
  int stride = 0;
  bool logits = false;
  int first = -1, last = -1;
  size_t offset = 0;
};

struct TcPlan;
struct HeadPlan;
extern int tc_head_mode;
extern int tc_rtma_mode, tc_halo_mode, tc_resident_mode, tc_base_offset_mode, tc_tma_store_mode, tc_group_mode, tc_res_tma_mode, tc_split_mode, tc_vstream_mode, tc_nsplit_mode;
extern int pad48_mode;
extern const int tc_debug_compiled;
extern unsigned long long* tc_debug_buf;

struct ConvLayer {
  ConvParams p;
  int cin_logical = 0, cout_logical = 0;
  int in = -1, out = -1, res0 = -1, res1 = -1;
  std::vector<float> w_f32;
  std::vector<float> bias_f32;
  bool tc_ok = false;
  TcPlan* tc = nullptr;
  HeadPlan* hp = nullptr;
  int pool_src = -1, pool_pad_left = 0;
  int up_squeeze = -1;
  int fused_into_up = -1;
  int skip_src = -1;
  int skip_into = -1;
  bool pair_view = false;
  ConvParams ptc;
  std::vector<float> w_tc, bias_tc;
  void* w_tc_dev = nullptr;
  float* bias_tc_dev = nullptr;
};

struct PoolLayer { int in, out, pad_left; int fused_conv = -1;  };

struct CamLayer {
  int in, out, C, R;
  std::vector<float> h;
  CamParams p;
};

enum OpType { OP_CONV = 0, OP_POOL = 1, OP_CAM = 2 };
struct OpRef { int type, index; };

constexpr int kIn16 = 0x100;

struct GraphKey {
  const void *lidar, *mask, *logits, *probs, *preds;
  int channels, B, raw, conv_impl;
  double norm[10];
};
struct CachedGraph { GraphKey key; cudaGraphExec_t exec = nullptr; uint64_t stamp = 0; };

struct Net {
  int H = 0, W = 0, precision = PCLS_F16, max_batch = 0;
  std::vector<TensorInfo> tensors;
  std::vector<ConvLayer> convs;
  std::vector<PoolLayer> pools;
  std::vector<CamLayer> cams;
  std::vector<OpRef> ops;
  bool finalized = false;
  int logits_tensor = -1, num_classes = 0, none_index = 0;
  int conv_impl = 0;
  bool use_graph = true;
  bool fuse_up = true;
  bool fuse_pool = true;
  bool fuse_head = true;
  bool fuse_skip = true;
  struct HeadArgs { int head = 0, none_index = 0; const uint8_t* mask = nullptr; float* probs = nullptr; int32_t* preds = nullptr; float* logits = nullptr; } head_args;
  int micro_batch = 0;
  int cam_px = 0;
  bool keep_tensors = false;
  int frames_per_pass = 0;
  size_t frame_bytes = 0, mask_offset = 0;
  void* arena = nullptr;
  size_t arena_bytes = 0;
  void* weights = nullptr;
  size_t weight_bytes = 0;
  int last_B = 0;
  std::vector<CachedGraph> graphs;
  uint64_t graph_clock = 0;
  int graph_misses = 0;
  cudaStream_t cap_stream = nullptr;

  ~Net();
  int add_tensor(int width, int channels, bool logits);
  size_t tensor_frame_bytes(const TensorInfo& t) const;
  int add_conv(const pcls_conv_desc& d);
  void build_pair_view(ConvLayer& L);
  void build_deconv_row3(ConvLayer& L);
  int add_pool(int in, int out);
  int add_cam(const pcls_cam_desc& d);
  void op_tensors(const OpRef& op, std::vector<int>& reads, std::vector<int>& writes) const;
  int finalize(int logits_tensor, int num_classes, int none_index);
  void* tensor_ptr(int t, int frames) const;
  template <typename T>
  int run_pass(const float* lidar, int channels, const uint8_t* mask, bool raw, const double* mean5, const double* std5,
               int nb, float* logits, float* probs, int32_t* preds, cudaStream_t s, cudaEvent_t* ev);
  int run_all(const float* lidar, int channels, const uint8_t* mask, bool raw, const double* mean5, const double* std5,
              int B, float* logits, float* probs, int32_t* preds, cudaStream_t s, cudaEvent_t* ev);
  void drop_graphs();
  int profile_ops(const float* lidar, int channels, const uint8_t* mask, const double* mean5, const double* std5, int B,
                  float* logits, float* probs, int32_t* preds, float* h_ms, cudaStream_t s);
  bool head_is_fused() const;
  int op_info(int i, char* name, int* family, int64_t* flops, int64_t* bytes) const;
  int forward(const float* lidar, int channels, const uint8_t* mask, const double* mean5, const double* std5, int B,
              float* logits, float* probs, int32_t* preds, cudaStream_t s);
  int read_tensor(int t, int B, float* out, cudaStream_t s);

  int tc_prepare();
  int tc_plan_layer(ConvLayer& L, bool allow_group, bool* retry);
  bool tc_skip_fusable(const ConvLayer& P, const ConvLayer& E) const;
  int tc_launch(ConvLayer& L, const ConvParams& p, int nb, cudaStream_t s);
  void tc_release();
  int head_plan_layer(ConvLayer& L);
  int head_launch(ConvLayer& L, const ConvParams& p, int nb, cudaStream_t s);
  void head_release(ConvLayer& L);
};

}
```

pclsegmentation_b200/csrc/squeeze_upconv.cu:

```cuda
#include "nn_kernels.cuh"

namespace pcls {

template <typename T> __device__ __forceinline__ void mma16816_su(float (&d)[4], const uint32_t (&a)[4], const uint32_t (&b)[2]);
template <> __device__ __forceinline__ void mma16816_su<__half>(float (&d)[4], const uint32_t (&a)[4], const uint32_t (&b)[2]) {
  asm volatile("mma.sync.aligned.m16n8k16.row.col.f32.f16.f16.f32 {%0,%1,%2,%3}, {%4,%5,%6,%7}, {%8,%9}, {%0,%1,%2,%3};"
               : "+f"(d[0]), "+f"(d[1]), "+f"(d[2]), "+f"(d[3])
               : "r"(a[0]), "r"(a[1]), "r"(a[2]), "r"(a[3]), "r"(b[0]), "r"(b[1]));
}
template <> __device__ __forceinline__ void mma16816_su<__nv_bfloat16>(float (&d)[4], const uint32_t (&a)[4], const uint32_t (&b)[2]) {
  asm volatile("mma.sync.aligned.m16n8k16.row.col.f32.bf16.bf16.f32 {%0,%1,%2,%3}, {%4,%5,%6,%7}, {%8,%9}, {%0,%1,%2,%3};"
               : "+f"(d[0]), "+f"(d[1]), "+f"(d[2]), "+f"(d[3])
               : "r"(a[0]), "r"(a[1]), "r"(a[2]), "r"(a[3]), "r"(b[0]), "r"(b[1]));
}
__device__ __forceinline__ void ldmatrix_x4(uint32_t (&r)[4], uint32_t addr) {
  asm volatile("ldmatrix.sync.aligned.m8n8.x4.shared.b16 {%0,%1,%2,%3}, [%4];"
               : "=r"(r[0]), "=r"(r[1]), "=r"(r[2]), "=r"(r[3]) : "r"(addr) : "memory");
}
template <typename T> __device__ __forceinline__ uint32_t pack2_su(float lo, float hi) {
  T h[2] = {from_f32<T>(lo), from_f32<T>(hi)};
  return *reinterpret_cast<uint32_t*>(h);
}
__device__ __forceinline__ float act_su(float v, int act) {
  return act == PCLS_ACT_RELU ? fmaxf(v, 0.0f) : (act == PCLS_ACT_LEAKY ? fmaxf(v, 0.1f * v) : v);
}

constexpr int SU_WARPS = 8;
constexpr int SU_TP = 14;

template <int C, int S> struct SuGeom {
  static constexpr int SLABS = C / 64, NT = S / 8, KS2 = S / 16;
  static constexpr int NLD = 4 * SLABS;
  static constexpr int W1_FRAGS = SLABS * 4 * NT;
  static constexpr int W2_FRAGS = 4 * KS2 * NT;
  static constexpr int QP = S * 2 + 16;
  static constexpr int OP = S * 4 + 16;
  static constexpr int WARP_BYTES = 16 * QP + 16 * OP;
  static constexpr int SMEM = (W1_FRAGS + W2_FRAGS) * 32 * 8 + SU_WARPS * WARP_BYTES;
};

template <typename T, int C, int S>
__global__ void __launch_bounds__(SU_WARPS * 32, (C <= 64 ? 3 : (C <= 128 ? 2 : 1)))
squeeze_upconv_kernel(const SqueezeUpconvParams p) {
  using G = SuGeom<C, S>;
  constexpr int SLABS = G::SLABS, NT = G::NT, KS2 = G::KS2, NLD = G::NLD, QP = G::QP, OP = G::OP;
  constexpr int CV = C / 8;
  extern __shared__ int4 su_smem[];
  uint2* const w1s = reinterpret_cast<uint2*>(su_smem);
  uint2* const w2s = w1s + G::W1_FRAGS * 32;
  const int warp = threadIdx.x >> 5, lane = threadIdx.x & 31, g = lane >> 2, t = lane & 3;
  unsigned char* const wbase = reinterpret_cast<unsigned char*>(w2s + G::W2_FRAGS * 32) + warp * G::WARP_BYTES;
  unsigned char* const sq = wbase;
  unsigned char* const st = wbase + 16 * QP;

  {
    const T* w1 = reinterpret_cast<const T*>(p.w1);
    for (int i = threadIdx.x; i < G::W1_FRAGS * 32; i += SU_WARPS * 32) {
      const int ln = i & 31, f = i >> 5, j = f % NT, s = (f / NT) % 4, sl = f / (NT * 4);
      w1s[i] = *reinterpret_cast<const uint2*>(w1 + (size_t)(8 * j + (ln >> 2)) * p.w1_stride + 64 * sl + 16 * (ln & 3) + 4 * s);
    }
    const T* w2 = reinterpret_cast<const T*>(p.w2);
    for (int i = threadIdx.x; i < G::W2_FRAGS * 32; i += SU_WARPS * 32) {
      const int ln = i & 31, f = i >> 5, j = f % NT, s2 = (f / NT) % KS2, k = f / (NT * KS2);
      const T* row = w2 + ((size_t)k * p.w2_cout_pad + 8 * j + (ln >> 2)) * p.w2_cin_pad + 16 * s2 + 2 * (ln & 3);
      w2s[i] = make_uint2(*reinterpret_cast<const uint32_t*>(row), *reinterpret_cast<const uint32_t*>(row + 8));
    }
    __syncthreads();
  }
  float b1r[NT][2], b2r[NT][2];
#pragma unroll
  for (int j = 0; j < NT; ++j) {
    b1r[j][0] = p.b1[8 * j + 2 * t]; b1r[j][1] = p.b1[8 * j + 2 * t + 1];
    b2r[j][0] = p.b2[8 * j + 2 * t]; b2r[j][1] = p.b2[8 * j + 2 * t + 1];
  }
  uint32_t a_addr[3];
  {
    const int r = (lane & 7) + 8 * ((lane >> 3) & 1);
#pragma unroll
    for (int d = 0; d < 3; ++d) {
      const int rr = min(max(r + d - 1, 0), 15);
      a_addr[d] = (uint32_t)__cvta_generic_to_shared(sq) + rr * QP + 16 * (lane >> 4);
    }
  }

  pdl_trigger(p.pdl_early);
  pdl_wait();
  const long long total = (long long)p.rows * p.tiles_per_row;
  const long long wstep = (long long)gridDim.x * SU_WARPS;
  const int4* const in = reinterpret_cast<const int4*>(p.in);
  T* const out = reinterpret_cast<T*>(p.out);
  int4 nx[NLD];
  auto load = [&](long long wt, int4 (&v)[NLD]) {
    const long long row = wt / p.tiles_per_row;
    const int p0 = (int)(wt % p.tiles_per_row) * SU_TP - 1;
    const int4* base = in + row * (long long)p.W * CV + 2 * t;
#pragma unroll
    for (int px = 0; px < 2; ++px) {
      const int4* src = base + (long long)min(max(p0 + g + 8 * px, 0), p.W - 1) * CV;
#pragma unroll
      for (int sl = 0; sl < SLABS; ++sl) {
        v[(px * SLABS + sl) * 2] = __ldg(src + sl * 8);
        v[(px * SLABS + sl) * 2 + 1] = __ldg(src + sl * 8 + 1);
      }
    }
  };
  long long wt = (long long)blockIdx.x * SU_WARPS + warp;
  if (wt < total) load(wt, nx);
  for (; wt < total; wt += wstep) {
    int4 cur[NLD];
#pragma unroll
    for (int i = 0; i < NLD; ++i) cur[i] = nx[i];
    if (wt + wstep < total) load(wt + wstep, nx);
    const long long row = wt / p.tiles_per_row;
    const int q = (int)(wt % p.tiles_per_row), p0 = q * SU_TP - 1;

    float acc[NT][4];
#pragma unroll
    for (int j = 0; j < NT; ++j) { acc[j][0] = 0.0f; acc[j][1] = 0.0f; acc[j][2] = 0.0f; acc[j][3] = 0.0f; }
#pragma unroll
    for (int sl = 0; sl < SLABS; ++sl) {
      const int4 &a0 = cur[sl * 2], &a1 = cur[sl * 2 + 1], &c0 = cur[(SLABS + sl) * 2], &c1 = cur[(SLABS + sl) * 2 + 1];
      const uint32_t aw[2][8] = {{(uint32_t)a0.x, (uint32_t)a0.y, (uint32_t)a0.z, (uint32_t)a0.w, (uint32_t)a1.x, (uint32_t)a1.y, (uint32_t)a1.z, (uint32_t)a1.w},
                                 {(uint32_t)c0.x, (uint32_t)c0.y, (uint32_t)c0.z, (uint32_t)c0.w, (uint32_t)c1.x, (uint32_t)c1.y, (uint32_t)c1.z, (uint32_t)c1.w}};
#pragma unroll
      for (int s = 0; s < 4; ++s) {
        const uint32_t a[4] = {aw[0][2 * s], aw[1][2 * s], aw[0][2 * s + 1], aw[1][2 * s + 1]};
#pragma unroll
        for (int j = 0; j < NT; ++j) {
          const uint2 bw = w1s[((sl * 4 + s) * NT + j) * 32 + lane];
          const uint32_t bfr[2] = {bw.x, bw.y};
          mma16816_su<T>(acc[j], a, bfr);
        }
      }
    }
    __syncwarp();
    {
      const bool v0 = p0 + g >= 0 && p0 + g < p.W, v1 = p0 + g + 8 >= 0 && p0 + g + 8 < p.W;
#pragma unroll
      for (int j = 0; j < NT; ++j) {
        const uint32_t lo = v0 ? pack2_su<T>(act_su(acc[j][0] + b1r[j][0], p.act1), act_su(acc[j][1] + b1r[j][1], p.act1)) : 0u;
        const uint32_t hi = v1 ? pack2_su<T>(act_su(acc[j][2] + b1r[j][0], p.act1), act_su(acc[j][3] + b1r[j][1], p.act1)) : 0u;
        *reinterpret_cast<uint32_t*>(sq + g * QP + (8 * j + 2 * t) * 2) = lo;
        *reinterpret_cast<uint32_t*>(sq + (g + 8) * QP + (8 * j + 2 * t) * 2) = hi;
      }
    }
    __syncwarp();

    float ev[NT][4], od[NT][4];
#pragma unroll
    for (int j = 0; j < NT; ++j)
#pragma unroll
      for (int i = 0; i < 4; ++i) { ev[j][i] = 0.0f; od[j][i] = 0.0f; }
#pragma unroll
    for (int s2 = 0; s2 < KS2; ++s2) {
      uint32_t al[4], ac[4], ar[4];
      ldmatrix_x4(al, a_addr[0] + 32 * s2);
      ldmatrix_x4(ac, a_addr[1] + 32 * s2);
      ldmatrix_x4(ar, a_addr[2] + 32 * s2);
#pragma unroll
      for (int j = 0; j < NT; ++j) {
        auto frag = [&](int k, uint32_t (&b)[2]) { const uint2 w = w2s[((k * KS2 + s2) * NT + j) * 32 + lane]; b[0] = w.x; b[1] = w.y; };
        uint32_t b[2];
        frag(1, b); mma16816_su<T>(ev[j], ac, b);
        frag(3, b); mma16816_su<T>(ev[j], al, b);
        frag(2, b); mma16816_su<T>(od[j], ac, b);
        frag(0, b); mma16816_su<T>(od[j], ar, b);
      }
    }
#pragma unroll
    for (int j = 0; j < NT; ++j) {
      unsigned char* d0 = st + g * OP + (8 * j + 2 * t) * 2;
      unsigned char* d1 = st + (g + 8) * OP + (8 * j + 2 * t) * 2;
      *reinterpret_cast<uint32_t*>(d0) = pack2_su<T>(act_su(ev[j][0] + b2r[j][0], p.act2), act_su(ev[j][1] + b2r[j][1], p.act2));
      *reinterpret_cast<uint32_t*>(d1) = pack2_su<T>(act_su(ev[j][2] + b2r[j][0], p.act2), act_su(ev[j][3] + b2r[j][1], p.act2));
      *reinterpret_cast<uint32_t*>(d0 + S * 2) = pack2_su<T>(act_su(od[j][0] + b2r[j][0], p.act2), act_su(od[j][1] + b2r[j][1], p.act2));
      *reinterpret_cast<uint32_t*>(d1 + S * 2) = pack2_su<T>(act_su(od[j][2] + b2r[j][0], p.act2), act_su(od[j][3] + b2r[j][1], p.act2));
    }
    __syncwarp();
    {
      constexpr int CPR = S * 4 / 16;
      const int n_out = min(SU_TP, p.W - q * SU_TP);
      int4* dst = reinterpret_cast<int4*>(out + ((row * p.W + (long long)q * SU_TP) * 2) * S);
#pragma unroll
      for (int c = lane; c < SU_TP * CPR; c += 32)
        if (c < n_out * CPR)
          dst[c] = *reinterpret_cast<const int4*>(st + (1 + c / CPR) * OP + (c % CPR) * 16);
    }
  }
}

template <typename T, int C, int S>
static int launch_su(const SqueezeUpconvParams& p, int B, cudaStream_t s) {
  using G = SuGeom<C, S>;
  SqueezeUpconvParams q = p;
  q.pdl_early = pdl_early_now;
  q.rows = B * p.H;
  q.tiles_per_row = (int)ceil_div(p.W, SU_TP);
  auto kern = squeeze_upconv_kernel<T, C, S>;
  static int ctas_per_sm = 0;
  if (ctas_per_sm == 0) {
    if (G::SMEM > 48 * 1024) PCLS_CHECK_CUDA(cudaFuncSetAttribute(kern, cudaFuncAttributeMaxDynamicSharedMemorySize, G::SMEM));
    PCLS_CHECK_CUDA(cudaOccupancyMaxActiveBlocksPerMultiprocessor(&ctas_per_sm, kern, SU_WARPS * 32, G::SMEM));
    if (ctas_per_sm < 1) ctas_per_sm = 1;
  }
  const long long total = (long long)q.rows * q.tiles_per_row;
  long long grid = (long long)sm_count() * ctas_per_sm;
  if (grid > ceil_div(total, SU_WARPS)) grid = ceil_div(total, SU_WARPS);
  if (grid < 1) grid = 1;
  PCLS_CHECK_CUDA(launch_pdl(kern, dim3((unsigned)grid), dim3(SU_WARPS * 32), (size_t)G::SMEM, s, q));
  return check_launch("squeeze_upconv_kernel");
}

bool squeeze_upconv_supported(int C, int S) {
  return (C == 64 && S == 16) || (C == 128 && S == 16) || (C == 256 && S == 32);
}

template <typename T>
int launch_squeeze_upconv(const SqueezeUpconvParams& p, int C, int S, int B, cudaStream_t s) {
  if (B == 0) return PCLS_OK;
  if (C == 64 && S == 16) return launch_su<T, 64, 16>(p, B, s);
  if (C == 128 && S == 16) return launch_su<T, 128, 16>(p, B, s);
  if (C == 256 && S == 32) return launch_su<T, 256, 32>(p, B, s);
  set_error("squeeze_upconv: unsupported shape C=%d S=%d", C, S);
  return PCLS_ERR_INVALID;
}
template int launch_squeeze_upconv<__half>(const SqueezeUpconvParams&, int, int, int, cudaStream_t);
template int launch_squeeze_upconv<__nv_bfloat16>(const SqueezeUpconvParams&, int, int, int, cudaStream_t);

}
```

Before: 12870.

## Fuse 1x1 squeeze conv into preceding residual 3x3 tensor-core conv epilogue

The residual 3x3 conv kernel gains a mode that runs the following 16-output 1x1 ReLU squeeze conv in its epilogue. It issues a second UMMA on the staged output tile against squeeze weights held in shared memory, and writes only the 16-channel squeezed tensor. The planner marks eligible conv pairs, skips launching the squeeze conv, and adds an upconv-only variant of the squeeze_upconv kernel that reads the precomputed 16-channel tensor with deeper prefetch. This removes one launch and a full-width write and read of the intermediate activation, at the cost of extra TMEM, barriers and shared memory, plus a more serialized epilogue.

```diff
diff --git a/pclsegmentation_b200/csrc/conv_tc.cu b/pclsegmentation_b200/csrc/conv_tc.cu
--- a/pclsegmentation_b200/csrc/conv_tc.cu
+++ b/pclsegmentation_b200/csrc/conv_tc.cu
@@ -61,6 +61,10 @@
   int32_t* preds;
   float* logits;
   unsigned long long* dbg;
+  int sqz;
+  const void* sq_w;
+  const float* sq_bias;
+  uint32_t sq_idesc;
 };
 
 template <typename T> __device__ __forceinline__ uint32_t pack2_relu(float lo, float hi);
@@ -196,11 +200,14 @@
                const __grid_constant__ TcParams p, const int num_tiles) {
   constexpr bool PRELOAD = !RES;
   constexpr int TC_NG = tc_ng(RES);
-  constexpr bool RTMA = RES && RM == 1;
+  constexpr bool RTMA = RES && (RM == 1 || RM == 4);
   constexpr bool PTMA = !RES && RM == 2;
   constexpr bool SKIP = RES && RM == 3;
   static_assert(!SKIP || (G == 4 && !LEAKY), "the computed skip exists for the pixel-group view G = 4 with ReLU");
   constexpr bool FIXED = RTMA || SKIP;
+  constexpr bool SQZ = RES && RM == 4;
+  static_assert(!SQZ || ((G == 2 || G == 4) && KC == 64 && !LEAKY), "the fused squeeze exists for the pixel-group views G = 2 / 4 with ReLU");
+  constexpr uint32_t SQW_BYTES = 8192u / (uint32_t)G;
   extern __shared__ uint8_t smem_raw[];
   const uint32_t smem_base = (smem_u32(smem_raw) + 1023u) & ~1023u;
   const int S = p.stages;
@@ -211,19 +218,32 @@
   const uint32_t bres_base = smem_base + (uint32_t)S * stage_bytes;
   const uint32_t cstage_base = bres_base + (uint32_t)p.bres_bytes;
   const uint32_t rstage_base = cstage_base + (p.tma_store ? (uint32_t)(p.n_cbuf * TC_NG) * (uint32_t)p.c_stage_bytes : 0u);
-  const uint32_t bar_base = rstage_base + ((RES && (SKIP || p.res_smem)) ? (uint32_t)TC_NG * 16384u : 0u);
+  const uint32_t sqw_base = rstage_base;
+  const uint32_t bar_base = rstage_base + ((RES && (SKIP || p.res_smem)) ? (uint32_t)TC_NG * 16384u : 0u) + (SQZ ? SQW_BYTES : 0u);
 #define FULL_BAR(s) (bar_base + 8u * (uint32_t)(s))
 #define EMPTY_BAR(s) (bar_base + 8u * (uint32_t)(S + (s)))
 #define TFULL_BAR(a) (bar_base + 8u * (uint32_t)(2 * S + (a)))
 #define TEMPTY_BAR(a) (bar_base + 8u * (uint32_t)(2 * S + 8 + (a)))
 #define BRES_BAR (bar_base + 8u * (uint32_t)(2 * S + 16))
 #define RFULL_BAR(i) (bar_base + 8u * (uint32_t)(2 * S + 17 + (i)))
-  const uint32_t tmem_slot = bar_base + 8u * (uint32_t)(2 * S + 17 + 3 * TC_NG);
+#define SQ_BAR(i) (bar_base + 8u * (uint32_t)(2 * S + 17 + 3 * TC_NG + (i)))
+  const uint32_t tmem_slot = bar_base + 8u * (uint32_t)(2 * S + 17 + 3 * TC_NG + (SQZ ? 3 * TC_NG : 0));
   volatile uint32_t* tmem_slot_ptr =
       reinterpret_cast<volatile uint32_t*>(smem_raw + (tmem_slot - smem_u32(smem_raw)));
   float* bias_s = reinterpret_cast<float*>(smem_raw + (((tmem_slot + 16u + 15u) & ~15u) - smem_u32(smem_raw)));
   for (int i = threadIdx.x; i < p.n_nt * p.BN; i += blockDim.x) bias_s[i] = p.bias[G > 1 ? i % p.cout_blk : i];
   float* head_s = bias_s + ((p.n_nt * p.BN + 3) & ~3);
+  float* const sqb_s = head_s;
+  if constexpr (SQZ) {
+    if (threadIdx.x < 16) sqb_s[threadIdx.x] = p.sq_bias[threadIdx.x];
+    constexpr int CPR = 32 / G;
+    const int4* w = reinterpret_cast<const int4*>(p.sq_w);
+    for (int i = threadIdx.x; i < 16 * CPR; i += blockDim.x) {
+      const int n = i / CPR, c = i % CPR;
+      st_shared_v4(sqw_base + (uint32_t)(c >> 3) * 2048u + (uint32_t)n * 128u + (uint32_t)(((c & 7) ^ (n & 7)) << 4), __ldg(w + i));
+    }
+    asm volatile("fence.proxy.async.shared::cta;" ::: "memory");
+  }
 
   const int warp = threadIdx.x >> 5, lane = threadIdx.x & 31;
   unsigned long long* const dbg = PCLS_TC_DEBUG ? p.dbg : nullptr;
@@ -237,6 +257,7 @@
     if (p.tma_store) asm volatile("prefetch.tensormap [%0];" ::"l"(&map_c) : "memory");
     if (RES && (SKIP || p.res_tma)) asm volatile("prefetch.tensormap [%0];" ::"l"(&map_r) : "memory");
     for (int i = 0; i < 3 * TC_NG; ++i) mbar_init(RFULL_BAR(i), 1);
+    if (SQZ) for (int i = 0; i < 3 * TC_NG; ++i) mbar_init(SQ_BAR(i), 1);
     for (int s = 0; s < S; ++s) { mbar_init(FULL_BAR(s), 1); mbar_init(EMPTY_BAR(s), 1); }
     for (int a = 0; a < 8; ++a) { mbar_init(TFULL_BAR(a), 1); mbar_init(TEMPTY_BAR(a), 4); }
     mbar_init(BRES_BAR, 1);
@@ -780,7 +801,10 @@
               int ntile = tile, ncb = cb + 64;
               if (ncb >= BN) { ncb = 0; ntile = tile_at(tl + ng); }
               if (ntile >= 0) {
-                if (nrb == 3u) bulk_wait_read1(); else bulk_wait_read0();
+                if constexpr (SQZ) {
+                  if (blk >= 2u) { DBG_T0; mbar_wait(SQ_BAR(grp * 3 + (int)((blk + 1u) % nrb)), ((blk - 2u) / nrb) & 1u); DBG_ADD(4); }
+                  bulk_wait_read0();
+                } else if (nrb == 3u) bulk_wait_read1(); else bulk_wait_read0();
                 issue_res(ntile, ncb, (blk + 1u) % nrb);
               }
             }
@@ -815,13 +839,24 @@
             process(va, cb, [&](int g, const int4& o) { st_shared_v4(row_addr + (uint32_t)((g ^ (m & 7)) << 4), o); });
             tmem_ld_wait();
             if (cb + 64 < BN) tmem_ld32(t_row + (uint32_t)(cb + 64), va);
-            else release_acc();
+            else if (!SQZ) release_acc();
             process(vb, cb + 32, [&](int g, const int4& o) { st_shared_v4(row_addr + (uint32_t)(((4 + g) ^ (m & 7)) << 4), o); });
           }
           asm volatile("fence.proxy.async.shared::cta;" ::: "memory");
           if (!res_tma) { DBG_T0; if (issuer) bulk_wait_read0(); DBG_ADD(4); }
+          if (SQZ) tc_fence_before();
           { DBG_T0; group_barrier(bar_id); DBG_ADD(5); }
-          if (issuer) {
+          if constexpr (SQZ) {
+            if (q == 3) {
+              tc_fence_after();
+              const uint32_t kb = (uint32_t)(cb & blk_mask) >> 6;
+              const uint32_t d = tmem_base + acc * (uint32_t)BN + (uint32_t)(cb & ~blk_mask);
+              const uint32_t desc_lo_flags = 0x10000u;
+              umma_f16_ksteps_elect<4>(d, ((buf >> 4) & 0x3FFFu) | desc_lo_flags, p.desc_hi,
+                                       (((sqw_base + kb * 2048u) >> 4) & 0x3FFFu) | desc_lo_flags, p.desc_hi, p.sq_idesc, kb);
+              umma_commit_elect(SQ_BAR(grp * 3 + (int)(blk % nrb)));
+            }
+          } else if (issuer) {
             const int pp = G > 1 ? (n0 + cb) >> blk_shift : 0;
             const int c0 = out_coff + (p.perm ? p.cblk_off[(n0 + cb) >> 6] : ((n0 + cb) & blk_mask));
             if (c_is_5d) tma_store_5d(&map_c, buf, c0, G > 1 ? pp : ph, wt * BW, ht * BH, b);
@@ -837,6 +872,38 @@
             if (off >= 0) *reinterpret_cast<int4*>(outp + off) = o;
           });
       }
+      if constexpr (SQZ) {
+        const uint32_t lb = blk - 1u;
+        const uint32_t sbuf = cstage_base + (uint32_t)(grp * (int)nrb + (int)(lb % nrb)) * c_stage_bytes;
+        { DBG_T0; mbar_wait(SQ_BAR(grp * 3 + (int)(lb % nrb)), (lb / nrb) & 1u); DBG_ADD(4); }
+        tc_fence_after();
+        uint32_t sv[G][16];
+#pragma unroll
+        for (int pp = 0; pp < G; ++pp) tmem_ld16(t_row + ((uint32_t)pp << blk_shift), sv[pp]);
+        tmem_ld_wait();
+        release_acc();
+#pragma unroll
+        for (int pp = 0; pp < G; ++pp)
+#pragma unroll
+          for (int h = 0; h < 2; ++h) {
+            const float4 b0 = *reinterpret_cast<const float4*>(sqb_s + 8 * h), b1 = *reinterpret_cast<const float4*>(sqb_s + 8 * h + 4);
+            const uint32_t* v = sv[pp] + 8 * h;
+            int4 o;
+            o.x = (int)pack2_relu<T>(__uint_as_float(v[0]) + b0.x, __uint_as_float(v[1]) + b0.y);
+            o.y = (int)pack2_relu<T>(__uint_as_float(v[2]) + b0.z, __uint_as_float(v[3]) + b0.w);
+            o.z = (int)pack2_relu<T>(__uint_as_float(v[4]) + b1.x, __uint_as_float(v[5]) + b1.y);
+            o.w = (int)pack2_relu<T>(__uint_as_float(v[6]) + b1.z, __uint_as_float(v[7]) + b1.w);
+            const uint32_t ch = (uint32_t)(2 * pp + h);
+            st_shared_v4(G == 4 ? sbuf + (uint32_t)m * 128u + ((ch ^ (uint32_t)(m & 7)) << 4)
+                                : sbuf + (uint32_t)m * 64u + ((ch ^ (uint32_t)((m >> 1) & 3)) << 4), o);
+          }
+        asm volatile("fence.proxy.async.shared::cta;" ::: "memory");
+        { DBG_T0; group_barrier(bar_id); DBG_ADD(5); }
+        if (issuer) {
+          tma_store_4d(&map_c, sbuf, 0, wt * BW, ht * BH, b);
+          bulk_commit();
+        }
+      }
       if (!released) release_acc();
       if (dbg) { dbg_acc[6] += clk() - _te; dbg_acc[7] += 1; }
     }
@@ -864,6 +931,7 @@
 #undef TEMPTY_BAR
 #undef BRES_BAR
 #undef RFULL_BAR
+#undef SQ_BAR
 }
 
 typedef void (*TcKernelFn)(const CUtensorMap, const CUtensorMap, const CUtensorMap, const CUtensorMap, const CUtensorMap, const CUtensorMap, const TcParams, const int);
@@ -976,6 +1044,10 @@
   return conv_tc_kernel<T, 64, 3, 1, true, LEAKY, 4, 1>;
 }
 static TcKernelFn tc_kernel_for(int KC, int SUB, int G, int is_bf16, int res, int leaky, int ks = 0, int rtma = 0) {
+  if (rtma == 4) {
+    if (is_bf16) return G == 4 ? conv_tc_kernel<__nv_bfloat16, 64, 3, 4, true, false, 4, 4> : conv_tc_kernel<__nv_bfloat16, 64, 3, 2, true, false, 4, 4>;
+    return G == 4 ? conv_tc_kernel<__half, 64, 3, 4, true, false, 4, 4> : conv_tc_kernel<__half, 64, 3, 2, true, false, 4, 4>;
+  }
   if (rtma == 3)
     return is_bf16 ? conv_tc_kernel<__nv_bfloat16, 64, 3, 4, true, false, 4, 3> : conv_tc_kernel<__half, 64, 3, 4, true, false, 4, 3>;
   if (rtma == 2 && !res) {
@@ -1069,6 +1141,20 @@
       (e.out_channels * 2) % 16 != 0)
     return false;
   return true;
+}
+
+bool Net::tc_squeeze_fusable(const ConvLayer& E, const ConvLayer& Q) const {
+  const ConvParams &e = E.p, &q = Q.p;
+  if (Q.in != E.out || q.mode != MODE_1x1 || q.act != PCLS_ACT_RELU || Q.res0 >= 0 || Q.res1 >= 0 || Q.pool_src >= 0 ||
+      q.out_f32 || q.out_coff != 0 || q.cout != 16 || q.cout_pad != 16 || q.out_channels != 16 || Q.cin_logical != e.cout ||
+      q.cin_pad != e.cout)
+    return false;
+  if (E.res0 < 0 || E.res1 >= 0 || E.skip_src >= 0 || E.pair_view || e.mode != MODE_3x3_S1 || e.act != PCLS_ACT_RELU ||
+      e.out_f32 || e.out_coff != 0 || e.cout != e.out_channels || e.cout != e.cout_pad || e.res0_channels != e.cout)
+    return false;
+  const int G = tc_group_size(e);
+  return tc_eligible(e) && (G == 2 || G == 4) && e.cout * G == 256 && tc_halo_mode && tc_tma_store_mode && tc_res_tma_mode &&
+         tc_rtma_mode;
 }
 
 int Net::tc_plan_layer(ConvLayer& L, bool allow_group, bool* retry) {
@@ -1089,6 +1175,7 @@
     q.n_nt = cp.cout_pad / q.BN;
     const int G = allow_group ? tc_group_size(cp) : 1;
     const bool skip = L.skip_src >= 0;
+    const bool sqz = L.sq_dst >= 0;
     const int cin_blk = cp.cin_pad;
     q.G = G; q.cout_blk = G > 1 ? cp.cout_pad : (1 << 30);
     q.cout_blk_shift = 0;
@@ -1228,7 +1315,13 @@
     q.res_tma = (!skip && tc_res_tma_mode && L.res0 >= 0 && q.tma_store && q.cbw == 64 && q.b_resident && (cp.res0_channels * 2) % 16 == 0) ? 1 : 0;
     q.n_cbuf = (q.res_tma && !q.nsplit) ? 3 : 2;
     q.res_smem = (!skip && !q.res_tma && L.res0 >= 0 && q.BN <= 128) ? 1 : 0;
-    const int cstage_total = (q.tma_store ? q.n_cbuf * TC_NG * q.c_stage_bytes : 0) + ((q.res_smem || skip) ? TC_NG * 16384 : 0);
+    const int cstage_total = (q.tma_store ? q.n_cbuf * TC_NG * q.c_stage_bytes : 0) + ((q.res_smem || skip) ? TC_NG * 16384 : 0) +
+                             (sqz ? 16 * cp.cout * 2 : 0);
+    if (sqz && !(G >= 2 && G * cp.cout == 256 && q.tma_store && q.cbw == 64 && q.b_resident && q.res_tma && q.n_cbuf == 3 &&
+                 q.BN == 256 && q.KC == 64 && q.BW == 128 && q.BH == 1 && q.n_nt == 1 && !q.nsplit)) {
+      set_error("tc plan: the layer that computes the fused squeeze is not planned on the pixel-group residual TMA-store path");
+      delete plan; return PCLS_ERR_STATE;
+    }
     if (skip && !(G == 4 && q.tma_store && q.cbw == 64 && q.b_resident && q.BN == 256 && q.BW == 128 && q.BH == 1)) {
       set_error("tc plan: the layer that computes the fused skip is not planned on the G = 4 TMA-store path");
       delete plan; return PCLS_ERR_STATE;
@@ -1243,6 +1336,7 @@
     q.R = 1; q.n_hseg = q.Hgrid;
     plan->smem_bytes = (size_t)stages * stage_bytes + q.bres_bytes + cstage_total + 1024  +
                        (size_t)(2 * stages + 17 + 3 * TC_NG) * 8 + 48 + (cp.out_f32 ? 4 * TC_NG * 32 * 33 * 4 : 0) + (size_t)cp.cout_pad * 4 ;
+    if (sqz) plan->smem_bytes += (size_t)3 * TC_NG * 8  + (size_t)(q.BN - cp.cout_pad) * 4  + 64;
     const uint32_t layout = swz == 128 ? 2u : swz == 64 ? 4u : 6u;
     const uint32_t sbo = (uint32_t)(8 * swz) >> 4;
     q.desc_hi = sbo | (1u << 14)  | (layout << 29);
@@ -1318,7 +1412,18 @@
       rc = make_map(&plan->map_b2, bf16, const_cast<void*>(w_src), 3, dims, str, box, swz_b);
       if (rc) { delete plan; return rc; }
     }
-    if (q.tma_store) {
+    if (sqz) {
+      const ConvLayer& Q = convs[L.sq_dst];
+      const uint64_t Cs = (uint64_t)G * 16, Wg = (uint64_t)cp.Wout / G;
+      const uint64_t dims[4] = {Cs, Wg, Hh, F};
+      const uint64_t str[3] = {Cs * 2, Wg * Cs * 2, Hh * Wg * Cs * 2};
+      const uint32_t box[4] = {(uint32_t)Cs, 128u, 1u, 1u};
+      rc = make_map(&plan->map_c, bf16, tensor_ptr(Q.out, frames_per_pass), 4, dims, str, box, G == 4 ? 128 : 64);
+      if (rc) { delete plan; return rc; }
+      plan->map_c2 = plan->map_c;
+      q.sqz = 1; q.sq_w = Q.p.w; q.sq_bias = Q.p.bias;
+      q.sq_idesc = (1u << 4) | ((bf16 ? 1u : 0u) << 7) | ((bf16 ? 1u : 0u) << 10) | ((uint32_t)(16 >> 3) << 17) | ((uint32_t)(128 >> 4) << 24);
+    } else if (q.tma_store) {
       char* c_base = (char*)tensor_ptr(L.out, frames_per_pass);
       const uint64_t Co = (uint64_t)cp.out_channels, Wo = (uint64_t)cp.Wout;
       const int csw = q.cbw == 64 ? 128 : 0;
@@ -1403,7 +1508,7 @@
   bool& attr_set = attr_set_dev[dev & 63];
   for (auto& L : convs) {
     bool retry = false;
-    if (L.skip_into >= 0) continue;
+    if (L.skip_into >= 0 || L.sq_into >= 0) continue;
     int rc = head_plan_layer(L);
     if (rc) return rc;
     if (L.hp) { L.tc_ok = true; continue; }
@@ -1435,6 +1540,8 @@
           }
       PCLS_CHECK_CUDA(cudaFuncSetAttribute(tc_kernel_for(64, 3, 1, bf, 0, 0, 3, 2), cudaFuncAttributeMaxDynamicSharedMemorySize, max_smem));
       PCLS_CHECK_CUDA(cudaFuncSetAttribute(tc_kernel_for(64, 3, 4, bf, 1, 0, 0, 3), cudaFuncAttributeMaxDynamicSharedMemorySize, max_smem));
+      for (int g = 2; g <= 4; g *= 2)
+        PCLS_CHECK_CUDA(cudaFuncSetAttribute(tc_kernel_for(64, 3, g, bf, 1, 0, 0, 4), cudaFuncAttributeMaxDynamicSharedMemorySize, max_smem));
     }
     attr_set = true;
   }
@@ -1463,7 +1570,7 @@
   }
   int grid = work < sm_count() ? work : sm_count();
   if (prm.nsplit) grid -= grid % prm.n_nt;
-  const int rtma = prm.skip ? 3 : (tc_rtma_mode && prm.res_tma && prm.res0 && !prm.res1 && prm.tma_store && !prm.out_f32 &&
+  const int rtma = prm.sqz ? 4 : prm.skip ? 3 : (tc_rtma_mode && prm.res_tma && prm.res0 && !prm.res1 && prm.tma_store && !prm.out_f32 &&
                     (prm.act == PCLS_ACT_RELU || prm.act == PCLS_ACT_LEAKY) && !(PCLS_TC_VSTREAM && prm.vstream)) ? 1
                  : ((tc_rtma_mode & 2) && !prm.res0 && !prm.res1 && prm.tma_store && !prm.out_f32 && !(PCLS_TC_VSTREAM && prm.vstream)) ? 2 : 0;
   const bool res = prm.res0 || prm.res1 || prm.skip;
diff --git a/pclsegmentation_b200/csrc/net.cu b/pclsegmentation_b200/csrc/net.cu
--- a/pclsegmentation_b200/csrc/net.cu
+++ b/pclsegmentation_b200/csrc/net.cu
@@ -281,14 +281,14 @@
   reads.clear(); writes.clear();
   if (op.type == OP_CONV) {
     const ConvLayer& L = convs[op.index];
-    if (L.skip_into >= 0) return;
+    if (L.skip_into >= 0 || L.sq_into >= 0) return;
     reads.push_back(L.in);
     if (L.pool_src >= 0) reads.push_back(L.pool_src);
-    if (L.up_squeeze >= 0) reads.push_back(convs[L.up_squeeze].in);
+    if (L.up_squeeze >= 0 && convs[L.up_squeeze].sq_into < 0) reads.push_back(convs[L.up_squeeze].in);
     if (L.skip_src >= 0) reads.push_back(convs[L.skip_src].in);
     else if (L.res0 >= 0) reads.push_back(L.res0);
     if (L.res1 >= 0) reads.push_back(L.res1);
-    writes.push_back(L.out);
+    writes.push_back(L.sq_dst >= 0 ? convs[L.sq_dst].out : L.out);
   } else if (op.type == OP_POOL) {
     reads.push_back(pools[op.index].in); writes.push_back(pools[op.index].out);
   } else {
@@ -326,6 +326,25 @@
       if (other_reader) continue;
       P.fused_conv = ops[i + 1].index;
       L.pool_src = P.in; L.pool_pad_left = P.pad_left;
+    }
+  if (fuse_squeeze && !keep_tensors && conv_impl == 0)
+    for (int i = 0; i < n_ops; ++i) {
+      if (ops[i].type != OP_CONV) continue;
+      ConvLayer& E = convs[ops[i].index];
+      if (E.out == logits_tensor || E.pool_src >= 0) continue;
+      int reader = -1, n_use = 0;
+      std::vector<int> rd, wr;
+      for (int k = 0; k < n_ops; ++k) {
+        if (k == i) continue;
+        op_tensors(ops[k], rd, wr);
+        for (int r : rd) if (r == E.out) { ++n_use; reader = k; }
+        for (int w : wr) if (w == E.out) n_use += 2;
+      }
+      if (n_use != 1 || ops[reader].type != OP_CONV) continue;
+      ConvLayer& Q = convs[ops[reader].index];
+      if (Q.out == logits_tensor || !tc_squeeze_fusable(E, Q)) continue;
+      E.sq_dst = ops[reader].index;
+      Q.sq_into = ops[i].index;
     }
   if (fuse_up && !keep_tensors)
     for (int i = 0; i + 1 < n_ops; ++i) {
@@ -366,7 +385,7 @@
       }
       if (n_use != 1 || ops[reader].type != OP_CONV) continue;
       ConvLayer& E = convs[ops[reader].index];
-      if (E.pool_src >= 0 || E.up_squeeze >= 0 || !tc_skip_fusable(P, E)) continue;
+      if (E.pool_src >= 0 || E.up_squeeze >= 0 || E.sq_dst >= 0 || !tc_skip_fusable(P, E)) continue;
       E.skip_src = ops[i].index;
       P.skip_into = ops[reader].index;
     }
@@ -428,7 +447,7 @@
   frame_bytes = align_up(peak, 1024);
   for (size_t t = 0; t < tensors.size(); ++t) {
     bool fused_skip = false;
-    for (const auto& L : convs) fused_skip = fused_skip || (L.skip_into >= 0 && L.out == (int)t);
+    for (const auto& L : convs) fused_skip = fused_skip || ((L.skip_into >= 0 || L.sq_dst >= 0) && L.out == (int)t);
     PCLS_REQUIRE(t == 0 || tensors[t].first >= 0 || fused_skip, "pcls_net_finalize: tensor %d is never written", (int)t);
   }
 
@@ -505,15 +524,16 @@
       p.res0 = (L.res0 >= 0 && L.skip_src < 0) ? tensor_ptr(L.res0, nb) : nullptr;
       p.res1 = L.res1 >= 0 ? tensor_ptr(L.res1, nb) : nullptr;
       if (conv_impl == 0 && L.fused_into_up >= 0) continue;
-      if (L.skip_into >= 0) continue;
+      if (L.skip_into >= 0 || L.sq_into >= 0) continue;
       if (conv_impl == 0 && L.up_squeeze >= 0) {
         const ConvLayer& Q = convs[L.up_squeeze];
+        const bool up_only = Q.sq_into >= 0;
         SqueezeUpconvParams su;
-        su.in = tensor_ptr(Q.in, nb); su.out = p.out;
-        su.w1 = Q.p.w; su.b1 = Q.p.bias; su.w1_stride = Q.p.cin_pad; su.act1 = Q.p.act;
+        su.in = tensor_ptr(up_only ? Q.out : Q.in, nb); su.out = p.out;
+        su.w1 = up_only ? nullptr : Q.p.w; su.b1 = Q.p.bias; su.w1_stride = Q.p.cin_pad; su.act1 = Q.p.act;
         su.w2 = p.w; su.b2 = p.bias; su.w2_cout_pad = p.cout_pad; su.w2_cin_pad = p.cin_pad; su.act2 = p.act;
         su.H = H; su.W = p.Win; su.rows = 0; su.tiles_per_row = 0;
-        rc = launch_squeeze_upconv<T>(su, Q.p.cin_pad, Q.p.cout, nb, s);
+        rc = launch_squeeze_upconv<T>(su, up_only ? Q.p.cout : Q.p.cin_pad, Q.p.cout, nb, s);
       } else if (conv_impl == 0 && L.pool_src >= 0) {
         PoolConvParams pc;
         pc.in = tensor_ptr(L.pool_src, nb); pc.out = p.out; pc.w = p.w; pc.bias = p.bias;
@@ -718,6 +738,11 @@
         by += (int64_t)H * (tensors[L.pool_src].width - p.Win) * cin * 2;
         snprintf(buf, sizeof(buf), "pool+%s_%dx%d_w%d", mode, (int)cin, (int)cout, p.Wout);
       }
+      if (L.sq_dst >= 0) {
+        const ConvLayer& Q = convs[L.sq_dst];
+        by += (int64_t)H * p.Wout * (Q.cout_logical - cout) * 2 + (int64_t)Q.cin_logical * Q.cout_logical * 2;
+        fl += 2 * (int64_t)H * p.Wout * Q.cin_logical * Q.cout_logical;
+      }
       if (L.skip_src >= 0) {
         const ConvLayer& P = convs[L.skip_src];
         by += (int64_t)H * W * tensors[P.in].stride * 2 + (int64_t)P.cin_logical * P.cout_logical * 2;
@@ -727,7 +752,7 @@
       }
       if (L.res1 >= 0) by += (int64_t)H * p.Wout * cout * 2;
       fam = (conv_impl == 0 && L.tc_ok) ? 1 : 0;
-      if (L.skip_into >= 0) {
+      if (L.skip_into >= 0 || L.sq_into >= 0) {
         snprintf(buf, sizeof(buf), "%s_%dx%d_w%d(fused)", mode, (int)cin, (int)cout, p.Wout);
         fl = 0; by = 0; fam = 0;
       }
@@ -735,7 +760,9 @@
         snprintf(buf, sizeof(buf), "%s_%dx%d_w%d(fused)", mode, (int)cin, (int)cout, p.Wout);
         fl = 0; by = 0; fam = 0;
       }
-      if (conv_impl == 0 && L.up_squeeze >= 0) {
+      if (conv_impl == 0 && L.up_squeeze >= 0 && convs[L.up_squeeze].sq_into >= 0) {
+        fam = 0;
+      } else if (conv_impl == 0 && L.up_squeeze >= 0) {
         const ConvLayer& Q = convs[L.up_squeeze];
         snprintf(buf, sizeof(buf), "conv1x1_%dx%d+%s_w%d", Q.cin_logical, Q.cout_logical, mode, p.Wout);
         fl += 2 * (int64_t)H * p.Win * Q.cin_logical * Q.cout_logical;
@@ -766,7 +793,7 @@
   PCLS_REQUIRE(finalized && t >= 0 && t < (int)tensors.size(), "pcls_net_read_tensor: bad tensor id %d", t);
   PCLS_REQUIRE(B >= 0 && B <= frames_per_pass, "pcls_net_read_tensor: B exceeds the frames of one pass");
   PCLS_REQUIRE(t == 0 || tensors[t].first >= 0, "pcls_net_read_tensor: tensor %d is computed inside the conv that reads it "
-               "(set keep_tensors or fuse_skip = 0 before finalize)", t);
+               "(set keep_tensors, or fuse_skip = 0 / fuse_squeeze = 0, before finalize)", t);
   const TensorInfo& ti = tensors[t];
   const int64_t n = (int64_t)B * H * ti.width * ti.channels;
   if (ti.logits) { PCLS_CHECK_CUDA(cudaMemcpyAsync(out, tensor_ptr(t, B), n * 4, cudaMemcpyDeviceToDevice, s)); return PCLS_OK; }
@@ -888,7 +915,7 @@
   int launches = 1;
   for (const OpRef& op : n->ops) {
     if (op.type == OP_CONV && n->conv_impl == 0 && n->convs[op.index].fused_into_up >= 0) continue;
-    if (op.type == OP_CONV && n->convs[op.index].skip_into >= 0) continue;
+    if (op.type == OP_CONV && (n->convs[op.index].skip_into >= 0 || n->convs[op.index].sq_into >= 0)) continue;
     if (op.type == OP_POOL && n->conv_impl == 0 && n->pools[op.index].fused_conv >= 0) continue;
     ++launches;
   }
@@ -906,8 +933,9 @@
   if (!strcmp(name, "conv_impl")) {
     PCLS_REQUIRE(value == 0 || value == 1, "conv_impl must be 0 or 1");
     bool skip_fused = false;
-    for (const auto& L : n->convs) skip_fused = skip_fused || L.skip_into >= 0;
-    PCLS_REQUIRE(value == 0 || !skip_fused, "conv_impl = 1 needs a net finalized with fuse_skip = 0 (or conv_impl = 1 set before)");
+    for (const auto& L : n->convs) skip_fused = skip_fused || L.skip_into >= 0 || L.sq_into >= 0;
+    PCLS_REQUIRE(value == 0 || !skip_fused,
+                 "conv_impl = 1 needs a net finalized with fuse_skip = 0 and fuse_squeeze = 0 (or conv_impl = 1 set before)");
     n->conv_impl = value; return PCLS_OK;
   }
   if (!strcmp(name, "use_graph")) { n->use_graph = value != 0; if (!n->use_graph) n->drop_graphs(); return PCLS_OK; }
@@ -950,6 +978,10 @@
     PCLS_REQUIRE(!n->finalized, "fuse_skip must be set before pcls_net_finalize");
     n->fuse_skip = value != 0; return PCLS_OK;
   }
+  if (!strcmp(name, "fuse_squeeze")) {
+    PCLS_REQUIRE(!n->finalized, "fuse_squeeze must be set before pcls_net_finalize");
+    n->fuse_squeeze = value != 0; return PCLS_OK;
+  }
   if (!strcmp(name, "fuse_head")) { n->fuse_head = value != 0; n->drop_graphs(); return PCLS_OK; }
   if (!strcmp(name, "tc_debug")) {
     PCLS_REQUIRE(!value || tc_debug_compiled, "tc_debug needs a library built with PCLS_NVCC_FLAGS=-DPCLS_TC_DEBUG=1");
diff --git a/pclsegmentation_b200/csrc/net.cuh b/pclsegmentation_b200/csrc/net.cuh
--- a/pclsegmentation_b200/csrc/net.cuh
+++ b/pclsegmentation_b200/csrc/net.cuh
@@ -35,6 +35,8 @@
   int fused_into_up = -1;
   int skip_src = -1;
   int skip_into = -1;
+  int sq_dst = -1;
+  int sq_into = -1;
   bool pair_view = false;
   ConvParams ptc;
   std::vector<float> w_tc, bias_tc;
@@ -77,6 +79,7 @@
   bool fuse_pool = true;
   bool fuse_head = true;
   bool fuse_skip = true;
+  bool fuse_squeeze = true;
   struct HeadArgs { int head = 0, none_index = 0; const uint8_t* mask = nullptr; float* probs = nullptr; int32_t* preds = nullptr; float* logits = nullptr; } head_args;
   int micro_batch = 0;
   int cam_px = 0;
@@ -121,6 +124,7 @@
   int tc_prepare();
   int tc_plan_layer(ConvLayer& L, bool allow_group, bool* retry);
   bool tc_skip_fusable(const ConvLayer& P, const ConvLayer& E) const;
+  bool tc_squeeze_fusable(const ConvLayer& E, const ConvLayer& Q) const;
   int tc_launch(ConvLayer& L, const ConvParams& p, int nb, cudaStream_t s);
   void tc_release();
   int head_plan_layer(ConvLayer& L);
diff --git a/pclsegmentation_b200/csrc/squeeze_upconv.cu b/pclsegmentation_b200/csrc/squeeze_upconv.cu
--- a/pclsegmentation_b200/csrc/squeeze_upconv.cu
+++ b/pclsegmentation_b200/csrc/squeeze_upconv.cu
@@ -39,11 +39,12 @@
   static constexpr int SMEM = (W1_FRAGS + W2_FRAGS) * 32 * 8 + SU_WARPS * WARP_BYTES;
 };
 
-template <typename T, int C, int S>
+template <typename T, int C, int S, bool SQ = true>
 __global__ void __launch_bounds__(SU_WARPS * 32, (C <= 64 ? 3 : (C <= 128 ? 2 : 1)))
 squeeze_upconv_kernel(const SqueezeUpconvParams p) {
   using G = SuGeom<C, S>;
-  constexpr int SLABS = G::SLABS, NT = G::NT, KS2 = G::KS2, NLD = G::NLD, QP = G::QP, OP = G::OP;
+  static_assert(SQ || (C == 16 && S == 16), "the upconv-only variant reads a 16-channel squeeze tensor");
+  constexpr int SLABS = G::SLABS, NT = G::NT, KS2 = G::KS2, NLD = SQ ? G::NLD : 1, QP = G::QP, OP = G::OP;
   constexpr int CV = C / 8;
   extern __shared__ int4 su_smem[];
   uint2* const w1s = reinterpret_cast<uint2*>(su_smem);
@@ -70,7 +71,7 @@
   float b1r[NT][2], b2r[NT][2];
 #pragma unroll
   for (int j = 0; j < NT; ++j) {
-    b1r[j][0] = p.b1[8 * j + 2 * t]; b1r[j][1] = p.b1[8 * j + 2 * t + 1];
+    if (SQ) { b1r[j][0] = p.b1[8 * j + 2 * t]; b1r[j][1] = p.b1[8 * j + 2 * t + 1]; }
     b2r[j][0] = p.b2[8 * j + 2 * t]; b2r[j][1] = p.b2[8 * j + 2 * t + 1];
   }
   uint32_t a_addr[3];
@@ -89,10 +90,15 @@
   const long long wstep = (long long)gridDim.x * SU_WARPS;
   const int4* const in = reinterpret_cast<const int4*>(p.in);
   T* const out = reinterpret_cast<T*>(p.out);
-  int4 nx[NLD];
+  constexpr int PF = SQ ? 1 : 4;
+  int4 nx[PF][NLD];
   auto load = [&](long long wt, int4 (&v)[NLD]) {
     const long long row = wt / p.tiles_per_row;
     const int p0 = (int)(wt % p.tiles_per_row) * SU_TP - 1;
+    if constexpr (!SQ) {
+      v[0] = __ldg(in + (row * p.W + min(max(p0 + (lane >> 1), 0), p.W - 1)) * CV + (lane & 1));
+      return;
+    }
     const int4* base = in + row * (long long)p.W * CV + 2 * t;
 #pragma unroll
     for (int px = 0; px < 2; ++px) {
@@ -105,15 +111,26 @@
     }
   };
   long long wt = (long long)blockIdx.x * SU_WARPS + warp;
-  if (wt < total) load(wt, nx);
+#pragma unroll
+  for (int d = 0; d < PF; ++d)
+    if (wt + d * wstep < total) load(wt + d * wstep, nx[d]);
   for (; wt < total; wt += wstep) {
     int4 cur[NLD];
 #pragma unroll
-    for (int i = 0; i < NLD; ++i) cur[i] = nx[i];
-    if (wt + wstep < total) load(wt + wstep, nx);
+    for (int i = 0; i < NLD; ++i) cur[i] = nx[0][i];
+#pragma unroll
+    for (int d = 0; d + 1 < PF; ++d)
+#pragma unroll
+      for (int i = 0; i < NLD; ++i) nx[d][i] = nx[d + 1][i];
+    if (wt + PF * wstep < total) load(wt + PF * wstep, nx[PF - 1]);
     const long long row = wt / p.tiles_per_row;
     const int q = (int)(wt % p.tiles_per_row), p0 = q * SU_TP - 1;
 
+    if constexpr (!SQ) {
+      __syncwarp();
+      const int px = p0 + (lane >> 1);
+      *reinterpret_cast<int4*>(sq + (lane >> 1) * QP + (lane & 1) * 16) = (px >= 0 && px < p.W) ? cur[0] : make_int4(0, 0, 0, 0);
+    } else {
     float acc[NT][4];
 #pragma unroll
     for (int j = 0; j < NT; ++j) { acc[j][0] = 0.0f; acc[j][1] = 0.0f; acc[j][2] = 0.0f; acc[j][3] = 0.0f; }
@@ -143,6 +160,7 @@
         *reinterpret_cast<uint32_t*>(sq + g * QP + (8 * j + 2 * t) * 2) = lo;
         *reinterpret_cast<uint32_t*>(sq + (g + 8) * QP + (8 * j + 2 * t) * 2) = hi;
       }
+    }
     }
     __syncwarp();
 
@@ -189,14 +207,14 @@
   }
 }
 
-template <typename T, int C, int S>
+template <typename T, int C, int S, bool SQ = true>
 static int launch_su(const SqueezeUpconvParams& p, int B, cudaStream_t s) {
   using G = SuGeom<C, S>;
   SqueezeUpconvParams q = p;
   q.pdl_early = pdl_early_now;
   q.rows = B * p.H;
   q.tiles_per_row = (int)ceil_div(p.W, SU_TP);
-  auto kern = squeeze_upconv_kernel<T, C, S>;
+  auto kern = squeeze_upconv_kernel<T, C, S, SQ>;
   static int ctas_per_sm = 0;
   if (ctas_per_sm == 0) {
     if (G::SMEM > 48 * 1024) PCLS_CHECK_CUDA(cudaFuncSetAttribute(kern, cudaFuncAttributeMaxDynamicSharedMemorySize, G::SMEM));
@@ -218,6 +236,11 @@
 template <typename T>
 int launch_squeeze_upconv(const SqueezeUpconvParams& p, int C, int S, int B, cudaStream_t s) {
   if (B == 0) return PCLS_OK;
+  if (p.w1 == nullptr) {
+    if (C == 16 && S == 16) return launch_su<T, 16, 16, false>(p, B, s);
+    set_error("squeeze_upconv: unsupported upconv-only shape C=%d S=%d", C, S);
+    return PCLS_ERR_INVALID;
+  }
   if (C == 64 && S == 16) return launch_su<T, 64, 16>(p, B, s);
   if (C == 128 && S == 16) return launch_su<T, 128, 16>(p, B, s);
   if (C == 256 && S == 32) return launch_su<T, 256, 32>(p, B, s);
```

After: 13150 (median of 6 runs). 2.2% higher.
